# MatthewRalston/kmerdb

Hardware: AMD Instinct MI355X
Metric: k-mers counted/sec at k=12, synthetic 150 bp FASTQ (higher is better)
Workload: dtype u64

## Files before the change

### kmerdb_amd/csrc/kdb_engine.hip

```cpp
#include <hip/hip_runtime.h>

#include <cstdarg>
#include <cstddef>
#include <cstdio>
#include <cstdlib>
#include <algorithm>
#include <atomic>
#include <cstring>
#include <string>
#include <thread>
#include <vector>

#include "../../include/kdbhip.h"
#include "kdb_kernels.hip.h"
#include "kdb_hist.hip.h"
#include "kdb_scatter.hip.h"
#include "kdb_smallk.hip.h"
#include "kdb_probe.hip.h"
#include "kdb_hostparse.cpp.h"
#include "kdb_kdbwriter.cpp.h"

namespace {

thread_local std::string g_err;
// ... 180 lines not shown
        e->ev_pool.push_back(s.a);
        e->ev_pool.push_back(s.b);
    }
    e->spans.clear();
    return KDB_OK;
}

int ensure_staging(kdb_engine *e)
{
    if (e->staging_ready) return KDB_OK;
    for (int b = 0; b < NBUF; b++) {
        HIP_TRY(hipHostMalloc((void **)&e->h_bases[b], e->stage_bytes + 64, hipHostMallocDefault));
        HIP_TRY(hipHostMalloc((void **)&e->h_offs[b], (e->stage_reads + 1) * sizeof(uint64_t), hipHostMallocDefault));
        HIP_TRY(hipMalloc((void **)&e->d_bases[b], e->stage_bytes + 64));
        HIP_TRY(hipMalloc((void **)&e->d_offs[b], (e->stage_reads + 1) * sizeof(uint64_t)));
        HIP_TRY(hipEventCreateWithFlags(&e->ev_copied[b], hipEventDisableTiming));
        HIP_TRY(hipEventCreateWithFlags(&e->ev_done[b], hipEventDisableTiming));
    }
    e->staging_ready = true;
    const int64_t want = e->accum_bytes >= 0 ? e->accum_bytes : (e->k >= 13 ? (int64_t)1 << 30 : 0);
    if (want > 0) {
        e->acc_cap = (size_t)want < e->stage_bytes ? e->stage_bytes : (size_t)want;
        e->acc_reads_cap = e->acc_cap / 64 + e->stage_reads;
        for (int s = 0; s < 2; s++) {
            HIP_TRY(hipMalloc((void **)&e->d_acc_bases[s], e->acc_cap + 64));
            HIP_TRY(hipMalloc((void **)&e->d_acc_offs[s], (e->acc_reads_cap + 1) * sizeof(uint64_t)));
            HIP_TRY(hipEventCreateWithFlags(&e->ev_acc_done[s], hipEventDisableTiming));
        }
        HIP_TRY(hipEventCreateWithFlags(&e->ev_acc_copied, hipEventDisableTiming));
        e->acc_ready = true;
    }
    return KDB_OK;
}

int overlap_join(kdb_engine *e)
{
    if (e->ov.last < 0) return KDB_OK;
    HIP_TRY(hipStreamWaitEvent(e->s_compute, e->ov.hist_done[e->ov.last], 0));
    e->ov.last = -1;
    return KDB_OK;
}

int overlap_streams(kdb_engine *e)
{
    const bool want_hist = e->overlap != 0, want_mask = want_hist && e->overlap_hist_cus > 0;
    if (e->s_hist) { HIP_TRY(hipStreamSynchronize(e->s_hist)); HIP_TRY(hipStreamDestroy(e->s_hist)); e->s_hist = nullptr; }
    kdb::overlap_free(e->ov);
    if (e->compute_masked || want_mask) {
        HIP_TRY(hipStreamSynchronize(e->s_compute));
        HIP_TRY(hipStreamDestroy(e->s_compute));
        e->s_compute = nullptr;
        e->compute_masked = false;
    }
    if (!want_hist) {
        if (!e->s_compute) HIP_TRY(hipStreamCreateWithFlags(&e->s_compute, hipStreamNonBlocking));
        return KDB_OK;
    }
    if (!want_mask) {
        if (!e->s_compute) HIP_TRY(hipStreamCreateWithFlags(&e->s_compute, hipStreamNonBlocking));
        HIP_TRY(hipStreamCreateWithFlags(&e->s_hist, hipStreamNonBlocking));
        e->ov.grid = 0;
        return KDB_OK;
    }
    if (!getenv("KDB_ALLOW_CU_MASKS")) {
        e->overlap_hist_cus = 0;
        (void)overlap_streams(e);
        return fail(KDB_ERR_ARG, "overlap_hist_cus: CU-masked streams are a diagnostic (set KDB_ALLOW_CU_MASKS=1; see include/kdbhip.h)");
    }
    hipDeviceProp_t prop;
    HIP_TRY(hipGetDeviceProperties(&prop, e->device));
    const int ncu = prop.multiProcessorCount, H = e->overlap_hist_cus;
    if (H >= ncu || ncu > 1024) return fail(KDB_ERR_ARG, "overlap_hist_cus=%d of %d CUs", H, ncu);
    std::vector<uint32_t> mh((size_t)(ncu + 31) / 32, 0u), ms((size_t)(ncu + 31) / 32, 0u);
    int given = 0;
    for (int i = 0; i < ncu; i++) {
        bool hist;
        if (e->overlap_mask_mode == 1) hist = given < H && (int)(((long long)i * H) / ncu) != (int)(((long long)(i + 1) * H) / ncu);
        else if (e->overlap_mask_mode == 2) hist = given < H && (i % 32) < (H * 32 + ncu - 1) / ncu;
        else hist = i < H;
        if (hist) { mh[(size_t)i / 32] |= 1u << (i % 32); given++; } else ms[(size_t)i / 32] |= 1u << (i % 32);
    }
    HIP_TRY(hipExtStreamCreateWithCUMask(&e->s_compute, (uint32_t)ms.size(), ms.data()));
    e->compute_masked = true;
    HIP_TRY(hipExtStreamCreateWithCUMask(&e->s_hist, (uint32_t)mh.size(), mh.data()));
    e->ov.grid = 2u * (uint32_t)(ncu - given);
    return KDB_OK;
}

enum : int { BATCH_HOST_FED = 1, BATCH_CONST_INPUT = 2 };
int grow(void **p, size_t *cap, size_t need_bytes);
int launch_batch(kdb_engine *e, uint8_t *d_bases, size_t nbytes, const uint64_t *d_offs, size_t nreads, int first_is_continuation, int flags);

int flush_accumulated(kdb_engine *e)
{
    if (!e->acc_ready || e->acc_nr == 0) return KDB_OK;
    const int s = e->acc_slot;
    HIP_TRY(hipEventRecord(e->ev_acc_copied, e->s_copy));
    HIP_TRY(hipStreamWaitEvent(e->s_compute, e->ev_acc_copied, 0));
    int rc = launch_batch(e, e->d_acc_bases[s], e->acc_nb, e->d_acc_offs[s], e->acc_nr, 0, BATCH_HOST_FED);
    if (rc != KDB_OK) return rc;
    HIP_TRY(hipEventRecord(e->ev_acc_done[s], e->s_compute));
    e->acc_inflight[s] = true;
    e->acc_slot = s ^ 1;
    e->acc_nb = e->acc_nr = 0;
    return KDB_OK;
}

int launch_batch(kdb_engine *e, uint8_t *d_bases, size_t nbytes, const uint64_t *d_offs, size_t nreads, int first_is_continuation, int flags)
{
    if (nreads == 0) return KDB_OK;
    if (e->tableless) return fail(KDB_ERR_STATE, "this engine was created by kdb_create_ids: it has no count vector");
    const uint64_t ntiles = (nbytes + kdb::TILE_BYTES - 1) / kdb::TILE_BYTES;
    if (ntiles > 0x7FFFFFFFull) return fail(KDB_ERR_ARG, "batch too large: %zu bytes", nbytes);
    bool marked = false;
    auto mark = [&]() {
        ProfScope ps(e, KDB_KERNEL_MARK);
        const unsigned mg = (unsigned)std::min<uint64_t>((nreads + 255) / 256, 4096);
        if (flags & BATCH_CONST_INPUT)
            hipLaunchKernelGGL(kdb::require_uniform_kernel, dim3(1), dim3(1), 0, e->s_compute, e->d_ctr);
        else {
            hipLaunchKernelGGL(kdb::mark_reads_kernel, dim3(mg), dim3(256), 0, e->s_compute, d_bases, d_offs, (uint64_t)nreads,
                               first_is_continuation, e->d_ctr);
            marked = true;
        }
    };
    auto unmark = [&]() {
        if (!marked) return;
        ProfScope ps(e, KDB_KERNEL_MARK);
        const unsigned ug = (unsigned)std::min<uint64_t>((nreads + 255) / 256, 4096);
        hipLaunchKernelGGL(kdb::unmark_reads_kernel, dim3(ug), dim3(256), 0, e->s_compute, d_bases, d_offs, (uint64_t)nreads, first_is_continuation,
                           (const kdb::DevCounters *)e->d_ctr);
        marked = false;
    };
    bool no_first_rec = false;
    {
        const size_t need = ((nbytes >> kdb::FIRST_REC_SHIFT) + 2) * sizeof(uint32_t);
        if (e->first_rec_cap < need && e->d_first_rec) HIP_TRY(hipStreamSynchronize(e->s_compute));
        int grc = grow((void **)&e->d_first_rec, &e->first_rec_cap, need);
        if (grc == KDB_ERR_NOMEM) no_first_rec = true;
        else if (grc != KDB_OK) return grc;
    }
    {
        ProfScope ps(e, KDB_KERNEL_MARK);
        const dim3 grid((unsigned)((nreads + 255) / 256)), block(256);
        HIP_TRY(hipMemsetAsync(&e->d_ctr->neg_min_len, 0, kdb::PER_BATCH_WORDS * sizeof(unsigned long long), e->s_compute));
        const dim3 lgrid(grid.x < 1024u ? grid.x : 1024u);
        hipLaunchKernelGGL(kdb::lens_kernel, lgrid, block, 0, e->s_compute, d_offs, (uint64_t)nreads, (uint64_t)nbytes,
                           e->min_len > 0 ? e->min_len : e->k, first_is_continuation, e->d_ctr, e->d_first_rec);
    }
    if (nbytes == 0) return KDB_OK;
    if (nreads > 0xFFFFFFF0ull) return fail(KDB_ERR_ARG, "batch of %zu records: at most 2^32 - 16 per submit", nreads);
    e->bytes_in += nbytes;
    const kdb::RecStarts rs{d_offs, e->d_first_rec, (uint32_t)nreads, first_is_continuation ? 1u : 0u};
    int algo = (int)e->algo;
    if (algo == 0 || algo == 3) algo = 2;
    if (no_first_rec && algo == 2) { algo = 1; e->oom_fallbacks++; e->tp.table_is_zero = false; }
    const bool paged2 = algo == 2 && e->k > e->one_level_max_k;
    if (!paged2 || e->n_mode == KDB_N_EXPAND || !e->tp.defer) e->tp.table_is_zero = false;
    if (algo == 2) {
        EngineProf hook(e);
        const bool ex = e->n_mode == KDB_N_EXPAND;
        int rc;
        if (e->k <= kdb::SMALLK_LDS_MAX_K && !e->smallk_old)
            rc = kdb::smallk_lds_count(e->s_compute, d_bases, nbytes, rs, e->k, e->canonical, ex, e->sc.grid, e->d_table, e->d_ctr, hook);
        else if (e->k <= kdb::SMALLK_MAX) {
            mark();
            rc = kdb::smallk_count(e->s_compute, d_bases, nbytes, e->k, e->canonical, ex, e->d_table, e->d_ctr, hook);
            unmark();
        }
        else if (e->k <= e->one_level_max_k) {
            rc = 3;
            if (e->overlap && e->s_hist && !ex) {
                e->ov.sc[0].grid = e->sc.grid; e->ov.sc[0].lo_bits = e->sc.lo_bits; e->ov.sc[0].contig_pages = e->sc.contig_pages; e->ov.sc[0].wide_lines = e->sc.wide_lines;
                rc = kdb::scatter_count_overlapped(e->ov, e->s_compute, e->s_hist, d_bases, nbytes, rs, e->k, e->canonical, e->d_table, e->d_ctr, hook);
            }
            if (rc == 3) {
                { const int jrc = overlap_join(e); if (jrc != KDB_OK) return jrc; }
                rc = kdb::scatter_count(e->sc, e->s_compute, d_bases, nbytes, rs, e->k, e->canonical, ex, e->d_table, e->d_ctr, hook);
            }
        }
        else {
            const size_t lost = nreads * (size_t)(e->k - 1);
            rc = kdb::twolevel_paged_count(e->tp, e->s_compute, d_bases, nbytes, rs, nbytes > lost ? nbytes - lost : 0, e->k, e->canonical, ex, e->d_table, e->d_ctr, hook);
        }
        if (rc == 2) { e->oom_fallbacks++; algo = 1; e->tp.table_is_zero = false; }
        else if (rc != 0) return fail(KDB_ERR_HIP, "LDS-histogram path failed: %s", kdb::partition_error());
    }
    if (algo == 1) {
        { const int jrc = overlap_join(e); if (jrc != KDB_OK) return jrc; }
        mark();
        {
            ProfScope ps(e, KDB_KERNEL_COUNT);
            const bool ex = (e->n_mode == KDB_N_EXPAND);
            const dim3 grid((unsigned)ntiles), block(kdb::TPB);
#define KDB_LAUNCH_DIRECT(ID, EX)                                                                              \
    hipLaunchKernelGGL((kdb::count_direct_kernel<ID, EX>), grid, block, 0, e->s_compute, d_bases, (uint64_t)nbytes, \
                       e->k, e->canonical, e->d_table, e->d_ctr)
            if (e->k <= 16) { if (ex) KDB_LAUNCH_DIRECT(uint32_t, true); else KDB_LAUNCH_DIRECT(uint32_t, false); }
            else            { if (ex) KDB_LAUNCH_DIRECT(uint64_t, true); else KDB_LAUNCH_DIRECT(uint64_t, false); }
#undef KDB_LAUNCH_DIRECT
        }
        unmark();
    }
    if (e->n_mode == KDB_N_EXPAND && e->d_worklist) {
        ProfScope ps(e, KDB_KERNEL_COUNT);
        hipLaunchKernelGGL(kdb::expand_worklist_kernel, dim3(1024), dim3(256), 0, e->s_compute, e->d_table, e->d_ctr, e->k, e->canonical);
    }
    if (e->n_mode == KDB_N_DROP) {
        ProfScope ps(e, KDB_KERNEL_MARK);
        hipLaunchKernelGGL(kdb::resolve_suspects_kernel, dim3(4), dim3(256), 0, e->s_compute, (const uint8_t *)d_bases, (uint64_t)nbytes, d_offs, (uint64_t)nreads,
                           e->k, e->d_ctr);
    }
    HIP_TRY(hipGetLastError());
    return KDB_OK;
}

int flush_pending_paged(kdb_engine *e)
{
    if (e->tp.pending == 0) return KDB_OK;
    EngineProf hook(e);
    if (kdb::twolevel_paged_flush(e->tp, e->s_compute, e->d_table, e->d_ctr, hook)) return fail(KDB_ERR_HIP, "LDS-histogram path failed: %s", kdb::partition_error());
    return KDB_OK;
}

int check_errors(kdb_engine *e)
{
    kdb::DevCounters c;
    HIP_TRY(hipMemcpy(&c, e->d_ctr, sizeof c, hipMemcpyDeviceToHost));
    if (c.n_short)
        return fail(KDB_ERR_SHORT_READ, "%llu record(s) shorter than k=%d (reference: kmer.py:461-463 raises)",
                    c.n_short, e->k);
    if (c.bad_layout)
        return fail(KDB_ERR_ARG, "read_offsets must rise from 0 to nbytes (records tile the residue buffer exactly)");
    if (c.internal_err)
        return fail(KDB_ERR_STATE, "internal: a scatter kernel ran out of its page sequence (%llu times); counts are incomplete", c.internal_err);
    if (c.not_uniform)
        return fail(KDB_ERR_ARG, "kdb_submit_device_const needs records of one length (the buffer is never marked); use kdb_submit_device");
    if (c.n_bad)
        return fail(KDB_ERR_BAD_RESIDUE, "%llu residue(s) outside ACGTN%s (reference: kmer.py:309 / :170 raises)", c.n_bad,
                    e->n_mode == KDB_N_DROP ? " that no N in their window shields" : "");
    if (c.marks_seen != c.marks_set)
        return fail(KDB_ERR_BAD_RESIDUE, "the residue buffer holds %lld byte(s) with bit 7 set that are not record starts of their batch "
                                         "(not residues -- kmer.py:170 raises -- or marks left in a device buffer by a job that was aborted)",
                    (long long)(c.marks_seen - c.marks_set));
    return KDB_OK;
}

int grow(void **p, size_t *cap, size_t need_bytes)
{
    if (*cap >= need_bytes) return KDB_OK;
    if (*p) { (void)hipFree(*p); *p = nullptr; *cap = 0; }
    size_t want = need_bytes + need_bytes / 4 + 256;
    hipError_t err = hipMalloc(p, want);
    if (err != hipSuccess) { (void)hipGetLastError(); return fail(KDB_ERR_NOMEM, "hipMalloc(%zu) failed: %s", want, hipGetErrorString(err)); }
    *cap = want;
    return KDB_OK;
}

int shred_scratch(kdb_engine *e, size_t nbytes, size_t nreads)
{
    int rc;
    if ((rc = grow((void **)&e->sh_seq, &e->sh_seq_cap, nbytes + 64)) != KDB_OK) return rc;
    if ((rc = grow((void **)&e->sh_ids, &e->sh_ids_cap, nbytes * 8ull)) != KDB_OK) return rc;
    if (nreads && (rc = grow((void **)&e->sh_offs, &e->sh_offs_cap, (nreads + 1) * sizeof(uint64_t))) != KDB_OK) return rc;
    if (!e->sh_ctr) HIP_TRY(hipMalloc((void **)&e->sh_ctr, sizeof(kdb::DevCounters)));
    if (!e->sh_suspects) HIP_TRY(hipMalloc((void **)&e->sh_suspects, e->suspects_cap * sizeof(unsigned long long)));
    return KDB_OK;
}

int create_common(kdb_engine *e, kdb_engine **out)
{
    hipError_t err;
    if ((err = hipStreamCreateWithFlags(&e->s_compute, hipStreamNonBlocking)) != hipSuccess ||
        (err = hipStreamCreateWithFlags(&e->s_copy, hipStreamNonBlocking)) != hipSuccess ||
        (err = hipMalloc((void **)&e->d_ctr, sizeof(kdb::DevCounters))) != hipSuccess) {
        kdb_destroy(e);
        return fail(KDB_ERR_HIP, "engine setup failed: %s", hipGetErrorString(err));
    }
    int rc = kdb_reset(e);
    if (rc != KDB_OK) { kdb_destroy(e); return rc; }
    if (const char *opts = getenv("KDB_ENGINE_OPTS")) {
        std::string all(opts);
        for (size_t at = 0; at < all.size();) {
            size_t end = all.find(',', at);
            if (end == std::string::npos) end = all.size();
            const std::string kv = all.substr(at, end - at);
            at = end + 1;
            if (kv.empty()) continue;
            const size_t eq = kv.find('=');
            if (eq == std::string::npos) { kdb_destroy(e); return fail(KDB_ERR_ARG, "KDB_ENGINE_OPTS: '%s' is not name=value", kv.c_str()); }
            rc = kdb_set_option(e, kv.substr(0, eq).c_str(), (int64_t)strtoll(kv.c_str() + eq + 1, nullptr, 0));
            if (rc != KDB_OK) { kdb_destroy(e); return rc; }
        }
    }
    *out = e;
    return KDB_OK;
}

}

namespace {
struct ProbePattern { const char *name; void (*launch)(const uint8_t *, uint64_t, uint8_t *, uint64_t, uint32_t, uint32_t *, hipStream_t); uint32_t read_bytes, write_bytes; };
template <int RM, int WM, int NR, int NW>
void probe_launch(const uint8_t *src, uint64_t sb, uint8_t *dst, uint64_t db, uint32_t steps, uint32_t *sink, hipStream_t st)
{
    hipLaunchKernelGGL((kdbprobe::pattern<RM, WM, NR, NW>), dim3(512), dim3(512), 0, st, src, sb, dst, db, steps, sink);
}
using namespace kdbprobe;
#define KDB_PROBE(name, RM, WM, NR, NW) {name, probe_launch<RM, WM, NR, NW>, (uint32_t)(NR * (RM == R_PAGES15 ? 1536 : RM ? 1024 : 0)), (uint32_t)(NW * (WM ? 1024 : 0))}
const ProbePattern PROBES[] = {
    KDB_PROBE("stream_read", R_STREAM, W_NONE, 4, 0),
    KDB_PROBE("stream_write", R_NONE, W_STREAM, 0, 4),
    KDB_PROBE("pages_1k_read", R_PAGES, W_NONE, 4, 0),
    KDB_PROBE("lines_64_write", R_NONE, W_LINES_SC1, 0, 2),
    KDB_PROBE("pieces_128_write", R_NONE, W_CHUNK128_SC1, 0, 2),
    KDB_PROBE("scatter_64", R_STREAM, W_LINES_SC1, 1, 2),
    KDB_PROBE("scatter_128", R_STREAM, W_CHUNK128_SC1, 1, 2),
    KDB_PROBE("level1_64", R_STREAM, W_LINES_SC1, 1, 3),
    KDB_PROBE("level1_128", R_STREAM, W_CHUNK128_SC1, 1, 3),
    KDB_PROBE("level2_64", R_PAGES15, W_LINES_SC1, 2, 2),
    KDB_PROBE("level2_128", R_PAGES15, W_CHUNK128_SC1, 2, 2),
};
#undef KDB_PROBE
constexpr int N_PROBES = (int)(sizeof(PROBES) / sizeof(PROBES[0]));
}

extern "C" {

int kdb_abi_version(void) { return KDB_ABI_VERSION; }

const char *kdb_last_error(void) { return g_err.c_str(); }

int kdb_device_count(int *n_out)
{
    if (!n_out) return fail(KDB_ERR_ARG, "n_out is NULL");
    HIP_TRY(hipGetDeviceCount(n_out));
    return KDB_OK;
}

const char *kdb_prof_kernel_name(int kernel_id)
{
    if (kernel_id < 0 || kernel_id >= KDB_N_KERNELS) return "";
    return KERNEL_NAMES[kernel_id];
}

int kdb_create(int k, int canonicalize, int n_mode, int device_id, void *d_table, kdb_engine **out)
{
    if (!out) return fail(KDB_ERR_ARG, "out is NULL");
    *out = nullptr;
    if (k < 1 || k > 17) return fail(KDB_ERR_ARG, "k=%d outside 1..17 (4^k uint64 table must fit in HBM)", k);
    if (n_mode != KDB_N_DROP && n_mode != KDB_N_EXPAND) return fail(KDB_ERR_ARG, "n_mode=%d", n_mode);
    int ndev = 0;
    HIP_TRY(hipGetDeviceCount(&ndev));
    if (device_id < 0 || device_id >= ndev) return fail(KDB_ERR_ARG, "device_id=%d but %d device(s) visible", device_id, ndev);
    DeviceGuard g(device_id);
    kdb_engine *e = new kdb_engine();
    e->k = k; e->canonical = canonicalize ? 1 : 0; e->n_mode = n_mode; e->device = device_id;
    e->nbins = 1ull << (2 * k);
    if (d_table) {
        e->d_table = (unsigned long long *)d_table;
        e->owns_table = false;
    } else {
        size_t free_b = 0, total_b = 0;
        (void)hipMemGetInfo(&free_b, &total_b);
        const unsigned long long need = e->nbins * 8ull;
        if (free_b && need > free_b) {
            delete e;
            return fail(KDB_ERR_NOMEM, "4^%d uint64 table needs %llu bytes, device has %zu free", k, need, free_b);
        }
        hipError_t me = hipMalloc((void **)&e->d_table, need);
        if (me != hipSuccess) { delete e; return fail(KDB_ERR_NOMEM, "hipMalloc(%llu) failed: %s", need, hipGetErrorString(me)); }
        e->owns_table = true;
    }
    return create_common(e, out);
}

int kdb_create_ids(int k, int canonicalize, int device_id, kdb_engine **out)
{
    if (!out) return fail(KDB_ERR_ARG, "out is NULL");
    *out = nullptr;
    if (k < 1 || k > 17) return fail(KDB_ERR_ARG, "k=%d outside 1..17", k);
    int ndev = 0;
    HIP_TRY(hipGetDeviceCount(&ndev));
    if (device_id < 0 || device_id >= ndev) return fail(KDB_ERR_ARG, "device_id=%d but %d device(s) visible", device_id, ndev);
    DeviceGuard g(device_id);
    kdb_engine *e = new kdb_engine();
    e->k = k; e->canonical = canonicalize ? 1 : 0; e->n_mode = KDB_N_DROP; e->device = device_id;
    e->nbins = 0; e->tableless = true;
    return create_common(e, out);
}

int kdb_destroy(kdb_engine *e)
{
    if (!e) return KDB_OK;
    DeviceGuard g(e->device);
    if (e->s_compute) (void)hipStreamSynchronize(e->s_compute);
    if (e->s_copy) (void)hipStreamSynchronize(e->s_copy);
    if (e->s_hist) { (void)hipStreamSynchronize(e->s_hist); (void)hipStreamDestroy(e->s_hist); }
    kdb::overlap_free(e->ov);
    kdb::scatter_free(e->sc);
    kdb::twolevel_paged_free(e->tp);
    for (auto &s : e->spans) { (void)hipEventDestroy(s.a); (void)hipEventDestroy(s.b); }
    for (auto ev : e->ev_pool) (void)hipEventDestroy(ev);
    for (int b = 0; b < NBUF; b++) {
        if (e->h_bases[b]) (void)hipHostFree(e->h_bases[b]);
        if (e->h_offs[b]) (void)hipHostFree(e->h_offs[b]);
        if (e->d_bases[b]) (void)hipFree(e->d_bases[b]);
        if (e->d_offs[b]) (void)hipFree(e->d_offs[b]);
        if (e->ev_copied[b]) (void)hipEventDestroy(e->ev_copied[b]);
        if (e->ev_done[b]) (void)hipEventDestroy(e->ev_done[b]);
    }
    for (int s2 = 0; s2 < 2; s2++) {
        if (e->d_acc_bases[s2]) (void)hipFree(e->d_acc_bases[s2]);
        if (e->d_acc_offs[s2]) (void)hipFree(e->d_acc_offs[s2]);
        if (e->ev_acc_done[s2]) (void)hipEventDestroy(e->ev_acc_done[s2]);
    }
    if (e->ev_acc_copied) (void)hipEventDestroy(e->ev_acc_copied);
    for (int s2 = 0; s2 < 2; s2++) if (e->ev_pin[s2]) (void)hipEventDestroy(e->ev_pin[s2]);
    if (e->d_worklist) (void)hipFree(e->d_worklist);
    if (e->d_suspects) (void)hipFree(e->d_suspects);
    if (e->d_first_rec) (void)hipFree(e->d_first_rec);
    if (e->sh_suspects) (void)hipFree(e->sh_suspects);
    if (e->sh_seq) (void)hipFree(e->sh_seq);
    if (e->sh_offs) (void)hipFree(e->sh_offs);
    if (e->sh_ids) (void)hipFree(e->sh_ids);
    if (e->sh_ctr) (void)hipFree(e->sh_ctr);
    if (e->d_acc_table) (void)hipFree(e->d_acc_table);
    if (e->d_ctr) (void)hipFree(e->d_ctr);
    if (e->owns_table && e->d_table) (void)hipFree(e->d_table);
    if (e->s_compute) (void)hipStreamDestroy(e->s_compute);
    if (e->s_copy) (void)hipStreamDestroy(e->s_copy);
    delete e;
    return KDB_OK;
}

int kdb_reset(kdb_engine *e)
{
    if (!e) return fail(KDB_ERR_ARG, "engine is NULL");
    DeviceGuard g(e->device);
    e->acc_nb = e->acc_nr = 0;
    kdb::twolevel_paged_drop(e->tp);
    HIP_TRY(hipStreamSynchronize(e->s_copy));
    HIP_TRY(hipStreamSynchronize(e->s_compute));
    if (e->s_hist) { HIP_TRY(hipStreamSynchronize(e->s_hist)); e->ov.last = -1; }
    if (e->nbins) HIP_TRY(hipMemsetAsync(e->d_table, 0, e->nbins * 8ull, e->s_compute));
    if (e->d_acc_table) HIP_TRY(hipMemsetAsync(e->d_acc_table, 0, e->nbins * 8ull, e->s_compute));
    e->folded_files = e->folded_total = 0;
    e->tp.table_is_zero = e->owns_table && !e->table_escaped;
    HIP_TRY(hipMemsetAsync(e->d_ctr, 0, sizeof(kdb::DevCounters), e->s_compute));
    unsigned long long wl[2] = {0, 0}, sus[2] = {0, 0};
    if (e->n_mode == KDB_N_EXPAND) {
        if (!e->d_worklist) HIP_TRY(hipMalloc((void **)&e->d_worklist, e->worklist_cap * sizeof(unsigned long long)));
        wl[0] = (unsigned long long)(uintptr_t)e->d_worklist; wl[1] = (unsigned long long)e->worklist_cap;
        HIP_TRY(hipMemcpyAsync(&e->d_ctr->wl, wl, sizeof wl, hipMemcpyHostToDevice, e->s_compute));
    } else if (!e->tableless) {
        if (!e->d_suspects) HIP_TRY(hipMalloc((void **)&e->d_suspects, e->suspects_cap * sizeof(unsigned long long)));
        sus[0] = (unsigned long long)(uintptr_t)e->d_suspects; sus[1] = (unsigned long long)e->suspects_cap;
        HIP_TRY(hipMemcpyAsync(&e->d_ctr->sus, sus, sizeof sus, hipMemcpyHostToDevice, e->s_compute));
    }
    HIP_TRY(hipStreamSynchronize(e->s_compute));
    return KDB_OK;
}

int kdb_submit_device(kdb_engine *e, void *d_bases, size_t nbytes, const void *d_read_offsets, size_t nreads)
{
    if (!e) return fail(KDB_ERR_ARG, "engine is NULL");
    if (nreads && (!d_bases || !d_read_offsets)) return fail(KDB_ERR_ARG, "NULL device buffer");
    if (((uintptr_t)d_bases & 15u) != 0) return fail(KDB_ERR_ARG, "d_bases must be 16-byte aligned");
    DeviceGuard g(e->device);
    return launch_batch(e, (uint8_t *)d_bases, nbytes, (const uint64_t *)d_read_offsets, nreads, 0, 0);
}

int kdb_submit_device_const(kdb_engine *e, const void *d_bases, size_t nbytes, const void *d_read_offsets, size_t nreads)
{
    if (!e) return fail(KDB_ERR_ARG, "engine is NULL");
    if (nreads && (!d_bases || !d_read_offsets)) return fail(KDB_ERR_ARG, "NULL device buffer");
    if (((uintptr_t)d_bases & 15u) != 0) return fail(KDB_ERR_ARG, "d_bases must be 16-byte aligned");
    DeviceGuard g(e->device);
    return launch_batch(e, (uint8_t *)const_cast<void *>(d_bases), nbytes, (const uint64_t *)d_read_offsets, nreads, 0, BATCH_CONST_INPUT);
}

static int submit_impl(kdb_engine *e, const uint8_t *bases, size_t nbytes, const uint64_t *offs, size_t nreads, bool src_pinned, bool first_continues = false)
{
    if (!e) return fail(KDB_ERR_ARG, "engine is NULL");
    if (nreads == 0) return KDB_OK;
    if (!offs || (!bases && nbytes)) return fail(KDB_ERR_ARG, "NULL host buffer");
    if (offs[nreads] < offs[0] || offs[nreads] > nbytes) return fail(KDB_ERR_ARG, "read_offsets exceed nbytes");
    DeviceGuard g(e->device);
    int rc = ensure_staging(e);
    if (rc != KDB_OK) return rc;
    if (src_pinned) {
        const int pi = e->pin_idx;
        if (!e->ev_pin[pi]) HIP_TRY(hipEventCreateWithFlags(&e->ev_pin[pi], hipEventDisableTiming));
        if (e->pin_used[pi]) HIP_TRY(hipEventSynchronize(e->ev_pin[pi]));
    }
    const uint64_t cap = e->stage_bytes;
    const uint64_t overlap = (uint64_t)(e->k - 1);
    size_t r = 0;
    bool cont = first_continues;
    uint64_t carry = first_continues ? offs[0] : 0;
    while (r < nreads) {
        const int b = e->next_buf;
        if (e->inflight[b]) { HIP_TRY(hipEventSynchronize(e->busy[b])); e->inflight[b] = false; }
        uint8_t *hb = e->h_bases[b];
        uint64_t *ho = e->h_offs[b];
        const int first_is_cont = cont ? 1 : 0;
        const uint64_t start = cont ? carry : offs[r];
        const size_t rmax = (nreads - r < e->stage_reads) ? nreads : r + e->stage_reads;
        const uint64_t *ub = std::upper_bound(offs + r + 1, offs + rmax + 1, start + cap);
        size_t r1 = (size_t)(ub - offs) - 1;
        uint64_t nb;
        size_t nr;
        ho[0] = 0;
        if (r1 <= r) {
            nb = cap; nr = 1; ho[1] = cap;
            carry = start + cap - overlap; cont = true;
        } else {
            nb = offs[r1] - start; nr = r1 - r;
            uint64_t prev = start;
            for (size_t i = 1; i <= nr; i++) {
                const uint64_t o = offs[r + i];
                if (o < prev) return fail(KDB_ERR_ARG, "read_offsets not monotone at %zu", r + i);
                prev = o;
                ho[i] = o - start;
            }
            r = r1; cont = false;
        }
        const bool accumulate = e->acc_ready && !first_is_cont && !cont && nb <= e->acc_cap && nr <= e->acc_reads_cap;
        if (accumulate) {
            if (e->acc_nb + nb > e->acc_cap || e->acc_nr + nr > e->acc_reads_cap) { rc = flush_accumulated(e); if (rc != KDB_OK) return rc; }
            const int s = e->acc_slot;
            if (e->acc_inflight[s]) { HIP_TRY(hipEventSynchronize(e->ev_acc_done[s])); e->acc_inflight[s] = false; }
            for (size_t i = 0; i <= nr; i++) ho[i] += e->acc_nb;
            const uint8_t *src = src_pinned ? bases + start : hb;
            if (!src_pinned) parallel_copy(hb, bases + start, nb, e->copy_threads);
            HIP_TRY(hipMemcpyAsync(e->d_acc_bases[s] + e->acc_nb, src, nb, hipMemcpyHostToDevice, e->s_copy));
            HIP_TRY(hipMemcpyAsync(e->d_acc_offs[s] + e->acc_nr, ho, (nr + 1) * sizeof(uint64_t), hipMemcpyHostToDevice, e->s_copy));
            HIP_TRY(hipEventRecord(e->ev_copied[b], e->s_copy));
            e->busy[b] = e->ev_copied[b];
            e->acc_nb += nb; e->acc_nr += nr;
        } else {
            rc = flush_accumulated(e);
            if (rc != KDB_OK) return rc;
            if (src_pinned) {
                HIP_TRY(hipMemcpyAsync(e->d_bases[b], bases + start, nb, hipMemcpyHostToDevice, e->s_copy));
            } else {
                parallel_copy(hb, bases + start, nb, e->copy_threads);
                HIP_TRY(hipMemcpyAsync(e->d_bases[b], hb, nb, hipMemcpyHostToDevice, e->s_copy));
            }
            HIP_TRY(hipMemcpyAsync(e->d_offs[b], ho, (nr + 1) * sizeof(uint64_t), hipMemcpyHostToDevice, e->s_copy));
            HIP_TRY(hipEventRecord(e->ev_copied[b], e->s_copy));
            HIP_TRY(hipStreamWaitEvent(e->s_compute, e->ev_copied[b], 0));
            rc = launch_batch(e, e->d_bases[b], nb, e->d_offs[b], nr, first_is_cont, BATCH_HOST_FED);
            if (rc != KDB_OK) return rc;
            HIP_TRY(hipEventRecord(e->ev_done[b], e->s_compute));
            e->busy[b] = e->ev_done[b];
        }
        e->inflight[b] = true;
        e->next_buf = (b + 1) % NBUF;
    }
    if (src_pinned) {
        HIP_TRY(hipEventRecord(e->ev_pin[e->pin_idx], e->s_copy));
        e->pin_used[e->pin_idx] = true;
        e->pin_idx ^= 1;
    }
    return KDB_OK;
}

int kdb_submit(kdb_engine *e, const uint8_t *bases, size_t nbytes, const uint64_t *offs, size_t nreads)
{
    return submit_impl(e, bases, nbytes, offs, nreads, false);
}

int kdb_submit_pinned(kdb_engine *e, const uint8_t *bases, size_t nbytes, const uint64_t *offs, size_t nreads)
{
    return submit_impl(e, bases, nbytes, offs, nreads, true);
}

int kdb_submit_ex(kdb_engine *e, const uint8_t *bases, size_t nbytes, const uint64_t *offs, size_t nreads, int flags)
{
    if (flags & ~(KDB_SUBMIT_PINNED | KDB_SUBMIT_CONTINUES)) return fail(KDB_ERR_ARG, "kdb_submit_ex: unknown flags 0x%x", flags);
    return submit_impl(e, bases, nbytes, offs, nreads, (flags & KDB_SUBMIT_PINNED) != 0, (flags & KDB_SUBMIT_CONTINUES) != 0);
}

int kdb_host_alloc(void **out, size_t nbytes)
{
    if (!out) return fail(KDB_ERR_ARG, "out is NULL");
    *out = nullptr;
    hipError_t err = hipHostMalloc(out, nbytes ? nbytes : 1, hipHostMallocDefault);
    if (err != hipSuccess) return fail(KDB_ERR_NOMEM, "hipHostMalloc(%zu) failed: %s", nbytes, hipGetErrorString(err));
    return KDB_OK;
}

int kdb_host_free(void *p)
{
    if (p) HIP_TRY(hipHostFree(p));
    return KDB_OK;
}

int kdb_sync(kdb_engine *e)
{
    if (!e) return fail(KDB_ERR_ARG, "engine is NULL");
// ... 810 lines not shown
```

### kmerdb_amd/csrc/kdb_kernels.hip.h

```cpp
#pragma once
#include <hip/hip_runtime.h>
#include <stdint.h>

namespace kdb {

constexpr int TPB = 256;
constexpr int CHUNKS_PER_THREAD = 4;
constexpr int TILE_CHUNKS = TPB * CHUNKS_PER_THREAD;
constexpr int TILE_BYTES = TILE_CHUNKS * 16;

struct DevCounters {
    unsigned long long total_kmers;
    unsigned long long n_short;
    unsigned long long n_bad;
    unsigned long long unique;
    unsigned long long sum;
    unsigned long long bad_layout;
    unsigned long long not_uniform;
    unsigned long long internal_err;
    unsigned long long table_dirty;
    unsigned long long marks_set, marks_seen;
    unsigned long long pages_bases, lines_bases;
    unsigned long long pages_ids, lines_ids;
    unsigned long long table_bytes;
    unsigned long long neg_min_len;
    unsigned long long max_len;
    unsigned long long wl_count;
    unsigned long long sus_count;
    unsigned long long *wl;
    unsigned long long wl_cap;
    unsigned long long *sus;
    unsigned long long sus_cap;
    unsigned long long *hot_side;
};
constexpr int PER_BATCH_WORDS = 4;

__device__ __forceinline__ uint32_t batch_uniform_len(const DevCounters *c)
{
    const unsigned long long mx = c->max_len, mn = ~c->neg_min_len;
    return (mx == mn && mx != 0 && mx < (1ull << 30)) ? (uint32_t)mx : 0u;
}

constexpr int FIRST_REC_SHIFT = 12;

__global__ void __launch_bounds__(256)
lens_kernel(const uint64_t *__restrict__ offs, uint64_t nreads, uint64_t nbytes, int k, int first_is_continuation, DevCounters *ctr,
            uint32_t *__restrict__ first_rec )
{
    __shared__ unsigned long long s_len[4], s_neg[4], s_short[4], s_bad[4];
    unsigned long long len = 0, neg = 0, nshort = 0, nbadl = 0;
    const uint64_t stride = (uint64_t)gridDim.x * blockDim.x;
    for (uint64_t rb = (uint64_t)blockIdx.x * blockDim.x + threadIdx.x; rb < nreads; rb += 4 * stride) {
        uint64_t sv[4], ev[4];
#pragma unroll
        for (int u = 0; u < 4; u++) {
            const uint64_t r = rb + (uint64_t)u * stride;
            sv[u] = r < nreads ? offs[r] : 0ull;
            ev[u] = r < nreads ? offs[r + 1] : 0ull;
        }
#pragma unroll
        for (int u = 0; u < 4; u++) {
            const uint64_t r = rb + (uint64_t)u * stride, s = sv[u], e = ev[u];
            if (r >= nreads) break;
            unsigned long long l = e - s;
            neg = neg > ~l ? neg : ~l;
            if (!(r == 0 && first_is_continuation)) nshort += (l < (uint64_t)k) ? 1 : 0;
            nbadl += (r == 0 && s != 0) + (r == nreads - 1 && e != nbytes) + (e < s || e > nbytes);
            if (r == 0 && first_is_continuation) l = ~0ull;
            len = len > l ? len : l;
            if (first_rec && e > s) {
                const uint64_t e2 = e < nbytes ? e : nbytes;
                for (uint64_t b = (s + ((1ull << FIRST_REC_SHIFT) - 1ull)) >> FIRST_REC_SHIFT; (b << FIRST_REC_SHIFT) < e2; b++) first_rec[b] = (uint32_t)r;
            }
        }
    }
#pragma unroll
    for (int o = 32; o > 0; o >>= 1) {
        const unsigned long long l2 = __shfl_down(len, o, 64), n2 = __shfl_down(neg, o, 64);
        len = len > l2 ? len : l2;
        neg = neg > n2 ? neg : n2;
        nshort += __shfl_down(nshort, o, 64);
        nbadl += __shfl_down(nbadl, o, 64);
    }
    const int wave = threadIdx.x >> 6;
    if ((threadIdx.x & 63) == 0) { s_len[wave] = len; s_neg[wave] = neg; s_short[wave] = nshort; s_bad[wave] = nbadl; }
    __syncthreads();
    if (threadIdx.x == 0) {
        for (int w = 1; w < 4; w++) {
            len = len > s_len[w] ? len : s_len[w];
            neg = neg > s_neg[w] ? neg : s_neg[w];
            nshort += s_short[w];
            nbadl += s_bad[w];
        }
        if (len > __hip_atomic_load(&ctr->max_len, __ATOMIC_RELAXED, __HIP_MEMORY_SCOPE_AGENT))
            __hip_atomic_fetch_max(&ctr->max_len, len, __ATOMIC_RELAXED, __HIP_MEMORY_SCOPE_AGENT);
        if (neg > __hip_atomic_load(&ctr->neg_min_len, __ATOMIC_RELAXED, __HIP_MEMORY_SCOPE_AGENT))
            __hip_atomic_fetch_max(&ctr->neg_min_len, neg, __ATOMIC_RELAXED, __HIP_MEMORY_SCOPE_AGENT);
        if (nshort) __hip_atomic_fetch_add(&ctr->n_short, nshort, __ATOMIC_RELAXED, __HIP_MEMORY_SCOPE_AGENT);
        if (nbadl) __hip_atomic_fetch_add(&ctr->bad_layout, nbadl, __ATOMIC_RELAXED, __HIP_MEMORY_SCOPE_AGENT);
    }
}

__global__ void __launch_bounds__(256)
mark_reads_kernel(uint8_t *__restrict__ bases, const uint64_t *__restrict__ offs, uint64_t nreads,
                  int first_is_continuation, DevCounters *ctr)
{
    if (batch_uniform_len(ctr) || ctr->bad_layout) return;
    const uint64_t stride = (uint64_t)gridDim.x * blockDim.x;
    for (uint64_t r = (uint64_t)blockIdx.x * blockDim.x + threadIdx.x; r < nreads; r += stride) {
        const uint64_t s = offs[r], e = offs[r + 1];
        if (e > s && !(r == 0 && first_is_continuation)) {
            const uint8_t b = bases[s];
            if (b & 0x80u) atomicAdd(&ctr->n_bad, 1ull);
            bases[s] = b | 0x80u;
        }
    }
    if (blockIdx.x == 0 && threadIdx.x == 0) ctr->marks_set += nreads - (first_is_continuation ? 1ull : 0ull);
}

__global__ void __launch_bounds__(256)
unmark_reads_kernel(uint8_t *__restrict__ bases, const uint64_t *__restrict__ offs, uint64_t nreads,
                    int first_is_continuation, const DevCounters *ctr)
{
    if (batch_uniform_len(ctr) || ctr->bad_layout) return;
    const uint64_t stride = (uint64_t)gridDim.x * blockDim.x;
    for (uint64_t r = (uint64_t)blockIdx.x * blockDim.x + threadIdx.x; r < nreads; r += stride) {
        const uint64_t s = offs[r], e = offs[r + 1];
        if (e > s && !(r == 0 && first_is_continuation))
            bases[s] = bases[s] & 0x7Fu;
    }
}

__global__ void __launch_bounds__(256)
hibit_check_kernel(const uint8_t *__restrict__ bases, uint64_t nbytes, DevCounters *ctr)
{
    const uint4 *v4 = reinterpret_cast<const uint4 *>(bases);
    const uint64_t n16 = nbytes / 16, stride = (uint64_t)gridDim.x * blockDim.x;
    uint32_t nbad = 0;
    for (uint64_t i = (uint64_t)blockIdx.x * blockDim.x + threadIdx.x; i < n16; i += stride) {
        const uint4 x = v4[i];
        const uint32_t m = (x.x | x.y | x.z | x.w) & 0x80808080u;
        if (m) nbad += __builtin_popcount(x.x & 0x80808080u) + __builtin_popcount(x.y & 0x80808080u) +
                       __builtin_popcount(x.z & 0x80808080u) + __builtin_popcount(x.w & 0x80808080u);
    }
    if (blockIdx.x == 0 && threadIdx.x < (nbytes & 15u)) nbad += bases[n16 * 16 + threadIdx.x] >> 7;
    if (__ballot(nbad != 0) == 0) return;
    unsigned long long w = 0;
#pragma unroll
    for (int o = 32; o > 0; o >>= 1) nbad += (uint32_t)__shfl_xor((int)nbad, o, 64);
    w = nbad;
    if ((threadIdx.x & 63) == 0 && w) __hip_atomic_fetch_add(&ctr->n_bad, w, __ATOMIC_RELAXED, __HIP_MEMORY_SCOPE_AGENT);
}

__global__ void require_uniform_kernel(DevCounters *ctr)
{
    const unsigned long long mx = ctr->max_len, mn = ~ctr->neg_min_len;
    if (!(mx == mn && mx != 0 && mx < (1ull << 30))) ctr->not_uniform += 1;
}

__device__ __forceinline__ uint32_t uniform_starts(uint32_t x , uint32_t L)
{
    uint32_t d = x ? L - x : 0u, m = 0;
    if (L >= 16u) {
        d = d < 16u ? d : 16u;
        return (1u << d) & 0xFFFFu;
    }
    while (d < 16u) { m |= 1u << d; d += L; }
    return m;
}

struct Enc {
    uint32_t fwd;
    uint32_t rc;
    uint32_t inv;
    uint32_t st;
    uint32_t nn;
    uint32_t bad;
};

__device__ __forceinline__ uint32_t nonzero_bytes(uint32_t z )
{
    return (z + 0x7F7F7F7Fu) & 0x80808080u;
}

__device__ __forceinline__ uint32_t rev2(uint32_t x)
{
    uint32_t y = __builtin_bitreverse32(x);
    return ((y >> 1) & 0x55555555u) | ((y & 0x55555555u) << 1);
}

__device__ __forceinline__ bool is_iupac10(uint32_t c )
{
    return (c & 0xE0u) == 0x40u && ((0x02CC2914u >> (c & 31u)) & 1u) != 0u;
}

__device__ __forceinline__ bool residue_has_n_free_window(const uint8_t *__restrict__ bases, uint64_t s, uint64_t e, uint64_t p, int k)
{
    int run = 1;
#pragma unroll 1
    for (uint64_t q = p; q > s && run < k;) {
        q--;
        if ((bases[q] & 0x7Fu) == 0x4Eu) break;
        run++;
    }
#pragma unroll 1
    for (uint64_t q = p + 1; q < e && run < k; q++) {
        if ((bases[q] & 0x7Fu) == 0x4Eu) break;
        run++;
    }
    return run >= k;
}

__device__ __forceinline__ uint32_t defer_suspects16(uint32_t errs, uint64_t pos0, DevCounters *ctr)
{
#pragma unroll 1
    for (uint32_t m = errs; m; m &= m - 1u) {
        const unsigned long long slot = __hip_atomic_fetch_add(&ctr->sus_count, 1ull, __ATOMIC_RELAXED, __HIP_MEMORY_SCOPE_AGENT);
        if (slot < ctr->sus_cap) ctr->sus[slot] = pos0 + (uint64_t)__builtin_ctz(m);
    }
    return 0u;
}

__device__ __forceinline__ bool suspect_is_bad(const uint8_t *__restrict__ bases, uint64_t nbytes, const uint64_t *__restrict__ offs, uint64_t nreads, uint64_t p, int k)
{
    if (!is_iupac10(bases[p] & 0x7Fu)) return true;
    uint64_t s = 0, e = nbytes;
    if (offs) {
        uint64_t lo = 0, hi = nreads - 1;
        while (lo < hi) { const uint64_t mid = (lo + hi + 1) >> 1; if (offs[mid] <= p) lo = mid; else hi = mid - 1; }
        s = offs[lo]; e = offs[lo + 1] < nbytes ? offs[lo + 1] : nbytes;
    }
    return residue_has_n_free_window(bases, s, e, p, k);
}

__global__ void __launch_bounds__(256)
resolve_suspects_kernel(const uint8_t *__restrict__ bases, uint64_t nbytes, const uint64_t *__restrict__ offs , uint64_t nreads,
                        int k, DevCounters *ctr)
{
    const unsigned long long listed = ctr->sus_count;
    const unsigned long long tid = (unsigned long long)blockIdx.x * blockDim.x + threadIdx.x, nthreads = (unsigned long long)gridDim.x * blockDim.x;
    unsigned long long bad = 0;
    if (listed <= ctr->sus_cap) {
        for (unsigned long long i = tid; i < listed; i += nthreads)
            if (suspect_is_bad(bases, nbytes, offs, nreads, ctr->sus[i], k)) bad++;
    } else {
        const uint64_t nwhole = nbytes / 16;
        for (uint64_t g0 = tid * 4; g0 < nwhole; g0 += nthreads * 4) {
            uint4 v[4];
#pragma unroll
            for (int u = 0; u < 4; u++) v[u] = g0 + u < nwhole ? *reinterpret_cast<const uint4 *>(bases + (g0 + u) * 16ull) : make_uint4(0x41414141u, 0x41414141u, 0x41414141u, 0x41414141u);
#pragma unroll
            for (int u = 0; u < 4; u++) {
                const uint32_t w[4] = {v[u].x, v[u].y, v[u].z, v[u].w};
#pragma unroll
                for (int q = 0; q < 4; q++) {
                    const uint32_t x7 = w[q] & 0x7F7F7F7Fu;
                    const uint32_t t = ((x7 ^ (x7 >> 1)) >> 1) & 0x03030303u;
                    const uint32_t other = nonzero_bytes(x7 ^ __builtin_amdgcn_perm(0u, 0x54474341u , t)) & nonzero_bytes(x7 ^ 0x4E4E4E4Eu);
                    for (uint32_t m = other; m; m &= m - 1u)
                        if (suspect_is_bad(bases, nbytes, offs, nreads, (g0 + u) * 16ull + 4u * (uint32_t)q + ((uint32_t)__builtin_ctz(m) >> 3), k)) bad++;
                }
            }
        }
        if (tid == 0)
            for (uint64_t p = nwhole * 16; p < nbytes; p++) {
                const uint32_t c = bases[p] & 0x7Fu;
                if (c != 0x41u && c != 0x43u && c != 0x47u && c != 0x54u && c != 0x4Eu && suspect_is_bad(bases, nbytes, offs, nreads, p, k)) bad++;
            }
    }
    if (bad) __hip_atomic_fetch_add(&ctr->n_bad, bad, __ATOMIC_RELAXED, __HIP_MEMORY_SCOPE_AGENT);
}

__device__ __forceinline__ uint32_t gather16(uint32_t y0, uint32_t y1, uint32_t y2, uint32_t y3)
{
    uint32_t lo = __builtin_amdgcn_udot4(y1, 0x80402010u, __builtin_amdgcn_udot4(y0, 0x08040201u, 0u, false), false);
    uint32_t hi = __builtin_amdgcn_udot4(y3, 0x80402010u, __builtin_amdgcn_udot4(y2, 0x08040201u, 0u, false), false);
    return ((hi << 8) | lo) >> 7;
}

template <bool EXPAND, bool NEED_BAD, bool FULL>
__device__ __forceinline__ Enc encode16(const uint32_t w[4], int nvalid , bool uniform, uint32_t ustarts)
{
    uint32_t fwd = 0;
    uint32_t notacgt[4], notn[4], start[4];
#pragma unroll
    for (int q = 0; q < 4; q++) {
        const uint32_t x = w[q];
        const uint32_t x7 = x & 0x7F7F7F7Fu;
        const uint32_t t = ((x7 >> 1) ^ (x7 >> 2)) & 0x03030303u;
        fwd |= __builtin_amdgcn_udot4(t, 0x01041040u, 0u, false) << (24 - 8 * q);
        const uint32_t expect = __builtin_amdgcn_perm(0u, 0x54474341u , t);
        notacgt[q] = nonzero_bytes(x7 ^ expect);
        if (EXPAND || NEED_BAD) notn[q] = nonzero_bytes(x7 ^ 0x4E4E4E4Eu);
        start[q] = x & 0x80808080u;
    }
    const uint32_t exist = (FULL || nvalid >= 16) ? 0xFFFFu : ((1u << nvalid) - 1u);
    Enc e;
    e.fwd = fwd;
    e.rc = ~rev2(fwd);
    const uint32_t inv = gather16(notacgt[0], notacgt[1], notacgt[2], notacgt[3]);
    e.inv = FULL ? inv : ((inv | ~exist) & 0xFFFFu);
    e.st = uniform ? ustarts : gather16(start[0], start[1], start[2], start[3]);
    if (!FULL) e.st &= exist;
    e.bad = 0; e.nn = 0;
    if (EXPAND || NEED_BAD) {
        e.bad = gather16(notacgt[0] & notn[0], notacgt[1] & notn[1], notacgt[2] & notn[2], notacgt[3] & notn[3]) & exist;
        if (EXPAND) e.nn = inv & ~e.bad & exist;
        if (NEED_BAD && uniform && ((start[0] | start[1] | start[2] | start[3]) != 0u))
            e.bad |= gather16(start[0], start[1], start[2], start[3]) & exist;
    }
    return e;
}

__device__ __forceinline__ int load_chunk(const uint8_t *__restrict__ bases, uint64_t nbytes, uint64_t g, uint32_t w[4])
{
    uint64_t b0 = g * 16ull;
    if (b0 + 16ull <= nbytes) {
        const uint4 v = *reinterpret_cast<const uint4 *>(bases + b0);
        w[0] = v.x; w[1] = v.y; w[2] = v.z; w[3] = v.w;
        return 16;
    }
    w[0] = w[1] = w[2] = w[3] = 0;
    if (b0 >= nbytes) return 0;
    int n = (int)(nbytes - b0);
    for (int i = 0; i < n; i++) w[i >> 2] |= (uint32_t)bases[b0 + i] << (8 * (i & 3));
    return n;
}

template <bool EXPAND>
struct TileLds {
    uint32_t fwd[TILE_CHUNKS + 1];
    uint32_t rc[TILE_CHUNKS + 1];
    uint32_t msk[TILE_CHUNKS + 1];
    uint32_t nn[EXPAND ? TILE_CHUNKS + 1 : 1];
};

struct UniformStarts {
    uint32_t L, stepmod, jmod;
    __device__ __forceinline__ UniformStarts(uint32_t ulen, int threads)
        : L(ulen), stepmod(ulen ? (uint32_t)(threads * 16) % ulen : 0u), jmod(ulen ? (16u * threadIdx.x) % ulen : 0u) {}
};

template <bool EXPAND, bool NEED_BAD>
__device__ __forceinline__ uint32_t stage_chunk(TileLds<EXPAND> &L, const uint8_t *__restrict__ bases, uint64_t nbytes, uint64_t g, int c,
                                                bool uniform, uint32_t ustarts, DevCounters *ctr = nullptr)
{
    uint32_t w[4];
    Enc e;
    if ((g + 1) * 16ull <= nbytes) {
        const uint4 v = *reinterpret_cast<const uint4 *>(bases + g * 16ull);
        w[0] = v.x; w[1] = v.y; w[2] = v.z; w[3] = v.w;
        e = encode16<EXPAND, NEED_BAD, true>(w, 16, uniform, ustarts);
    } else {
        const int nv = load_chunk(bases, nbytes, g, w);
        e = encode16<EXPAND, NEED_BAD, false>(w, nv, uniform, ustarts);
    }
    L.fwd[c] = e.fwd; L.rc[c] = e.rc; L.msk[c] = e.inv | (e.st << 16);
    if (EXPAND) L.nn[c] = e.nn;
    if (NEED_BAD && !EXPAND && e.bad && ctr) {
        uint32_t hib = 0;
        if (uniform) hib = gather16(w[0] & 0x80808080u, w[1] & 0x80808080u, w[2] & 0x80808080u, w[3] & 0x80808080u);
        const uint32_t over = defer_suspects16(e.bad & ~hib, g * 16ull, ctr);
        return ((uint32_t)__builtin_popcount(e.bad & hib) + over) | (uniform ? 0u : (uint32_t)__builtin_popcount(e.st) << 16);
    }
    return NEED_BAD ? (uint32_t)__builtin_popcount(e.bad) | (uniform ? 0u : (uint32_t)__builtin_popcount(e.st) << 16) : 0u;
}

template <bool EXPAND, int THREADS = TPB, bool NEED_BAD = true>
__device__ __forceinline__ void stage_tile(TileLds<EXPAND> &L, const uint8_t *__restrict__ bases, uint64_t nbytes,
                                           uint64_t tile, uint32_t *bad_count, const UniformStarts &us, DevCounters *ctr = nullptr)
{
    const int j = threadIdx.x;
    uint32_t nbad = 0;
    uint32_t x = 0, tmod = 0;
    const bool uniform = us.L != 0;
    if (uniform) {
        tmod = (uint32_t)((tile * (uint64_t)TILE_BYTES) % us.L);
        x = tmod + us.jmod;
        if (x >= us.L) x -= us.L;
    }
#pragma unroll
    for (int q = 0; q < TILE_CHUNKS / THREADS; q++) {
        const int c = j + q * THREADS;
        nbad += stage_chunk<EXPAND, NEED_BAD>(L, bases, nbytes, tile * TILE_CHUNKS + (uint64_t)c, c, uniform,
                                              uniform ? uniform_starts(x, us.L) : 0u, ctr);
        if (uniform) { x += us.stepmod; if (x >= us.L) x -= us.L; }
    }
    if (j == 0) {
        uint32_t hx = 0;
        if (uniform) { hx = tmod + (uint32_t)TILE_BYTES % us.L; if (hx >= us.L) hx -= us.L; }
        (void)stage_chunk<EXPAND, false>(L, bases, nbytes, (tile + 1) * TILE_CHUNKS, TILE_CHUNKS, uniform,
                                         uniform ? uniform_starts(hx, us.L) : 0u);
    }
    *bad_count = nbad;
}

struct Hood {
    uint32_t f0, f1;
    uint32_t r0, r1;
    uint32_t V;
    uint32_t S;
    __device__ __forceinline__ uint64_t F() const { return ((uint64_t)f0 << 32) | f1; }
    __device__ __forceinline__ uint64_t R() const { return ((uint64_t)r1 << 32) | r0; }
};

template <bool EXPAND>
__device__ __forceinline__ Hood load_hood(const TileLds<EXPAND> &L, int c)
{
    Hood h;
    h.f0 = L.fwd[c]; h.f1 = L.fwd[c + 1]; h.r0 = L.rc[c]; h.r1 = L.rc[c + 1];
    const uint32_t m0 = L.msk[c], m1 = L.msk[c + 1];
    h.V = (m0 & 0xFFFFu) | (m1 << 16);
    h.S = (m0 >> 16) | (m1 & 0xFFFF0000u);
    return h;
}

__device__ __forceinline__ bool window_crosses(const Hood &h, int i, uint32_t k1mask) { return (((h.S >> 1) >> i) & k1mask) != 0; }

struct WinOr {
    uint32_t s0, s1, s2, s3, d, w;
    __device__ __forceinline__ explicit WinOr(int k)
    {
        w = (uint32_t)(k - 1);
        uint32_t m = 1;
// ... 412 lines not shown
```

### kmerdb_amd/csrc/kdb_scatter.hip.h

```cpp
#pragma once
#include <hip/hip_runtime.h>
#include <stdint.h>

#include "kdb_kernels.hip.h"
#include "kdb_hist.hip.h"

namespace kdb {

constexpr int SC_THREADS = 512;
constexpr int SC_TILE_CHUNKS = 512;
constexpr int SC_LINE_BYTES = 64;
constexpr int SC_PAGE_LINES = 16;
constexpr int SC_PAGE_BYTES = SC_LINE_BYTES * SC_PAGE_LINES;
constexpr int SC_TAG_SHIFT = 12;
constexpr uint32_t SC_NO_PAGE = 0xFFFFFFFFu;
constexpr int SC_GRID = 512;
constexpr int SC_HOT = 64;
constexpr int SC_LO_BITS_ONE_LEVEL = 9, SC_LO_BITS_TWO_LEVEL = 12;
constexpr int SC_LO_BITS_MAX = 15;


constexpr int SC_TILE_STRIDE = SC_TILE_CHUNKS - 1;
constexpr int SC_TILE_POS = SC_TILE_STRIDE * 16;
constexpr uint32_t SC_NPOS_MAX = 256;
// ... 81 lines not shown
        mark(p);
    }
}

template <bool EXPAND, bool NLIST = false , typename TILE>
__device__ __forceinline__ uint32_t sc_stage_chunk(TILE &L, const ScChunk &ch, int c, bool uniform, uint32_t ustarts, uint32_t gen, uint64_t pos0, DevCounters *ctr,
                                                   bool owner = true )
{
    const uint32_t w[4] = {ch.v.x, ch.v.y, ch.v.z, ch.v.w};
    uint32_t fwd = 0, back[4];
#pragma unroll
    for (int q = 0; q < 4; q++) {
        const uint32_t t = ((w[q] ^ (w[q] >> 1)) >> 1) & 0x03030303u;
        fwd |= __builtin_amdgcn_udot4(t, 0x01041040u, 0u, false) << (24 - 8 * q);
        back[q] = w[q] ^ __builtin_amdgcn_perm(0u, 0x54474341u , t);
    }
    if (uniform && ((back[0] | back[1] | back[2] | back[3]) | ch.nexist) == 0u) {
        L.fwd[c] = fwd; L.msk[c] = ustarts << 16;
        if (EXPAND) L.nn[c] = 0u;
        return 0u;
    }
    uint32_t notacgt[4];
#pragma unroll
    for (int q = 0; q < 4; q++) notacgt[q] = nonzero_bytes(back[q] & 0x7F7F7F7Fu);
    const uint32_t exist = 0xFFFFu & ~ch.nexist;
    const uint32_t inv = gather16(notacgt[0], notacgt[1], notacgt[2], notacgt[3]) | ch.nexist;
    uint32_t st = ustarts;
    uint32_t nbad = 0, nn = 0, nmark = 0, hi16 = 0;
    const uint32_t hib = (w[0] | w[1] | w[2] | w[3]) & 0x80808080u;
    if (!uniform) {
        st = gather16(w[0] & 0x80808080u, w[1] & 0x80808080u, w[2] & 0x80808080u, w[3] & 0x80808080u) & exist;
        nmark = (uint32_t)__builtin_popcount(st);
    } else if (hib) {
        hi16 = gather16(w[0] & 0x80808080u, w[1] & 0x80808080u, w[2] & 0x80808080u, w[3] & 0x80808080u) & exist;
        nbad = (uint32_t)__builtin_popcount(hi16);
    }
    if (inv & exist) {
        uint32_t b4[4];
#pragma unroll
        for (int q = 0; q < 4; q++) b4[q] = notacgt[q] & nonzero_bytes((w[q] & 0x7F7F7F7Fu) ^ 0x4E4E4E4Eu);
        const uint32_t bad = gather16(b4[0], b4[1], b4[2], b4[3]) & exist;
        nn = inv & ~bad & exist;
        uint32_t errs = bad & ~hi16;
        nbad += (!EXPAND && errs) ? (owner ? defer_suspects16(errs, pos0, ctr) : 0u) : (uint32_t)__builtin_popcount(errs);
    }
    L.fwd[c] = fwd; L.msk[c] = inv | ((st & exist) << 16);
    if (EXPAND) { L.nn[c] = nn; if (nn) L.has_n[0] = gen; }
    if (EXPAND && NLIST && nn) {
        uint32_t sl = atomicAdd(&L.ncnt, (uint32_t)__builtin_popcount(nn));
#pragma unroll 1
        for (uint32_t m = nn; m; m &= m - 1u) { if (sl < SC_NPOS_MAX) L.npos[sl] = (uint16_t)(16u * (uint32_t)c + (uint32_t)__builtin_ctz(m)); sl++; }
    }
    return nbad | (nmark << 16);
}

#ifdef KDB_SC_PROF
__device__ unsigned long long g_sc_prof[32];
__device__ int g_sc_ablate;
#define SC_ABLATE(bit) (g_sc_ablate & (bit))
#define SC_STAMP_INIT unsigned long long sc_last, sc_acc[8] = {0, 0, 0, 0, 0, 0, 0, 0}; asm volatile("s_memtime %0\n\ts_waitcnt lgkmcnt(0)" : "=s"(sc_last) :: "memory")
#define SC_STAMP(i) do { unsigned long long sc_t; asm volatile("s_memtime %0\n\ts_waitcnt lgkmcnt(0)" : "=s"(sc_t) :: "memory"); sc_acc[i] += sc_t - sc_last; sc_last = sc_t; } while (0)
#define SC_STAMP_FN [&](int sc_i) { SC_STAMP(sc_i); }
#define SC_STAMP_END_AT(o) do { if ((threadIdx.x & 63) == 0) for (int q = 0; q < 8; q++) atomicAdd(&g_sc_prof[(o) + q], sc_acc[q]); if (threadIdx.x == 0) atomicAdd(&g_sc_prof[(o) + 8], 1ull); } while (0)
#define SC_STAMP_END SC_STAMP_END_AT(0)
__device__ unsigned long long g_sc_wg[2][2][1024];
#define SC_WG_CLOCK(kern, what) do { if (threadIdx.x == 0 && blockIdx.x < 1024) g_sc_wg[kern][what][blockIdx.x] = wall_clock64(); } while (0)
#else
#define SC_WG_CLOCK(kern, what)
#define SC_ABLATE(bit) 0
#define SC_STAMP_INIT
#define SC_STAMP(i)
#define SC_STAMP_FN NoStamp()
#define SC_STAMP_END_AT(o)
#define SC_STAMP_END
#endif

struct u24 {};
struct u16w {};
template <typename ELEM> struct ElemFmt;
template <> struct ElemFmt<uint16_t> { using lo_t = uint16_t; static constexpr bool HI = false; static constexpr int LINE_ELEMS = 32, PAGE_BYTES = 1024, LINE_BYTES = 64, PAGE_LINES = 16; };
template <> struct ElemFmt<uint32_t> { using lo_t = uint32_t; static constexpr bool HI = false; static constexpr int LINE_ELEMS = 16, PAGE_BYTES = 1024, LINE_BYTES = 64, PAGE_LINES = 16; };
template <> struct ElemFmt<u24>      { using lo_t = uint16_t; static constexpr bool HI = true;  static constexpr int LINE_ELEMS = 32, PAGE_BYTES = 1536, LINE_BYTES = 64, PAGE_LINES = 16; };
template <> struct ElemFmt<u16w>     { using lo_t = uint16_t; static constexpr bool HI = false; static constexpr int LINE_ELEMS = 64, PAGE_BYTES = 1024, LINE_BYTES = 128, PAGE_LINES = 8; };
struct u24w {};
struct u32w {};
template <> struct ElemFmt<u24w>     { using lo_t = uint16_t; static constexpr bool HI = true;  static constexpr int LINE_ELEMS = 64, PAGE_BYTES = 1536, LINE_BYTES = 128, PAGE_LINES = 8; };
template <> struct ElemFmt<u32w>     { using lo_t = uint32_t; static constexpr bool HI = false; static constexpr int LINE_ELEMS = 32, PAGE_BYTES = 1024, LINE_BYTES = 128, PAGE_LINES = 8; };
constexpr int SC_HI_OFFSET = SC_PAGE_LINES * SC_LINE_BYTES;

template <typename ELEM, int RINGS, int C>
struct alignas(16) RingLds {
    using F = ElemFmt<ELEM>;
    using lo_t = typename F::lo_t;
    static_assert((C & (C - 1)) == 0 && C >= 2 * F::LINE_ELEMS, "ring = at least two lines, power of two");
    static constexpr uint32_t SZ = (uint32_t)sizeof(lo_t);
    static constexpr uint32_t INC = (1u << 16) | SZ;
    static constexpr uint32_t POS_MASK = (uint32_t)C * SZ - 1u;
    static constexpr uint32_t FULL_MASK = 0xFFFF0000u & ~((uint32_t)(C - 1) << 16);
    static constexpr uint32_t WRAP = F::HI ? 2u * (uint32_t)C : (uint32_t)C;
    uint32_t word[RINGS];
    lo_t ring[RINGS * C];
    uint8_t hi[F::HI ? RINGS * WRAP : 4];
    uint32_t pg_count;
    uint32_t retry[2];
    unsigned long long hot_tag[SC_HOT];
    uint32_t hot_cnt[SC_HOT];

    __device__ __forceinline__ void put(uint32_t woff , uint32_t got , uint32_t el)
    {
        const uint32_t off = (woff * (uint32_t)(C * sizeof(lo_t) / 4)) | (got & POS_MASK);
        *reinterpret_cast<lo_t *>(reinterpret_cast<char *>(ring) + off) = (lo_t)el;
        if (F::HI) *(reinterpret_cast<uint8_t *>(hi) + ((woff * (WRAP / 4u)) | ((got & (WRAP * SZ - 1u)) / SZ))) = (uint8_t)(el >> 16);
    }
    static __device__ __forceinline__ void decode(uint32_t wd, uint32_t *r, uint32_t *head)
    {
        const uint32_t fill = wd >> 16;
        *head = ((wd & 0xFFFFu) / SZ - fill) & (WRAP - 1u);
        *r = fill > (uint32_t)C ? (uint32_t)C : fill;
    }
    static __device__ __forceinline__ uint32_t encode(uint32_t head, uint32_t fill)
    {
        return (fill << 16) | (((head + fill) & (WRAP - 1u)) * SZ);
    }
    static __device__ __forceinline__ uint32_t line_elem(uint32_t b, uint32_t p)
    {
        const uint32_t lo = b * (uint32_t)C + (p & (uint32_t)(C - 1));
        return F::HI ? lo | ((b * WRAP + (p & (WRAP - 1u) & ~(2u * (uint32_t)F::LINE_ELEMS - 1u))) << 16) : lo;
    }
};

template <typename ELEM>
__device__ __forceinline__ uint8_t *page_line(uint8_t *pages, uint32_t line )
{
    using F = ElemFmt<ELEM>;
    if (F::PAGE_BYTES == F::PAGE_LINES * F::LINE_BYTES) return pages + (size_t)line * F::LINE_BYTES;
    return pages + (size_t)(line / F::PAGE_LINES) * F::PAGE_BYTES + (size_t)(line % F::PAGE_LINES) * F::LINE_BYTES;
}
template <typename ELEM>
__device__ __forceinline__ uint8_t *page_line_hi(uint8_t *pages, uint32_t line)
{
    using F = ElemFmt<ELEM>;
    return pages + (size_t)(line / F::PAGE_LINES) * F::PAGE_BYTES + SC_HI_OFFSET + (size_t)(line % F::PAGE_LINES) * (F::LINE_BYTES / 2);
}

struct ScOut {
    uint8_t *pages;
    uint32_t *tag;
    uint32_t wg_pages;
    const uint32_t *wg_range;
    uint32_t contig;
    uint32_t wg_base;
    uint32_t grid;
    uint32_t extra_elems;
};

__device__ __forceinline__ uint32_t sc_pin(uint32_t v) { asm volatile("" : "+s"(v)); return v; }

__device__ __forceinline__ ScOut sc_out_of_workgroup(ScOut o)
{
    if (o.wg_range) {
        o.wg_base = o.wg_range[blockIdx.x];
        o.wg_pages = o.wg_range[blockIdx.x + 1] - o.wg_base;
    } else {
        o.wg_base = o.contig ? blockIdx.x * o.wg_pages : blockIdx.x;
    }
    o.wg_base = sc_pin(o.wg_base); o.wg_pages = sc_pin(o.wg_pages); o.contig = sc_pin(o.contig);
    o.grid = sc_pin(gridDim.x);
    return o;
}

struct RingOwner {
    uint32_t pg = SC_NO_PAGE, ln = 0;
};

template <typename ELEM, int RINGS, int C>
__device__ __forceinline__ uint32_t ring_next_line(RingLds<ELEM, RINGS, C> &R, const ScOut &o, RingOwner &w, uint32_t bucket, DevCounters *ctr)
{
    constexpr uint32_t LINE_ELEMS = ElemFmt<ELEM>::LINE_ELEMS, PAGE_LINES = ElemFmt<ELEM>::PAGE_LINES;
    if (w.pg == SC_NO_PAGE || w.ln == PAGE_LINES) {
        const bool tag_when_taken = o.wg_range == nullptr;
        if (w.pg != SC_NO_PAGE && !tag_when_taken && !SC_ABLATE(4)) o.tag[w.pg] = (bucket << SC_TAG_SHIFT) | (PAGE_LINES * LINE_ELEMS);
        uint32_t p = atomicAdd(&R.pg_count, 1u);
        const uint32_t cap = o.wg_pages;
        if (p >= cap) {
            __hip_atomic_fetch_add(&ctr->internal_err, 1ull, __ATOMIC_RELAXED, __HIP_MEMORY_SCOPE_AGENT);
            p = cap - 1;
        }
        w.pg = (o.wg_range || o.contig) ? o.wg_base + p : p * o.grid + o.wg_base;
        w.ln = 0;
        if (tag_when_taken && !SC_ABLATE(4)) o.tag[w.pg] = (bucket << SC_TAG_SHIFT) | (PAGE_LINES * LINE_ELEMS);
    }
    return w.pg * PAGE_LINES + w.ln++;
}

__device__ __forceinline__ void store_line16(uint8_t *p, const uint4 &x)
{
#if defined(KDB_LINE_STORE_PLAIN)
    *reinterpret_cast<uint4 *>(p) = x;
#else
    typedef uint32_t u32x4 __attribute__((ext_vector_type(4)));
    const u32x4 v = {x.x, x.y, x.z, x.w};
#if defined(KDB_LINE_STORE_NT)
    asm volatile("global_store_dwordx4 %0, %1, off nt" : : "v"(p), "v"(v) : "memory");
#else
    asm volatile("global_store_dwordx4 %0, %1, off sc1" : : "v"(p), "v"(v) : "memory");
#endif
#endif
}

struct LineDesc { uint32_t elem, line; };

template <typename ELEM, int RINGS, int C, typename Stamp>
__device__ __forceinline__ void rings_flush_wave(RingLds<ELEM, RINGS, C> &R, const ScOut &o, RingOwner &w, uint32_t b, uint32_t bucket, DevCounters *ctr,
                                                 LineDesc *desc , Stamp stamp)
{
    using F = ElemFmt<ELEM>;
    using lo_t = typename F::lo_t;
    constexpr uint32_t LINE_ELEMS = F::LINE_ELEMS;
    const uint32_t lane = threadIdx.x & 63u;
    const uint32_t wd = b < (uint32_t)RINGS ? R.word[b] : 0u;
    uint32_t r, base;
    R.decode(wd, &r, &base);
    const uint32_t nfull = r / LINE_ELEMS;
#pragma unroll 1
    for (uint32_t l = 0; l < (uint32_t)C / LINE_ELEMS; l++) {
        const bool has = nfull > l;
        const uint64_t m = __ballot(has);
        if (!m) break;
        const uint32_t n = (uint32_t)__popcll(m);
        if (has) {
            LineDesc d;
            d.elem = R.line_elem(b, base + l * LINE_ELEMS);
            d.line = ring_next_line(R, o, w, bucket, ctr);
            desc[lane_rank_in(m)] = d;
        }
        __builtin_amdgcn_wave_barrier();
        stamp(6);
        const char *const rb = reinterpret_cast<const char *>(R.ring), *const hb = reinterpret_cast<const char *>(R.hi);
        constexpr uint32_t LPL = (uint32_t)F::LINE_BYTES / 16u, GROUP = 64u / LPL;
        const uint32_t q16 = (lane & (LPL - 1u)) * 16u;
        for (uint32_t g = 0; g < n; g += 2u * GROUP) {
            const uint32_t e0 = g + lane / LPL, e1 = e0 + GROUP;
            const LineDesc d0 = desc[e0 < n ? e0 : 0u], d1 = desc[e1 < n ? e1 : 0u];
            const uint32_t lo0 = F::HI ? d0.elem & 0xFFFFu : d0.elem, lo1 = F::HI ? d1.elem & 0xFFFFu : d1.elem;
            const uint4 x0 = *reinterpret_cast<const uint4 *>(rb + lo0 * (uint32_t)sizeof(lo_t) + q16);
            const uint4 x1 = *reinterpret_cast<const uint4 *>(rb + lo1 * (uint32_t)sizeof(lo_t) + q16);
            uint4 y0 = make_uint4(0, 0, 0, 0), y1 = y0;
            const bool pair0 = F::HI && (lo0 & LINE_ELEMS) != 0u, pair1 = F::HI && (lo1 & LINE_ELEMS) != 0u;
            if (F::HI) {
                y0 = *reinterpret_cast<const uint4 *>(hb + (d0.elem >> 16) + q16);
                y1 = *reinterpret_cast<const uint4 *>(hb + (d1.elem >> 16) + q16);
            }
            if (e0 < n) {
                if (!SC_ABLATE(1)) store_line16(page_line<ELEM>(o.pages, d0.line) + q16, x0);
                if (pair0 && !SC_ABLATE(2)) store_line16(page_line_hi<ELEM>(o.pages, d0.line - 1u) + q16, y0);
            }
            if (e1 < n) {
                if (!SC_ABLATE(1)) store_line16(page_line<ELEM>(o.pages, d1.line) + q16, x1);
                if (pair1 && !SC_ABLATE(2)) store_line16(page_line_hi<ELEM>(o.pages, d1.line - 1u) + q16, y1);
            }
        }
        __builtin_amdgcn_wave_barrier();
        stamp(7);
    }
    if (nfull) R.word[b] = R.encode(base + nfull * LINE_ELEMS, r - nfull * LINE_ELEMS);
}

template <typename ELEM, int RINGS, int C>
__device__ __forceinline__ void ring_copy_line(RingLds<ELEM, RINGS, C> &R, const ScOut &o, RingOwner &w, uint32_t elem, uint32_t bucket, DevCounters *ctr)
{
    using F = ElemFmt<ELEM>;
    const uint32_t line = ring_next_line(R, o, w, bucket, ctr);
    const uint4 *src = reinterpret_cast<const uint4 *>(&R.ring[F::HI ? elem & 0xFFFFu : elem]);
    uint4 *dst = reinterpret_cast<uint4 *>(page_line<ELEM>(o.pages, line));
    constexpr int Q = F::LINE_BYTES / 16;
    uint4 x[Q];
#pragma unroll
    for (int q = 0; q < Q; q++) x[q] = src[q];
#pragma unroll
    for (int q = 0; q < Q; q++) dst[q] = x[q];
    if (F::HI) {
        const uint4 *sh = reinterpret_cast<const uint4 *>(&R.hi[elem >> 16]);
        uint4 *dh = reinterpret_cast<uint4 *>(page_line_hi<ELEM>(o.pages, line & ~1u));
        uint4 y[Q];
#pragma unroll
        for (int q = 0; q < Q; q++) y[q] = sh[q];
#pragma unroll
        for (int q = 0; q < Q; q++) dh[q] = y[q];
    }
}

template <typename ELEM, int RINGS, int C>
__device__ __forceinline__ void ring_drain(RingLds<ELEM, RINGS, C> &R, const ScOut &o, RingOwner &w, uint32_t b, uint32_t bucket, DevCounters *ctr)
{
    constexpr uint32_t LINE_ELEMS = ElemFmt<ELEM>::LINE_ELEMS;
    uint32_t r, base;
    R.decode(R.word[b], &r, &base);
    const uint32_t nfull = r / LINE_ELEMS, rem = r - nfull * LINE_ELEMS;
    if (ElemFmt<ELEM>::HI && r == 0 && w.pg != SC_NO_PAGE && (w.ln & 1u)) {
        constexpr int Q = ElemFmt<ELEM>::LINE_BYTES / 16;
        const uint4 *sh = reinterpret_cast<const uint4 *>(&R.hi[R.line_elem(b, base - LINE_ELEMS) >> 16]);
        uint4 *dh = reinterpret_cast<uint4 *>(page_line_hi<ELEM>(o.pages, w.pg * (uint32_t)ElemFmt<ELEM>::PAGE_LINES + w.ln - 1u));
        uint4 y[Q];
#pragma unroll
        for (int q = 0; q < Q; q++) y[q] = sh[q];
#pragma unroll
        for (int q = 0; q < Q; q++) dh[q] = y[q];
    }
    for (uint32_t l = 0; l < nfull + (rem ? 1u : 0u); l++)
        ring_copy_line(R, o, w, R.line_elem(b, base + l * LINE_ELEMS), bucket, ctr);
    if (w.pg != SC_NO_PAGE) o.tag[w.pg] = (bucket << SC_TAG_SHIFT) | ((w.ln - (rem ? 1u : 0u)) * LINE_ELEMS + rem);
    R.word[b] = 0;
    w = RingOwner();
}

struct NoStamp { __device__ __forceinline__ void operator()(int) const {} };
struct NoHook { __device__ __forceinline__ void operator()() const {} };
template <bool V> struct BoolTag { static constexpr bool value = V; };
template <typename ELEM, int RINGS, int C, int NID, int ROUND, typename Make, typename Overlap, typename Stamp = NoStamp, typename Between = NoHook>
__device__ __forceinline__ void rings_place(RingLds<ELEM, RINGS, C> &R, const ScOut &out, RingOwner &own, uint32_t my_ring ,
                                            uint32_t my_bucket, DevCounters *ctr,
                                            LineDesc *desc, Make make, uint32_t pend, uint32_t &round,
                                            Overlap overlap, Stamp stamp = Stamp() , Between between = Between())
{
    static_assert(NID % ROUND == 0, "whole rounds");
    using RL = RingLds<ELEM, RINGS, C>;
    const int j = threadIdx.x;
    bool overlapped = false, hooked = false;
    uint32_t woff[NID], el[NID];
#pragma unroll
    for (int g = 0; g < NID; g += ROUND) {
        uint32_t retry_mask = (pend >> g) & ((1u << ROUND) - 1u);
        auto pass = [&](auto first_tag) -> bool {
            constexpr bool FIRST = decltype(first_tag)::value;
            auto requests = [&]() {
            uint32_t sh = retry_mask << (32 - ROUND);
            bool act[ROUND];
            uint32_t got[ROUND];
#pragma unroll
            for (int u = ROUND - 1; u >= 0; u--) {
                if (FIRST) make(g + u, woff[g + u], el[g + u]);
                uint32_t nsh;
                act[u] = __builtin_uadd_overflow(sh, sh, &nsh);
                sh = nsh;
                got[u] = 0u;
                if (act[u]) got[u] = atomicAdd(reinterpret_cast<uint32_t *>(reinterpret_cast<char *>(R.word) + woff[g + u]), RL::INC);
            }
            if (!overlapped) { overlapped = true; overlap(); }
            uint32_t ovf = 0;
#pragma unroll
            for (int u = 0; u < ROUND; u++) ovf |= got[u];
            if (FIRST && __ballot((ovf & RL::FULL_MASK) != 0) == 0) {
#pragma unroll
                for (int u = 0; u < ROUND; u++) {
                    if (act[u])
                        R.put(woff[g + u], got[u], el[g + u]);
                }
                retry_mask = 0;
            } else {
                uint32_t still = 0;
#pragma unroll
                for (int u = 0; u < ROUND; u++) {
                    if (act[u]) {
                        if ((got[u] & RL::FULL_MASK) == 0) R.put(woff[g + u], got[u], el[g + u]);
                        else still |= 1u << u;
                    }
                }
                retry_mask = still;
            }
            };
            requests();
            if (__ballot(retry_mask != 0) && (j & 63) == 0) R.retry[round & 1u] = 1u;
            stamp(1);
            __syncthreads();
            stamp(2);
            if (!hooked) { hooked = true; between(); }
            const uint32_t again = R.retry[round & 1u];
            if (j == 0) R.retry[(round + 1u) & 1u] = 0u;
            rings_flush_wave(R, out, own, my_ring, my_bucket, ctr, desc + (j & ~63), stamp);
            round++;
            stamp(3);
            __syncthreads();
            stamp(4);
            return again != 0u;
        };
        bool again = pass(BoolTag<true>());
        while (again) again = pass(BoolTag<false>());
    }
}

__device__ __forceinline__ void hot_add(unsigned long long *__restrict__ table, DevCounters *ctr, unsigned long long id, unsigned long long n)
{
    unsigned long long *side = ctr->hot_side;
    if (side) {
        const unsigned long long slot = __hip_atomic_fetch_add(&side[0], 1ull, __ATOMIC_RELAXED, __HIP_MEMORY_SCOPE_AGENT);
        if (slot < side[1]) { side[2 + 2 * slot] = id; side[3 + 2 * slot] = n; }
        else __hip_atomic_fetch_add(&ctr->internal_err, 1ull, __ATOMIC_RELAXED, __HIP_MEMORY_SCOPE_AGENT);
        return;
    }
    __hip_atomic_fetch_add(&table[id], n, __ATOMIC_RELAXED, __HIP_MEMORY_SCOPE_AGENT);
    ctr->table_dirty = 1;
}

__global__ void hot_side_kernel(DevCounters *ctr, unsigned long long *side, unsigned long long cap)
{
    if (side) { side[0] = 0ull; side[1] = cap; }
    ctr->hot_side = side;
}

__global__ void __launch_bounds__(256)
apply_hot_kernel(const unsigned long long *__restrict__ side, unsigned long long *__restrict__ table)
{
    const unsigned long long n = side[0] < side[1] ? side[0] : side[1];
    for (unsigned long long i = (unsigned long long)blockIdx.x * blockDim.x + threadIdx.x; i < n; i += (unsigned long long)gridDim.x * blockDim.x)
        __hip_atomic_fetch_add(&table[side[2 + 2 * i]], side[3 + 2 * i], __ATOMIC_RELAXED, __HIP_MEMORY_SCOPE_AGENT);
}

__device__ __forceinline__ uint32_t windows_nonly16(const Hood &h, uint32_t N32, uint32_t bad16, const WinOr &o)
{
    Hood a = h, b = h;
    a.V = h.V & ~N32; a.S = 0u;
    b.V = 0u;
    return bad16 & ~windows_bad16(a, o) & ~windows_bad16(b, o) & 0xFFFFu;
}

struct NWindow { uint64_t base; uint32_t sh0, sh1, nfill; };

__device__ __forceinline__ NWindow nwindow_decode(uint64_t F, int i, int k, uint64_t idmask, uint32_t nwin )
{
    NWindow w;
    const uint32_t m = (uint32_t)__builtin_popcount(nwin);
    const uint32_t j0 = (uint32_t)__builtin_ctz(nwin | 0x80000000u), rest = nwin & (nwin - 1u);
    const uint32_t j1 = rest ? (uint32_t)__builtin_ctz(rest) : j0;
    w.sh0 = 2u * ((uint32_t)k - 1u - j0); w.sh1 = 2u * ((uint32_t)k - 1u - j1);
    w.base = ((F >> (64 - 2 * k - 2 * i)) & idmask) & ~(3ull << w.sh0) & ~(3ull << w.sh1);
    w.nfill = m == 1u ? 4u : m == 2u ? 16u : 0u;
    return w;
}

template <bool CANON>
__device__ __forceinline__ uint64_t nwindow_fill(const NWindow &w, uint32_t f, int k, uint64_t idmask)
{
    uint64_t id = w.base | ((uint64_t)(f & 3u) << w.sh0) | ((uint64_t)(f >> 2) << w.sh1);
    if (CANON) {
        uint64_t y = __builtin_bitreverse64(id);
        y = ((y >> 1) & 0x5555555555555555ull) | ((y & 0x5555555555555555ull) << 1);
        const uint64_t r = (~y >> (64 - 2 * k)) & idmask;
        id = id < r ? id : r;
    }
    return id;
}

constexpr uint32_t NQ_ENTRIES = 128;
struct NQueue {
    uint32_t *q0, *q1;
    uint32_t n;
    __device__ __forceinline__ uint32_t &at(uint32_t e) { return (e < 64u ? q0 : q1)[e & 63u]; }
};

__device__ __forceinline__ uint32_t wave_incl_scan(uint32_t v);

__device__ __forceinline__ uint32_t wave_incl_scan(uint32_t v)
{
    v += (uint32_t)__builtin_amdgcn_update_dpp(0, (int)v, 0x111, 0xF, 0xF, false);
    v += (uint32_t)__builtin_amdgcn_update_dpp(0, (int)v, 0x112, 0xF, 0xF, false);
    v += (uint32_t)__builtin_amdgcn_update_dpp(0, (int)v, 0x114, 0xF, 0xF, false);
    v += (uint32_t)__builtin_amdgcn_update_dpp(0, (int)v, 0x118, 0xF, 0xF, false);
    v += (uint32_t)__builtin_amdgcn_update_dpp(0, (int)v, 0x142, 0xA, 0xF, false);
    v += (uint32_t)__builtin_amdgcn_update_dpp(0, (int)v, 0x143, 0xC, 0xF, false);
    return v;
}

template <typename ID, typename ELEM, int RINGS, int C, int ROUND, bool EXPAND, bool CANON, int K = 0, int THREADS = SC_THREADS, bool RAGGED = false>
__global__ void __launch_bounds__(THREADS, 4)
scatter_bases_kernel(const uint8_t *__restrict__ bases, uint64_t nbytes, uint32_t tile0, uint32_t ntiles, int k,
                     int ring_shift ,
                     int ring_bits , int sub_log2 ,
                     ScOut out_arg, unsigned long long *__restrict__ table, DevCounters *ctr, RecStarts rs)
{
    constexpr int NID = 16;
    if ((batch_uniform_len(ctr) == 0u) != RAGGED) return;
    if (RAGGED && ctr->bad_layout) return;
    constexpr int TILE_CHUNKS = THREADS, TILE_STRIDE = THREADS - 1, TILE_POS = TILE_STRIDE * 16;
    using Tile = ScTile<EXPAND, TILE_CHUNKS>;
    if (K == 17 && !ElemFmt<ELEM>::HI) { k = 17; ring_shift = SC_LO_BITS_TWO_LEVEL + 9; ring_bits = 9; sub_log2 = __builtin_ctz((unsigned)RINGS) - 9; }
    else
    if (K && !ElemFmt<ELEM>::HI) { k = K; ring_shift = SC_LO_BITS_ONE_LEVEL; ring_bits = 2 * K - (int)(8 * sizeof(typename ElemFmt<ELEM>::lo_t) - (K <= 12 ? 1 : 0)); sub_log2 = __builtin_ctz((unsigned)RINGS) - ring_bits; }
    if (K && ElemFmt<ELEM>::HI) { k = K; ring_shift = SC_LO_BITS_TWO_LEVEL + 9; ring_bits = 2 * K - 24; sub_log2 = __builtin_ctz((unsigned)RINGS) - ring_bits; }
    const ScOut out = sc_out_of_workgroup(out_arg);
    const uint32_t G = out.grid;
    ntiles = sc_pin(ntiles);
    __shared__ Tile T[2];
    static_assert(sizeof(Tile) >= THREADS * sizeof(LineDesc), "a dead tile image holds the waves' line lists");
    __shared__ RingLds<ELEM, RINGS, C> R;
    const int j = threadIdx.x;
    for (int b = j; b < RINGS; b += THREADS) R.word[b] = 0;
    if (j == 0) { R.pg_count = 0; R.retry[0] = 0; R.retry[1] = 0; T[0].has_n[0] = 0; T[1].has_n[0] = 0; T[0].ncnt = 0; T[1].ncnt = 0; }
    if (j < SC_HOT) { R.hot_tag[j] = 0ull; R.hot_cnt[j] = 0; }
    if (EXPAND) __syncthreads();
    RingOwner own;
    static_assert(THREADS % RINGS == 0, "whole threads per ring");
    constexpr int OWN_STEP = THREADS / RINGS;
    const uint32_t my_ring = (j % OWN_STEP) == 0 ? (uint32_t)(j / OWN_STEP) : (uint32_t)RINGS;
    const uint32_t my_bucket = my_ring >> sub_log2;
    const uint32_t sub4 = ((uint32_t)j & ((1u << sub_log2) - 1u)) * 4u;
    const int ring_word_sh = sub_log2 + 2;
    const int canonical = CANON ? 1 : 0;
    const IdParams<ID> idp(k, canonical);
    const WinOr winor(k);
    const uint64_t idmask = (1ull << (2 * k)) - 1ull;
    const uint32_t kmask = (1u << k) - 1u;
    const ID keep = (ID)(((ID)1 << ring_shift) - 1);
    const bool owner_of_windows = j < TILE_STRIDE;
    const uint32_t ulen = batch_uniform_len(ctr);
    uint32_t x = 0, xstep = 0;
    if (ulen) {
        x = (uint32_t)((((uint64_t)tile0 + blockIdx.x) * (uint64_t)TILE_POS + 16ull * j) % ulen);
        xstep = (uint32_t)(((uint64_t)G * TILE_POS) % ulen);
    }
    unsigned long long extra = 0;
    uint32_t stat_tot = 0;
    uint32_t round = 0;
    int buf = sc_pin(0);
    SC_STAMP_INIT;
    SC_WG_CLOCK(0, 0);

    const uint32_t my_byte = 16u * (uint32_t)j;
    auto fetch_tile = [&](uint64_t tile_no) -> ScChunk {
        const uint64_t first = tile_no * (uint64_t)(TILE_STRIDE * 16);
        if (first + (uint64_t)(TILE_CHUNKS * 16) <= nbytes) {
            ScChunk c;
            c.v = load_once16(bases + first + my_byte);
            c.nexist = 0u;
            return c;
        }
        return sc_fetch(bases, nbytes, tile_no * TILE_STRIDE + (uint64_t)j);
    };
    ScChunk mine;
    mine.v = make_uint4(0, 0, 0, 0); mine.nexist = 0xFFFFu;
    if (blockIdx.x < ntiles) {
        mine = fetch_tile((uint64_t)tile0 + blockIdx.x);
        const uint32_t nb_ = sc_stage_chunk<EXPAND, true>(T[0], mine, j, true, ulen ? uniform_starts(x, ulen) : 0u, blockIdx.x + 1u,
                                                          (((uint64_t)tile0 + blockIdx.x) * TILE_STRIDE + (uint64_t)j) * 16ull, ctr, owner_of_windows);
        if (owner_of_windows) stat_tot += nb_;
        if (ulen) { x += xstep; if (x >= ulen) x -= ulen; }
        if (blockIdx.x + G < ntiles) mine = fetch_tile((uint64_t)tile0 + blockIdx.x + G);
    }
    __syncthreads();
    constexpr bool ragged = RAGGED;
    auto first_rec_of = [&](uint64_t tile_no) -> uint32_t {
        uint32_t idx = (uint32_t)((tile_no * (uint64_t)TILE_POS) >> FIRST_REC_SHIFT);
        asm volatile("" : "+v"(idx));
        return rs.first_rec[idx];
    };
    uint32_t first_next = 0;
    StartProbe probe, probe2;
    probe.r = 0; probe.off = ~0ull; probe.beyond = ~0ull;
    probe2 = probe;
    if (ragged && blockIdx.x < ntiles) {
        const uint64_t P0 = ((uint64_t)tile0 + blockIdx.x) * (uint64_t)TILE_POS;
        starts_apply<THREADS>(T[0], rs, P0, starts_fetch<THREADS>(rs, rs.first_rec[P0 >> FIRST_REC_SHIFT], j));
        if (blockIdx.x + G < ntiles) probe2 = starts_fetch<THREADS>(rs, rs.first_rec[(((uint64_t)tile0 + blockIdx.x + G) * (uint64_t)TILE_POS) >> FIRST_REC_SHIFT], j);
        if (blockIdx.x + 2 * G < ntiles) first_next = first_rec_of((uint64_t)tile0 + blockIdx.x + 2ull * G);
        __syncthreads();
    }

    auto ring_and_element = [&](ID id, uint32_t &woff_u, uint32_t &el_u) {
        const uint32_t ring = sizeof(ID) > 4 ? (uint32_t)((uint64_t)id >> ring_shift) & ((1u << ring_bits) - 1u)
                                             : __builtin_amdgcn_ubfe((uint32_t)id, (uint32_t)ring_shift, (uint32_t)ring_bits);
        woff_u = (ring << ring_word_sh) | sub4;
        el_u = bfi((uint32_t)keep, (uint32_t)id, (uint32_t)(id >> ring_bits));
    };

    for (uint32_t t = blockIdx.x; t < ntiles; t += G) {
        const uint64_t tile = (uint64_t)tile0 + t;
        const Hood h = sc_load_hood<CANON>(T[buf], j < TILE_STRIDE ? j : 0);
        const uint32_t bad16 = owner_of_windows ? windows_bad16(h, winor) : 0xFFFFu;
        uint32_t N32 = 0;
        if (EXPAND && owner_of_windows) N32 = (T[buf].nn[j] & 0xFFFFu) | (T[buf].nn[j + 1] << 16);
        const uint32_t ncnt = EXPAND ? T[buf].ncnt : 0u;
        const uint32_t kinv = (1u << 20) / (uint32_t)k + 1u;
        uint32_t np_first = 0;
        if (EXPAND) np_first = T[buf].npos[(((uint32_t)j * kinv) >> 20) & (SC_NPOS_MAX - 1u)];
        if (EXPAND && ncnt != 0u) {
            SC_STAMP(0);
            constexpr uint32_t PAGE_ELEMS = (uint32_t)ElemFmt<ELEM>::LINE_ELEMS * (uint32_t)ElemFmt<ELEM>::PAGE_LINES;
            using RL = RingLds<ELEM, RINGS, C>;
            const uint32_t tiles_left = (ntiles - t + G - 1u) / G;
            const uint32_t fills_max = ncnt <= SC_NPOS_MAX ? 8u * ncnt * (uint32_t)k : (uint32_t)THREADS * 8u;
            const uint32_t need = (uint32_t)(((uint64_t)tiles_left * TILE_POS + (uint64_t)fills_max + (uint64_t)RINGS * C + PAGE_ELEMS - 1u) / PAGE_ELEMS) + (uint32_t)RINGS + 2u;
            const bool room = R.pg_count + need <= out.wg_pages;
            auto place4 = [&](const ID (&fid)[4], uint32_t live) {
                uint32_t fw[4], fe[4], fg[4];
#pragma unroll
                for (int u = 0; u < 4; u++) {
                    ring_and_element(fid[u], fw[u], fe[u]);
                    fg[u] = RL::FULL_MASK;
                    if (room && ((live >> u) & 1u)) fg[u] = atomicAdd(reinterpret_cast<uint32_t *>(reinterpret_cast<char *>(R.word) + fw[u]), RL::INC);
                }
#pragma unroll
                for (int u = 0; u < 4; u++) {
                    if (!((live >> u) & 1u)) continue;
                    if ((fg[u] & RL::FULL_MASK) == 0u) { R.put(fw[u], fg[u], fe[u]); continue; }
                    __hip_atomic_fetch_add(&table[(uint64_t)fid[u]], 1ull, __ATOMIC_RELAXED, __HIP_MEMORY_SCOPE_AGENT);
                    extra += 1ull; ctr->table_dirty = 1;
                }
            };
            if (ncnt <= SC_NPOS_MAX) {
                const uint32_t npairs = ncnt * (uint32_t)k;
#pragma unroll 1
                for (uint32_t pr = (uint32_t)j; pr < npairs; pr += (uint32_t)THREADS) {
                    const uint32_t n = (pr * kinv) >> 20, w = pr - n * (uint32_t)k;
                    const int W = (int)(pr == (uint32_t)j ? np_first : (uint32_t)T[buf].npos[n]) - (int)w;
                    if (W < 0 || W >= TILE_POS) continue;
                    const int wc = W >> 4;
                    const uint32_t wi = (uint32_t)W & 15u;
                    const uint32_t m0 = T[buf].msk[wc], m1 = T[buf].msk[wc + 1];
                    const uint32_t f0w = T[buf].fwd[wc], f1w = T[buf].fwd[wc + 1];
                    const uint32_t Vw = (m0 & 0xFFFFu) | (m1 << 16), Sw = (m0 >> 16) | (m1 & 0xFFFF0000u);
                    const uint32_t Nw = (T[buf].nn[wc] & 0xFFFFu) | (T[buf].nn[wc + 1] << 16);
                    const uint32_t nwin = (Nw >> wi) & kmask;
                    const bool ok = ((Vw >> wi) & kmask) == nwin && (((Sw >> 1) >> wi) & (kmask >> 1)) == 0u && (nwin & ((1u << w) - 1u)) == 0u;
                    if (!ok) continue;
                    const uint64_t F = ((uint64_t)f0w << 32) | f1w;
                    if (__builtin_popcount(nwin) > 2) { expand_n_window(table, F, (int)wi, k, canonical, idmask, nwin, &extra, ctr); continue; }
                    if (sizeof(ID) == 4) {
                        const uint32_t km2 = 2u * (uint32_t)(k - 1), rest = nwin & (nwin - 1u);
                        const uint32_t s0 = km2 - 2u * (uint32_t)__builtin_ctz(nwin), s1 = rest ? km2 - 2u * (uint32_t)__builtin_ctz(rest) : s0;
                        const uint32_t top = wi ? __builtin_amdgcn_alignbit(f0w, f1w, 32u - 2u * wi) : f0w;
                        const uint32_t bf = (top >> (32 - 2 * k)) & ~(3u << s0) & ~(3u << s1);
                        const uint32_t br = CANON ? (rc_word(bf) >> (32 - 2 * k)) & ~(3u << (km2 - s0)) & ~(3u << (km2 - s1)) : 0u;
#pragma unroll 1
                        for (uint32_t g = 0; g < (rest ? 4u : 1u); g++) {
                            const uint32_t bfg = rest ? bf | (g << s1) : bf, brg = rest ? br | ((3u - g) << (km2 - s1)) : br;
                            ID fid[4];
#pragma unroll
                            for (uint32_t u = 0; u < 4u; u++) {
                                const uint32_t a = bfg | (u << s0), r = brg | ((3u - u) << (km2 - s0));
                                fid[u] = (ID)(CANON ? (a < r ? a : r) : a);
                            }
                            place4(fid, 0xFu);
                        }
                        continue;
                    }
                    const NWindow nw = nwindow_decode(F, (int)wi, k, idmask, nwin);
#pragma unroll 1
                    for (uint32_t f0 = 0; f0 < nw.nfill; f0 += 4u) {
                        ID fid[4];
// ... 15 lines not shown
            const uint32_t nonly = (N32 && bad16) ? windows_nonly16(h, N32, bad16, winor) : 0u;
            const uint32_t km2 = 2u * (uint32_t)(k - 1);
            ID nbf[2] = {0, 0}, nbr[2] = {0, 0};
            uint32_t nsh[2] = {0, 0}, pend2 = 0;
            if (__ballot(nonly != 0u)) {
                uint32_t one_n = 0, two_n = 0;
#pragma unroll 1
                for (uint32_t m = nonly; m; m &= m - 1u) {
                    const int i = __builtin_ctz(m);
                    const uint32_t nwin = (N32 >> i) & kmask, cnt = (uint32_t)__builtin_popcount(nwin);
                    if (cnt == 1u) one_n |= 1u << i;
                    else if (cnt == 2u) two_n |= 1u << i;
                    else expand_n_window(table, h.F(), i, k, canonical, idmask, nwin, &extra, ctr);
                }
                const uint32_t mine_n = (uint32_t)__builtin_popcount(one_n) + 4u * (uint32_t)__builtin_popcount(two_n);
                const uint32_t incl = wave_incl_scan(mine_n), tot = (uint32_t)__builtin_amdgcn_readlane((int)incl, 63);
                uint32_t sl = incl - mine_n;
                Q.n = tot < NQ_ENTRIES ? tot : NQ_ENTRIES;
#pragma unroll 1
                for (uint32_t m = one_n | two_n; m; m &= m - 1u) {
                    const uint32_t i = (uint32_t)__builtin_ctz(m), nwin = (N32 >> i) & kmask;
                    const uint32_t j0 = (uint32_t)__builtin_ctz(nwin), rest = nwin & (nwin - 1u);
                    const uint32_t e0 = lane | (i << 6) | (j0 << 10);
                    if (!rest) {
                        if (sl < NQ_ENTRIES) Q.at(sl) = e0; else to_vector(nwindow_decode(h.F(), (int)i, k, idmask, nwin));
                        sl++;
                    } else if (sl + 4u <= NQ_ENTRIES) {
                        const uint32_t e1 = e0 | ((uint32_t)__builtin_ctz(rest) << 15) | (1u << 22);
                        Q.at(sl) = e1; Q.at(sl + 1u) = e1 | (1u << 20); Q.at(sl + 2u) = e1 | (2u << 20); Q.at(sl + 3u) = e1 | (3u << 20);
                        sl += 4u;
                    } else {
                        to_vector(nwindow_decode(h.F(), (int)i, k, idmask, nwin));
                        for (uint32_t q = 0; q < 4u; q++) if (sl + q < NQ_ENTRIES) Q.at(sl + q) = 0xFFFFFFFFu;
                        sl += 4u;
                    }
                }
                __builtin_amdgcn_wave_barrier();
            }
            if (Q.n) {
#pragma unroll
                for (uint32_t q = 0; q < 2u; q++) {
                    const uint32_t ei = lane * 2u + q;
                    const uint32_t e = ei < Q.n ? Q.at(ei) : 0xFFFFFFFFu;
                    if (e != 0xFFFFFFFFu) {
                        const int c = wbase + (int)(e & 63u);
                        const uint32_t i = (e >> 6) & 15u, s0 = km2 - 2u * ((e >> 10) & 31u);
                        const uint64_t F = ((uint64_t)T[buf].fwd[c] << 32) | T[buf].fwd[c + 1];
                        ID bf = (ID)((F >> (64 - 2 * k - 2 * (int)i)) & idmask) & ~((ID)3 << s0);
                        if ((e >> 22) & 1u) { const uint32_t s1 = km2 - 2u * ((e >> 15) & 31u); bf = (bf & ~((ID)3 << s1)) | ((ID)((e >> 20) & 3u) << s1); }
                        nbf[q] = bf; nsh[q] = s0; pend2 |= 0xFu << (4u * q);
                        if (CANON) {
                            uint64_t y = __builtin_bitreverse64((uint64_t)bf);
                            y = ((y >> 1) & 0x5555555555555555ull) | ((y & 0x5555555555555555ull) << 1);
                            nbr[q] = (ID)((~y >> (64 - 2 * k)) & idmask) & ~((ID)3 << (km2 - s0));
                        }
                    }
                }
            }
            auto fill_id = [&](int u) -> ID {
                const ID f0 = (ID)(u & 3);
                ID id = nbf[u >> 2] | (f0 << nsh[u >> 2]);
                if (CANON) {
                    const ID r = nbr[u >> 2] | (((ID)3 - f0) << (km2 - nsh[u >> 2]));
                    id = id < r ? id : r;
                }
                return id;
            };
            if (pend2 & 0xFu) { const ID fid[4] = {fill_id(0), fill_id(1), fill_id(2), fill_id(3)}; place4(fid, pend2 & 0xFu); }
            if (pend2 >> 4)   { const ID fid[4] = {fill_id(4), fill_id(5), fill_id(6), fill_id(7)}; place4(fid, pend2 >> 4); }
            }
            SC_STAMP(5);
        }
        uint64_t same; uint32_t id0;
        const bool degenerate = wave_dominant(k < 16 ? h.f0 >> (32 - 2 * k) : h.f0, &same, &id0);
        uint32_t pend = ~bad16 & 0xFFFFu;
        if (degenerate) {
#pragma unroll 1
            for (int u = 0; u < NID; u++) {
                const ID idu = idp.id_any(h, u);
                const bool live = (pend >> u) & 1u;
                const uint64_t act = __ballot(live);
                if (!act) continue;
                const int first = __ffsll((unsigned long long)act) - 1;
                const uint32_t lo0 = (uint32_t)__builtin_amdgcn_readlane((int)(uint32_t)idu, first);
                const uint32_t hi0 = sizeof(ID) > 4 ? (uint32_t)__builtin_amdgcn_readlane((int)(uint32_t)((uint64_t)idu >> 32), first) : 0u;
                const bool same_id = live && (uint32_t)idu == lo0 && (sizeof(ID) > 4 ? (uint32_t)((uint64_t)idu >> 32) == hi0 : true);
                const uint64_t grp = __ballot(same_id);
                if (__popcll(grp) >= 16 && same_id) {
                    pend &= ~(1u << u);
                    if (lane_rank_in(grp) == 0) {
                        const uint32_t n = (uint32_t)__popcll(grp);
                        const unsigned long long want = (1ull << 40) | (unsigned long long)idu;
                        const uint32_t hs = ((uint32_t)idu * 2654435761u) >> (32 - 6);
                        const unsigned long long old = atomicCAS(&R.hot_tag[hs], 0ull, want);
                        if (old == 0ull || old == want) atomicAdd(&R.hot_cnt[hs], n);
                        else hot_add(table, ctr, (unsigned long long)idu, (unsigned long long)n);
                        extra += (unsigned long long)n;
                    }
                }
            }
        }
        uint32_t r2lo = 0, r2hi = 0;
        if (CANON && sizeof(ID) == 4) {
            const uint64_t r2 = h.R() << (2 * (16 - k));
            r2lo = (uint32_t)r2; r2hi = (uint32_t)(r2 >> 32);
        }
        auto make = [&](int u, uint32_t &woff_u, uint32_t &el_u) {
            ID id;
            if (CANON && sizeof(ID) == 4) {
                const uint32_t wf = u == 0 ? h.f0 : __builtin_amdgcn_alignbit(h.f0, h.f1, 32 - 2 * u);
                const uint32_t wr = u == 0 ? r2lo : __builtin_amdgcn_alignbit(r2hi, r2lo, 2 * u);
                id = (ID)((wf < wr ? wf : wr) >> (32 - 2 * k));
            } else {
                id = idp.id(h, u);
            }
            ring_and_element(id, woff_u, el_u);
        };
        SC_STAMP(0);
        rings_place<ELEM, RINGS, C, NID, ROUND>(R, out, own, my_ring, my_bucket, ctr, reinterpret_cast<LineDesc *>(&T[buf]), make, pend, round, [&]() {
            if (t + G < ntiles) {
                const uint32_t nb_ = sc_stage_chunk<EXPAND, true>(T[buf ^ 1], mine, j, true, ulen ? uniform_starts(x, ulen) : 0u, t + G + 1u,
                                                                  ((tile + G) * TILE_STRIDE + (uint64_t)j) * 16ull, ctr, owner_of_windows);
                if (owner_of_windows) stat_tot += nb_;
                if (ulen) { x += xstep; if (x >= ulen) x -= ulen; }
                if (ragged) {
                    probe = probe2;
                    if (t + 2 * G < ntiles) {
                        probe2 = starts_fetch<THREADS>(rs, first_next, j);
                        if (t + 3 * G < ntiles) first_next = first_rec_of(tile + 3ull * G);
                    }
                }
                if (t + 2 * G < ntiles) mine = fetch_tile(tile + 2ull * G);
            }
        }, SC_STAMP_FN, [&]() {
            if (ragged && t + G < ntiles) starts_apply<THREADS>(T[buf ^ 1], rs, (tile + G) * (uint64_t)TILE_POS, probe);
            if (EXPAND && j == 0) T[buf].ncnt = 0u;
        });
        SC_STAMP(1);
        buf = sc_pin(buf ^ 1);
    }

    if (my_ring < (uint32_t)RINGS && !SC_ABLATE(8)) ring_drain(R, out, own, my_ring, my_bucket, ctr);
    if (j < SC_HOT && R.hot_tag[j])
        hot_add(table, ctr, R.hot_tag[j] & ((1ull << 40) - 1ull), (unsigned long long)R.hot_cnt[j]);
    SC_STAMP(5);
    SC_STAMP_END;
    SC_WG_CLOCK(0, 1);
    const unsigned long long we = wave_sum(extra), wb = wave_sum((unsigned long long)(stat_tot & 0xFFFFu)), wm = wave_sum((unsigned long long)(stat_tot >> 16));
    if ((j & 63) == 0) {
        if (we) __hip_atomic_fetch_add(&ctr->total_kmers, we, __ATOMIC_RELAXED, __HIP_MEMORY_SCOPE_AGENT);
        if (wb) __hip_atomic_fetch_add(&ctr->n_bad, wb, __ATOMIC_RELAXED, __HIP_MEMORY_SCOPE_AGENT);
        if (wm) __hip_atomic_fetch_add(&ctr->marks_seen, wm, __ATOMIC_RELAXED, __HIP_MEMORY_SCOPE_AGENT);
    }
}

struct PageEntry { uint32_t page, nelems; };

__device__ __forceinline__ uint32_t l2_digit_of(const uint32_t *__restrict__ page_base, uint32_t nb1, uint32_t p)
{
    uint32_t lo = 0, hi = nb1 - 1;
    while (lo < hi) { const uint32_t mid = (lo + hi + 1) >> 1; if (page_base[mid] <= p) lo = mid; else hi = mid - 1; }
    return lo;
}

__global__ void __launch_bounds__(1024)
l2_plan_kernel(const uint32_t *__restrict__ page_base1 , uint32_t nb1, uint32_t G, uint32_t rings, uint32_t in_page_elems,
               uint32_t *__restrict__ wg_range , uint32_t *__restrict__ cursor ,
               uint32_t cap , DevCounters *ctr)
{
    __shared__ uint32_t wsum[1024 / 64];
    const uint32_t w = threadIdx.x, P = page_base1[nb1];
    uint32_t need = 0;
    if (w < G) {
        const uint32_t s0 = (uint32_t)((uint64_t)P * w / G), s1 = (uint32_t)((uint64_t)P * (w + 1) / G);
        if (s1 > s0) {
            const uint32_t d0 = l2_digit_of(page_base1, nb1, s0), d1 = l2_digit_of(page_base1, nb1, s1 - 1);
            need = ((s1 - s0) * in_page_elems + 511u) / 512u + rings * (d1 - d0 + 1u) + 1u;
        }
    }
    uint32_t tot;
    const uint32_t excl = block_excl_scan<1024>(need, wsum, &tot);
    const uint32_t range0 = *cursor;
    const bool fits = tot <= cap - (range0 < cap ? range0 : cap);
    __syncthreads();
    if (w < G) wg_range[w] = range0 + (fits ? excl : 0u);
    if (w == 0) { wg_range[G] = range0 + (fits ? tot : 0u); *cursor = range0 + (fits ? tot : 0u); if (!fits) atomicAdd(&ctr->internal_err, 1ull); }
}

template <typename IN , typename ELEM , int RINGS, int C, bool FIXED = false ,
          int THREADS = SC_THREADS>
__global__ void __launch_bounds__(THREADS, 4)
scatter_ids_kernel(const uint8_t *__restrict__ pages1, const PageEntry *__restrict__ list1, const uint32_t *__restrict__ page_base1, uint32_t nb1,
                   int ring_shift, int ring_bits, ScOut out_arg, DevCounters *ctr)
{
    if (FIXED) { ring_shift = SC_LO_BITS_TWO_LEVEL; ring_bits = 9; }
    const ScOut out = sc_out_of_workgroup(out_arg);
    constexpr int NID = 16;
    constexpr int EP = ElemFmt<IN>::LINE_ELEMS * SC_PAGE_LINES / 64;
    constexpr int PPT = NID / EP;
    constexpr uint32_t NWAVES = THREADS / 64;
    constexpr uint32_t L2_TILE_PAGES = NWAVES * PPT;
    constexpr size_t IN_PAGE_BYTES = ElemFmt<IN>::PAGE_BYTES;
    static_assert(THREADS % RINGS == 0, "whole threads per ring");
    constexpr int OWN_STEP = THREADS / RINGS;
    __shared__ RingLds<ELEM, RINGS, C> R;
    __shared__ LineDesc desc[THREADS];
    const int j = threadIdx.x, wave = j >> 6, lane = j & 63;
    for (int b = j; b < RINGS; b += THREADS) R.word[b] = 0;
    if (j == 0) { R.pg_count = 0; R.retry[0] = 0; R.retry[1] = 0; }
    RingOwner own;
    const uint32_t my_ring = (j % OWN_STEP) == 0 ? (uint32_t)(j / OWN_STEP) : (uint32_t)RINGS;
    const uint32_t keep = (1u << ring_shift) - 1u;
    const uint32_t P = page_base1[nb1];
    const uint32_t s0 = (uint32_t)((uint64_t)P * blockIdx.x / out.grid), s1 = (uint32_t)((uint64_t)P * (blockIdx.x + 1) / out.grid);
    uint32_t round = 0;
    __syncthreads();
    if (s1 == s0) return;

    struct TileIt { uint32_t pos, npg, b1, end_b1; bool valid; };
    auto tile_after = [&](const TileIt &t) {
        TileIt n = t;
        n.pos = t.pos + t.npg;
        n.valid = t.valid && n.pos < s1;
        if (n.valid && n.pos == t.end_b1) {
            n.b1 = l2_digit_of(page_base1, nb1, n.pos);
            n.end_b1 = page_base1[n.b1 + 1] < s1 ? page_base1[n.b1 + 1] : s1;
        }
        n.npg = n.valid ? (n.end_b1 - n.pos < L2_TILE_PAGES ? n.end_b1 - n.pos : L2_TILE_PAGES) : 0u;
        return n;
    };
    uint4 nx[PPT];
    uint2 nh[ElemFmt<IN>::HI ? PPT : 1];
    uint32_t nxvalid[PPT];
    PageEntry ent[PPT];
    auto load_entries = [&](const TileIt &t) {
#pragma unroll
        for (int q = 0; q < PPT; q++) {
            const uint32_t pi = (uint32_t)q * NWAVES + (uint32_t)wave;
            ent[q].page = 0; ent[q].nelems = 0;
            if (pi < t.npg) ent[q] = list1[t.pos + pi];
        }
    };
    auto load_pages = [&]() {
#pragma unroll
        for (int q = 0; q < PPT; q++) {
            const uint32_t first = (uint32_t)lane * (uint32_t)EP, ne = ent[q].nelems;
            nxvalid[q] = ne > first ? (ne - first < (uint32_t)EP ? ne - first : (uint32_t)EP) : 0u;
            nx[q] = make_uint4(0, 0, 0, 0);
            if (ElemFmt<IN>::HI) nh[q] = make_uint2(0, 0);
            if (ne) {
                const uint8_t *pg = pages1 + (size_t)ent[q].page * IN_PAGE_BYTES;
                nx[q] = reinterpret_cast<const uint4 *>(pg)[lane];
                if (ElemFmt<IN>::HI) nh[q] = reinterpret_cast<const uint2 *>(pg + SC_HI_OFFSET)[lane];
            }
        }
    };
    constexpr bool ENTRIES_AHEAD = ElemFmt<IN>::HI;
    TileIt A;
    A.pos = s0; A.b1 = l2_digit_of(page_base1, nb1, s0); A.valid = true;
    A.end_b1 = page_base1[A.b1 + 1] < s1 ? page_base1[A.b1 + 1] : s1;
    A.npg = A.end_b1 - A.pos < L2_TILE_PAGES ? A.end_b1 - A.pos : L2_TILE_PAGES;
    uint32_t cur_b1 = A.b1;
    load_entries(A);
    load_pages();
    TileIt B = tile_after(A);
    if (ENTRIES_AHEAD) load_entries(B);
    TileIt Cn = tile_after(B);
    SC_STAMP_INIT;
    SC_WG_CLOCK(1, 0);
    while (true) {
        uint32_t pend = 0;
#pragma unroll
        for (int q = 0; q < PPT; q++) pend |= ((1u << nxvalid[q]) - 1u) << (q * EP);
        auto make = [&](int idx, uint32_t &woff_u, uint32_t &el_u) {
            const int q = idx / EP, i = idx % EP;
            const uint32_t lo[4] = {nx[q].x, nx[q].y, nx[q].z, nx[q].w};
            uint32_t e;
            if (ElemFmt<IN>::HI) {
                const uint32_t hb[2] = {nh[q].x, nh[q].y};
                e = ((lo[i >> 1] >> (16 * (i & 1))) & 0xFFFFu) | (((hb[i >> 2] >> (8 * (i & 3))) & 0xFFu) << 16);
            } else {
                e = lo[i & 3];
            }
            woff_u = __builtin_amdgcn_ubfe(e, (uint32_t)ring_shift, (uint32_t)ring_bits) << 2;
            el_u = bfi(keep, e, e >> ring_bits);
        };
        SC_STAMP(0);
        if (A.b1 != cur_b1) {
            if (my_ring < (uint32_t)RINGS) ring_drain(R, out, own, my_ring, (cur_b1 << ring_bits) | my_ring, ctr);
            cur_b1 = A.b1;
            __syncthreads();
        }
        const TileIt Dn = tile_after(Cn);
        rings_place<ELEM, RINGS, C, NID, NID>(R, out, own, my_ring, (cur_b1 << ring_bits) | my_ring, ctr, desc, make, pend, round, [&]() {
            if (!B.valid) return;
            if (ENTRIES_AHEAD) {
                load_pages();
#pragma unroll
                for (int q = 0; q < PPT; q++) asm volatile("" : "+v"(nxvalid[q]));
                asm volatile("" ::: "memory");
                load_entries(Cn);
            }
            else { load_entries(B); load_pages(); }
        }, SC_STAMP_FN);
        if (!B.valid) break;
        A = B;
        B = Cn;
        Cn = Dn;
    }
    if (my_ring < (uint32_t)RINGS) ring_drain(R, out, own, my_ring, (cur_b1 << ring_bits) | my_ring, ctr);
    SC_STAMP(5);
    SC_STAMP_END_AT(16);
    SC_WG_CLOCK(1, 1);
}

constexpr int PAGES_LDS_NB = 4096;
constexpr int PAGES_THREADS = 1024;

__device__ __forceinline__ uint32_t pages_window_start(const uint32_t *__restrict__ tag, uint32_t p0, uint32_t p1, uint32_t *s_min)
{
    if (threadIdx.x == 0) *s_min = 0xFFFFFFFFu;
    __syncthreads();
    uint32_t m = 0xFFFFFFFFu;
    for (uint32_t p = p0 + threadIdx.x; p < p1; p += PAGES_THREADS) {
        const uint32_t t = tag[p];
        if (t != SC_NO_PAGE && (t & ((1u << SC_TAG_SHIFT) - 1u))) { const uint32_t b = t >> SC_TAG_SHIFT; m = b < m ? b : m; }
    }
#pragma unroll
    for (int o = 32; o > 0; o >>= 1) { const uint32_t x = (uint32_t)__shfl_xor((int)m, o, 64); m = x < m ? x : m; }
    if ((threadIdx.x & 63) == 0 && m != 0xFFFFFFFFu) atomicMin(s_min, m);
    __syncthreads();
    return *s_min;
}

__global__ void __launch_bounds__(PAGES_THREADS)
pages_count_kernel(const uint32_t *__restrict__ tag, uint32_t npages, uint32_t nb, uint32_t *__restrict__ bkt_pages, uint32_t *__restrict__ bkt_elems,
                   unsigned long long *__restrict__ stat , uint32_t line_elems)
{
    __shared__ uint32_t cp[PAGES_LDS_NB], ce[PAGES_LDS_NB];
    __shared__ uint32_t s_min, s_pages, s_lines;
    const uint32_t chunk = (npages + gridDim.x - 1) / gridDim.x, p0 = blockIdx.x * chunk, p1 = p0 + chunk < npages ? p0 + chunk : npages;
    const uint32_t w0 = pages_window_start(tag, p0, p1, &s_min);
    if (w0 == 0xFFFFFFFFu) return;
    for (uint32_t b = threadIdx.x; b < (uint32_t)PAGES_LDS_NB; b += PAGES_THREADS) { cp[b] = 0; ce[b] = 0; }
    if (threadIdx.x == 0) { s_pages = 0; s_lines = 0; }
    __syncthreads();
    uint32_t my_pages = 0, my_lines = 0;
    for (uint32_t p = p0 + threadIdx.x; p < p1; p += PAGES_THREADS) {
        const uint32_t t = tag[p];
        if (t == SC_NO_PAGE) continue;
        const uint32_t b = t >> SC_TAG_SHIFT, n = t & ((1u << SC_TAG_SHIFT) - 1u);
        if (n == 0) continue;
        my_pages++; my_lines += (n + line_elems - 1u) / line_elems;
        if (b - w0 < (uint32_t)PAGES_LDS_NB) { atomicAdd(&cp[b - w0], 1u); atomicAdd(&ce[b - w0], n); }
        else { atomicAdd(&bkt_pages[b], 1u); atomicAdd(&bkt_elems[b], n); }
    }
    if (stat) {
#pragma unroll
        for (int o = 32; o > 0; o >>= 1) { my_pages += (uint32_t)__shfl_xor((int)my_pages, o, 64); my_lines += (uint32_t)__shfl_xor((int)my_lines, o, 64); }
        if ((threadIdx.x & 63) == 0 && my_pages) { atomicAdd(&s_pages, my_pages); atomicAdd(&s_lines, my_lines); }
    }
    __syncthreads();
    for (uint32_t b = threadIdx.x; b < (uint32_t)PAGES_LDS_NB && w0 + b < nb; b += PAGES_THREADS)
        if (cp[b]) { atomicAdd(&bkt_pages[w0 + b], cp[b]); atomicAdd(&bkt_elems[w0 + b], ce[b]); }
    if (stat && threadIdx.x == 0 && s_pages) {
        __hip_atomic_fetch_add(&stat[0], (unsigned long long)s_pages, __ATOMIC_RELAXED, __HIP_MEMORY_SCOPE_AGENT);
        __hip_atomic_fetch_add(&stat[1], (unsigned long long)s_lines, __ATOMIC_RELAXED, __HIP_MEMORY_SCOPE_AGENT);
    }
}

__global__ void __launch_bounds__(1024)
pages_scan_kernel(const uint32_t *__restrict__ bkt_pages, const uint32_t *__restrict__ bkt_elems, uint32_t nb,
                  uint32_t *__restrict__ page_base, uint32_t *__restrict__ slice_base, uint32_t slice_pages, DevCounters *ctr)
{
    __shared__ uint32_t wsum[1024 / 64];
    __shared__ unsigned long long s_tot;
    const uint32_t j = threadIdx.x;
    if (j == 0) s_tot = 0;
    const uint32_t per = (nb + 1023u) / 1024u;
    const uint32_t lo = j * per < nb ? j * per : nb, hi = lo + per < nb ? lo + per : nb;
    uint32_t sum = 0, ssum = 0;
    unsigned long long el = 0;
    for (uint32_t i = lo; i < hi; i++) { const uint32_t v = bkt_pages[i]; sum += v; ssum += (v + slice_pages - 1) / slice_pages; el += bkt_elems[i]; }
    uint32_t tot, stot;
    uint32_t run = block_excl_scan<1024>(sum, wsum, &tot);
    uint32_t srun = block_excl_scan<1024>(ssum, wsum, &stot);
    for (uint32_t i = lo; i < hi; i++) {
        const uint32_t v = bkt_pages[i];
        page_base[i] = run; slice_base[i] = srun;
        run += v; srun += (v + slice_pages - 1) / slice_pages;
    }
    el = wave_sum(el);
    if ((j & 63) == 0 && el) atomicAdd(&s_tot, el);
    __syncthreads();
    if (j == 0) {
        page_base[nb] = tot; slice_base[nb] = stot;
        if (ctr && s_tot) __hip_atomic_fetch_add(&ctr->total_kmers, s_tot, __ATOMIC_RELAXED, __HIP_MEMORY_SCOPE_AGENT);
    }
}

__global__ void __launch_bounds__(PAGES_THREADS)
pages_place_kernel(const uint32_t *__restrict__ tag, uint32_t npages, uint32_t nb, uint32_t *__restrict__ bkt_pages, const uint32_t *__restrict__ page_base,
                   PageEntry *__restrict__ list)
{
    __shared__ uint32_t cur[PAGES_LDS_NB];
    __shared__ uint32_t s_min;
    const uint32_t chunk = (npages + gridDim.x - 1) / gridDim.x, p0 = blockIdx.x * chunk, p1 = p0 + chunk < npages ? p0 + chunk : npages;
    const uint32_t w0 = pages_window_start(tag, p0, p1, &s_min);
    if (w0 == 0xFFFFFFFFu) return;
    for (uint32_t b = threadIdx.x; b < (uint32_t)PAGES_LDS_NB; b += PAGES_THREADS) cur[b] = 0;
    __syncthreads();
    for (uint32_t p = p0 + threadIdx.x; p < p1; p += PAGES_THREADS) {
        const uint32_t t = tag[p];
        if (t != SC_NO_PAGE && (t & ((1u << SC_TAG_SHIFT) - 1u)) && (t >> SC_TAG_SHIFT) - w0 < (uint32_t)PAGES_LDS_NB) atomicAdd(&cur[(t >> SC_TAG_SHIFT) - w0], 1u);
    }
    __syncthreads();
    for (uint32_t b = threadIdx.x; b < (uint32_t)PAGES_LDS_NB && w0 + b < nb; b += PAGES_THREADS) {
        const uint32_t c = cur[b];
        if (c) cur[b] = page_base[w0 + b] + atomicSub(&bkt_pages[w0 + b], c) - c;
    }
    __syncthreads();
    for (uint32_t p = p0 + threadIdx.x; p < p1; p += PAGES_THREADS) {
        const uint32_t t = tag[p];
        if (t == SC_NO_PAGE) continue;
        const uint32_t b = t >> SC_TAG_SHIFT, n = t & ((1u << SC_TAG_SHIFT) - 1u);
        if (n == 0) continue;
        const uint32_t pos = b - w0 < (uint32_t)PAGES_LDS_NB ? atomicAdd(&cur[b - w0], 1u) : page_base[b] + atomicSub(&bkt_pages[b], 1u) - 1u;
        list[pos].page = p;
        list[pos].nelems = n;
    }
}

constexpr uint32_t WRAP_MAX = 4096;
template <uint32_t CAP> struct WrapListT { uint32_t n; uint32_t e[CAP]; };
using WrapList = WrapListT<WRAP_MAX>;

__device__ __forceinline__ void wrap_note(WrapList &wl, uint32_t bin, uint32_t negative)
{
    const uint32_t s = atomicAdd(&wl.n, 1u);
    if (s < WRAP_MAX) wl.e[s] = bin | (negative << 16);
}

__device__ __noinline__ void hist_wrapped16(uint32_t *hist, uint32_t v, uint32_t old, WrapList &wl)
{
    if (v >> 15) {
        if ((old >> 16) == 0xFFFFu) wrap_note(wl, v, 0u);
    } else if ((old & 0xFFFFu) == 0xFFFFu) {
        wrap_note(wl, v, 0u);
        if ((old >> 16) == 0xFFFFu) wrap_note(wl, v | 0x8000u, 0u);
        const uint32_t old2 = atomicSub(&hist[v & 0x7FFFu], 0x10000u);
        if ((old2 >> 16) == 0u) wrap_note(wl, v | 0x8000u, 1u);
    }
}

__device__ __forceinline__ void hist_add_page_chunk16(uint32_t *hist, const uint4 &x, uint32_t nvalid, WrapList &wl)
{
    if (nvalid >= 8u) {
        const uint32_t w[4] = {x.x, x.y, x.z, x.w};
        uint32_t sh[8], old[8];
#pragma unroll
        for (uint32_t e = 0; e < 8; e++) {
            const uint32_t byte = (e & 1u) ? (w[e >> 1] >> 14) & 0x1FFFCu : (w[e >> 1] << 2) & 0x1FFFCu;
            sh[e] = (e & 1u) ? (w[e >> 1] >> 27) & 16u : (w[e >> 1] >> 11) & 16u;
            old[e] = atomicAdd(reinterpret_cast<uint32_t *>(reinterpret_cast<uint8_t *>(hist) + byte), 1u << sh[e]);
        }
        uint32_t m = 0u;
#pragma unroll
        for (uint32_t e = 0; e < 8; e++) {
            const uint32_t fld = __builtin_amdgcn_ubfe(old[e], sh[e], 16u);
            m = fld > m ? fld : m;
        }
        if (m == 0xFFFFu) {
#pragma unroll
            for (uint32_t e = 0; e < 8; e++) hist_wrapped16(hist, (e & 1u) ? w[e >> 1] >> 16 : w[e >> 1] & 0xFFFFu, old[e], wl);
        }
        return;
    }
    unsigned long long lo = ((unsigned long long)x.y << 32) | x.x, hi = ((unsigned long long)x.w << 32) | x.z;
#pragma unroll 1
    for (uint32_t e = 0; e < nvalid; e++) {
        const uint32_t v = (uint32_t)((e < 4u ? lo : hi) >> (16u * (e & 3u))) & 0xFFFFu;
        const uint32_t old = atomicAdd(&hist[v & 0x7FFFu], 1u << ((v >> 11) & 16u));
        hist_wrapped16(hist, v, old, wl);
    }
}

__device__ __forceinline__ void hist_add_page_chunk(uint32_t *hist, const uint4 &x, uint32_t nvalid)
{
    if (nvalid >= 8) { hist_add8(hist, x); return; }
    unsigned long long lo = ((unsigned long long)x.y << 32) | x.x, hi = ((unsigned long long)x.w << 32) | x.z;
    for (uint32_t e = 0; e < nvalid; e++) {
        const unsigned long long w = e < 4 ? lo : hi;
        atomicAdd(&hist[(uint32_t)(w >> (16 * (e & 3))) & 0xFFFFu], 1u);
    }
}

template <bool HALF = false>
__device__ __forceinline__ uint32_t hist_flush_runs(const uint32_t *hist_words, unsigned long long *__restrict__ dst, int lo_bits, int hi_shift, bool only_writer,
                                                int tid, bool dst_is_zero, uint64_t half_stride = 0 )
{
    const uint32_t lom = (1u << lo_bits) - 1u;
    constexpr int PAIRS = BUCKET_BINS / 2, NH = HALF ? 2 : 1, FLIGHT = HALF ? 8 : 4, U = FLIGHT / NH;
    auto pair = [&](int p, int h) -> uint2 {
        uint2 w = reinterpret_cast<const uint2 *>(hist_words)[p];
        if (HALF) { w.x = (w.x >> (16 * h)) & 0xFFFFu; w.y = (w.y >> (16 * h)) & 0xFFFFu; }
        return w;
    };
    auto at = [&](int p, int h) -> ulonglong2 * {
        const uint32_t i = 2u * (uint32_t)p;
        return reinterpret_cast<ulonglong2 *>(dst + (HALF && h ? half_stride : 0ull) + (((uint64_t)(i >> lo_bits)) << hi_shift) + (i & lom));
    };
    uint32_t moved = 0;
    if (only_writer && dst_is_zero) {
        for (int base = 0; base < PAIRS; base += U * P2_THREADS) {
#pragma unroll
            for (int u = 0; u < U; u++) {
#pragma unroll
                for (int h = 0; h < NH; h++) {
                    const uint2 c = pair(base + u * P2_THREADS + tid, h);
                    *at(base + u * P2_THREADS + tid, h) = make_ulonglong2((unsigned long long)c.x, (unsigned long long)c.y);
                }
            }
        }
        moved = 16u * (uint32_t)(NH * PAIRS / P2_THREADS);
    } else if (only_writer) {
        for (int base = 0; base < PAIRS; base += U * P2_THREADS) {
            uint2 c[U][NH];
            ulonglong2 v[U][NH];
#pragma unroll
            for (int u = 0; u < U; u++)
#pragma unroll
                for (int h = 0; h < NH; h++) c[u][h] = pair(base + u * P2_THREADS + tid, h);
#pragma unroll
            for (int u = 0; u < U; u++)
#pragma unroll
                for (int h = 0; h < NH; h++) v[u][h] = (c[u][h].x | c[u][h].y) ? *at(base + u * P2_THREADS + tid, h) : make_ulonglong2(0ull, 0ull);
#pragma unroll
            for (int u = 0; u < U; u++)
#pragma unroll
                for (int h = 0; h < NH; h++)
                    if (c[u][h].x | c[u][h].y) {
                        v[u][h].x += c[u][h].x; v[u][h].y += c[u][h].y;
                        *at(base + u * P2_THREADS + tid, h) = v[u][h];
                        moved += 32u;
                    }
        }
    } else {
        for (int p = tid; p < PAIRS; p += P2_THREADS) {
#pragma unroll
            for (int h = 0; h < NH; h++) {
                const uint2 c = pair(p, h);
                unsigned long long *const a = reinterpret_cast<unsigned long long *>(at(p, h));
                if (c.x) { __hip_atomic_fetch_add(a, (unsigned long long)c.x, __ATOMIC_RELAXED, __HIP_MEMORY_SCOPE_AGENT); moved += 16u; }
                if (c.y) { __hip_atomic_fetch_add(a + 1, (unsigned long long)c.y, __ATOMIC_RELAXED, __HIP_MEMORY_SCOPE_AGENT); moved += 16u; }
            }
        }
    }
    return moved;
}

template <bool BINS16>
__global__ void __launch_bounds__(P2_THREADS)
page_hist_kernel(const uint8_t *__restrict__ pages, const PageEntry *__restrict__ list, const uint32_t *__restrict__ page_base,
                 const uint32_t *__restrict__ slice_base, uint32_t nbuckets, unsigned long long *__restrict__ table,
                 int lo_bits ,
                 int hi_shift ,
                 int table_is_zero , DevCounters *ctr)
{
    constexpr int CH = SC_PAGE_BYTES / 16;
    constexpr int PPS = P2_THREADS / CH;
    __shared__ uint32_t hist[BUCKET_BINS];
    __shared__ WrapListT<BINS16 ? WRAP_MAX : 1u> wl;
    __shared__ unsigned long long s_moved;
    const int tid = threadIdx.x;
    uint32_t b, s, nslices;
    if (!p2_locate(slice_base, nbuckets, blockIdx.x, &b, &s, &nslices)) return;
    const uint32_t P0 = page_base[b], n = page_base[b + 1] - P0;
    const uint32_t g0 = P0 + (uint32_t)((uint64_t)n * s / nslices), g1 = P0 + (uint32_t)((uint64_t)n * (s + 1) / nslices);
    if (g1 == g0) return;
    const uint32_t ch = (uint32_t)tid & (CH - 1), first = ch * 8u;
    for (int i = tid; i < BUCKET_BINS; i += P2_THREADS) hist[i] = 0;
    if (tid == 0) s_moved = 0;
    if (BINS16 && tid == 0) wl.n = 0;
    __syncthreads();
    uint32_t i = g0 + (uint32_t)tid / CH;
    for (; i + 3u * PPS < g1; i += 4u * PPS) {
        PageEntry e[4];
        uint4 x[4];
#pragma unroll
        for (int u = 0; u < 4; u++) e[u] = list[i + u * PPS];
#pragma unroll
        for (int u = 0; u < 4; u++) x[u] = load_once16(reinterpret_cast<const uint4 *>(pages + (size_t)e[u].page * SC_PAGE_BYTES) + ch);
#pragma unroll
        for (int u = 0; u < 4; u++) {
            const uint32_t nv = e[u].nelems > first ? e[u].nelems - first : 0u;
            if constexpr (BINS16) hist_add_page_chunk16(hist, x[u], nv, wl); else hist_add_page_chunk(hist, x[u], nv);
        }
    }
    for (; i < g1; i += PPS) {
        const PageEntry e = list[i];
        const uint4 x = load_once16(reinterpret_cast<const uint4 *>(pages + (size_t)e.page * SC_PAGE_BYTES) + ch);
        const uint32_t nv = e.nelems > first ? e.nelems - first : 0u;
        if constexpr (BINS16) hist_add_page_chunk16(hist, x, nv, wl); else hist_add_page_chunk(hist, x, nv);
    }
    __syncthreads();
    unsigned long long *const dst = table + ((uint64_t)b << lo_bits);
    const bool zero = table_is_zero != 0 && ctr->table_dirty == 0;
    auto account = [&](uint32_t moved) {
        unsigned long long m = wave_sum((unsigned long long)moved);
        if ((tid & 63) == 0 && m) atomicAdd(&s_moved, m);
        __syncthreads();
        if (tid == 0 && s_moved) __hip_atomic_fetch_add(&ctr->table_bytes, s_moved, __ATOMIC_RELAXED, __HIP_MEMORY_SCOPE_AGENT);
    };
    if constexpr (!BINS16) { account(hist_flush_runs(hist, dst, lo_bits, hi_shift, nslices == 1, tid, zero)); return; }
    account(hist_flush_runs<true>(hist, dst, lo_bits, hi_shift, nslices == 1, tid, zero, (uint64_t)(1u << (BIN_BITS - lo_bits)) << hi_shift));
    if (wl.n == 0) return;
    __threadfence();
    __syncthreads();
    const uint32_t nw = wl.n < WRAP_MAX ? wl.n : WRAP_MAX;
    if (tid == 0 && wl.n > WRAP_MAX) __hip_atomic_fetch_add(&ctr->internal_err, 1ull, __ATOMIC_RELAXED, __HIP_MEMORY_SCOPE_AGENT);
    const uint32_t lom = (1u << lo_bits) - 1u;
    for (uint32_t q = (uint32_t)tid; q < nw; q += P2_THREADS) {
        const uint32_t v = wl.e[q] & 0xFFFFu;
        const unsigned long long d = (wl.e[q] >> 16) ? 0ull - 65536ull : 65536ull;
        __hip_atomic_fetch_add(dst + ((uint64_t)(v >> lo_bits) << hi_shift) + (v & lom), d, __ATOMIC_RELAXED, __HIP_MEMORY_SCOPE_AGENT);
    }
}

struct ScatterState {
    uint8_t *d_pages = nullptr; size_t pages_cap = 0, page_bytes = 0;
    uint32_t *d_tag = nullptr;
    PageEntry *d_list = nullptr;
    uint32_t *d_bkt = nullptr;
    size_t bkt_cap = 0;
    int grid = 0;
    int lo_bits = 0;
    int contig_pages = 1;
    int wide_lines = 1;
};

inline void scatter_free(ScatterState &st)
{
    if (st.d_pages) (void)hipFree(st.d_pages);
    if (st.d_tag) (void)hipFree(st.d_tag);
    if (st.d_list) (void)hipFree(st.d_list);
    if (st.d_bkt) (void)hipFree(st.d_bkt);
    st = ScatterState();
}

inline uint64_t scatter_max_tiles(uint32_t Gmax, uint32_t tile_pos = SC_TILE_POS)
{
    const uint64_t a = (1ull << 31) / tile_pos, b = 4095ull * Gmax;
    return a < b ? a : b;
}

inline uint32_t scatter_wg_pages(uint32_t tiles_per_wg, int rings, uint32_t page_elems, uint32_t tile_pos = SC_TILE_POS, uint32_t extra_elems = 0)
{
    return (uint32_t)(((uint64_t)tiles_per_wg * tile_pos + extra_elems + page_elems - 1) / page_elems) + (uint32_t)rings + 1u;
}

inline uint32_t scatter_extra_elems(uint32_t tiles_per_wg, uint32_t tile_pos, int n_expand)
{
    if (!n_expand) return 0u;
    const uint64_t half = (uint64_t)tiles_per_wg * tile_pos / 2, floor_ = 16u * 1024u + 1024u * 64u + 2048u;
    const uint64_t v = half > floor_ ? half : floor_;
    return (uint32_t)(v < 0x7FFFFFFFull ? v : 0x7FFFFFFFull);
}

inline int scatter_reserve(ScatterState &st, hipStream_t stream, size_t npages, size_t nb, size_t page_bytes = SC_PAGE_BYTES)
{
    if (st.pages_cap < npages || st.page_bytes != page_bytes) {
        if (st.d_pages) { if (hipStreamSynchronize(stream) != hipSuccess) return 1; (void)hipFree(st.d_pages); (void)hipFree(st.d_tag); (void)hipFree(st.d_list); st.d_pages = nullptr; st.d_tag = nullptr; st.d_list = nullptr; st.pages_cap = 0; }
        if (hipMalloc((void **)&st.d_pages, npages * page_bytes) != hipSuccess ||
            hipMalloc((void **)&st.d_tag, npages * sizeof(uint32_t)) != hipSuccess ||
            hipMalloc((void **)&st.d_list, npages * sizeof(PageEntry)) != hipSuccess) {
            (void)hipGetLastError();
            if (st.d_pages) (void)hipFree(st.d_pages);
            if (st.d_tag) (void)hipFree(st.d_tag);
            if (st.d_list) (void)hipFree(st.d_list);
            st.d_pages = nullptr; st.d_tag = nullptr; st.d_list = nullptr;
            return 2;
        }
        st.pages_cap = npages;
        st.page_bytes = page_bytes;
    }
    if (st.bkt_cap < nb) {
        if (st.d_bkt) { if (hipStreamSynchronize(stream) != hipSuccess) return 1; (void)hipFree(st.d_bkt); st.d_bkt = nullptr; st.bkt_cap = 0; }
        if (hipMalloc((void **)&st.d_bkt, (4 * nb + 2) * sizeof(uint32_t)) != hipSuccess) { (void)hipGetLastError(); return 2; }
        st.bkt_cap = nb;
    }
    return 0;
}

constexpr int SC1_THREADS = 1024, SC1_RINGS = 1024, SC1_GRID = 256, SC1_K = 13;
constexpr int SC1_TILE_POS = (SC1_THREADS - 1) * 16;

struct ScGeom {
    bool big; bool wide ;
    int binb, nb, rings, sub_log2, nb_bits, lo_bits, hi_shift;
    uint32_t tile_stride, tile_pos, Gmax;
    uint64_t ntiles_all, max_tiles;
};
struct ScLaunch { uint32_t nt, G, npages; };

inline ScGeom scatter_geometry(const ScatterState &st, size_t nbytes, int k, uint32_t grid_default = 0)
{
    ScGeom g;
    g.big = k == SC1_K;
    g.binb = g.big ? 16 : BIN_BITS;
    g.nb = 1 << (2 * k - g.binb);
    g.rings = g.big ? SC1_RINGS : 512;
    g.lo_bits = st.lo_bits ? st.lo_bits : SC_LO_BITS_ONE_LEVEL;
    g.wide = !g.big && st.wide_lines != 0;
    g.tile_stride = (g.big || g.wide) ? (uint32_t)SC1_THREADS - 1u : (uint32_t)SC_TILE_STRIDE;
    g.tile_pos = g.tile_stride * 16u;
    g.sub_log2 = 0; g.nb_bits = 2 * k - g.binb;
    while ((g.nb << g.sub_log2) < g.rings) g.sub_log2++;
    g.hi_shift = g.lo_bits + g.nb_bits;
    g.ntiles_all = ((nbytes + 15) / 16 + g.tile_stride - 1) / g.tile_stride;
    g.Gmax = st.grid > 0 ? (uint32_t)st.grid : (grid_default ? grid_default : (uint32_t)((g.big || g.wide) ? SC1_GRID : SC_GRID));
    g.max_tiles = scatter_max_tiles(g.Gmax, g.tile_pos);
    return g;
}

inline int scatter_reserve_for(ScatterState &st, hipStream_t stream, const ScGeom &g, int n_expand)
{
    const uint64_t nt = g.ntiles_all < g.max_tiles ? g.ntiles_all : g.max_tiles;
    const uint32_t G = (uint32_t)(nt < g.Gmax ? nt : g.Gmax);
    const uint32_t tpw = (uint32_t)((nt + G - 1) / G);
    const uint32_t wg_pages = scatter_wg_pages(tpw, g.rings, 512, g.tile_pos, scatter_extra_elems(tpw, g.tile_pos, n_expand));
    const int rc = scatter_reserve(st, stream, (size_t)G * wg_pages, (size_t)g.nb);
    if (rc == 2) { partition_error_ref() = "scratch allocation failed"; return 2; }
    if (rc) { partition_error_ref() = "stream error"; return 1; }
    return 0;
}

inline int scatter_stage1(ScatterState &st, hipStream_t stream, const ScGeom &g, uint64_t t0, const uint8_t *d_bases, size_t nbytes, const RecStarts &rs, int k,
                          int canonical, int n_expand, unsigned long long *d_table, DevCounters *d_ctr, ProfHook &prof, ScLaunch *L)
{
    constexpr int C = 64;
    const int nb = g.nb, lo_bits = g.lo_bits, nb_bits = g.nb_bits, sub_log2 = g.sub_log2;
    const uint32_t nt = (uint32_t)((g.ntiles_all - t0) < g.max_tiles ? (g.ntiles_all - t0) : g.max_tiles);
    const uint32_t G = nt < g.Gmax ? nt : g.Gmax;
    ScOut out;
    out.pages = st.d_pages; out.tag = st.d_tag;
    out.extra_elems = scatter_extra_elems((nt + G - 1) / G, g.tile_pos, n_expand);
    out.wg_pages = scatter_wg_pages((nt + G - 1) / G, g.rings, 512, g.tile_pos, out.extra_elems);
    out.wg_range = nullptr; out.contig = (uint32_t)st.contig_pages; out.wg_base = 0; out.grid = 0;
    const uint32_t npages = G * out.wg_pages;
    L->nt = nt; L->G = G; L->npages = npages;
    if (hipMemsetAsync(st.d_tag, 0xFF, (size_t)npages * sizeof(uint32_t), stream) != hipSuccess ||
        hipMemsetAsync(st.d_bkt, 0, 2 * (size_t)nb * sizeof(uint32_t), stream) != hipSuccess) { partition_error_ref() = "memset failed"; return 1; }
    prof.begin_on(KDB_KERNEL_SCATTER, stream);
#define KDB_LAUNCH_SC1(EL, CC, E, CN, KK, RG, TH, RAG)                                                                                     \
    hipLaunchKernelGGL((scatter_bases_kernel<uint32_t, EL, RG, CC, 16, E, CN, KK, TH, RAG>), dim3(G), dim3(TH), 0, stream, d_bases,       \
                       (uint64_t)nbytes, (uint32_t)t0, nt, k, lo_bits, nb_bits, sub_log2, out, d_table, d_ctr, rs)
#define KDB_LAUNCH_SC(EL, CC, E, CN, KK, RG, TH) do { KDB_LAUNCH_SC1(EL, CC, E, CN, KK, RG, TH, false); KDB_LAUNCH_SC1(EL, CC, E, CN, KK, RG, TH, true); } while (0)
#define KDB_LAUNCH_SC_MODES(EL, CC, KK, RG, TH)                                                                                            \
    do {                                                                                                                                   \
        if (n_expand) { if (canonical) KDB_LAUNCH_SC(EL, CC, true, true, KK, RG, TH); else KDB_LAUNCH_SC(EL, CC, true, false, KK, RG, TH); }   \
        else          { if (canonical) KDB_LAUNCH_SC(EL, CC, false, true, KK, RG, TH); else KDB_LAUNCH_SC(EL, CC, false, false, KK, RG, TH); } \
    } while (0)
    if (g.big) {
        if (lo_bits == SC_LO_BITS_ONE_LEVEL) KDB_LAUNCH_SC_MODES(uint16_t, C, SC1_K, SC1_RINGS, SC1_THREADS);
        else                                 KDB_LAUNCH_SC_MODES(uint16_t, C, 0, SC1_RINGS, SC1_THREADS);
    } else if (g.wide) {
        const bool compiled = lo_bits == SC_LO_BITS_ONE_LEVEL && (nb << sub_log2) == 512;
        if (compiled && k == 12)      KDB_LAUNCH_SC_MODES(u16w, 128, 12, 512, SC1_THREADS);
        else if (compiled && k == 11) KDB_LAUNCH_SC_MODES(u16w, 128, 11, 512, SC1_THREADS);
        else if (compiled && k == 10) KDB_LAUNCH_SC_MODES(u16w, 128, 10, 512, SC1_THREADS);
        else if (compiled && k == 9)  KDB_LAUNCH_SC_MODES(u16w, 128, 9, 512, SC1_THREADS);
        else                          KDB_LAUNCH_SC_MODES(u16w, 128, 0, 512, SC1_THREADS);
    } else if (k == 12 && lo_bits == SC_LO_BITS_ONE_LEVEL && sub_log2 == 0) {
        KDB_LAUNCH_SC_MODES(uint16_t, C, 12, 512, SC_THREADS);
    } else {
        KDB_LAUNCH_SC_MODES(uint16_t, C, 0, 512, SC_THREADS);
    }
#undef KDB_LAUNCH_SC_MODES
#undef KDB_LAUNCH_SC
#undef KDB_LAUNCH_SC1
    prof.end();
    if (hipGetLastError() != hipSuccess) { partition_error_ref() = "paged scatter failed to launch"; return 1; }
    return 0;
}

inline int scatter_stage2(ScatterState &st, hipStream_t stream, const ScGeom &g, const ScLaunch &L, unsigned long long *d_table, DevCounters *d_ctr, ProfHook &prof)
{
    const int nb = g.nb;
    const uint32_t npages = L.npages;
    uint32_t *const bkt_pages = st.d_bkt, *const bkt_elems = st.d_bkt + nb, *const page_base = st.d_bkt + 2 * nb, *const slice_base = st.d_bkt + 3 * nb + 1;
    prof.begin_on(KDB_KERNEL_PAGE_SORT, stream);
    const uint32_t pgrid = (npages + 4095u) / 4096u < 256u ? (npages + 4095u) / 4096u : 256u;
    const uint32_t target = 512u;
    const uint32_t est_pages = (uint32_t)(((uint64_t)L.nt * g.tile_pos * 2) / SC_PAGE_BYTES) + 1u;
    uint32_t slice_pages = (est_pages + target - 1) / target;
    if (slice_pages < 128u) slice_pages = 128u;
    hipLaunchKernelGGL(pages_count_kernel, dim3(pgrid), dim3(PAGES_THREADS), 0, stream, (const uint32_t *)st.d_tag, npages, (uint32_t)nb, bkt_pages, bkt_elems,
                       &d_ctr->pages_bases, 32u);
    hipLaunchKernelGGL(pages_scan_kernel, dim3(1), dim3(1024), 0, stream, (const uint32_t *)bkt_pages, (const uint32_t *)bkt_elems, (uint32_t)nb,
                       page_base, slice_base, slice_pages, d_ctr);
    hipLaunchKernelGGL(pages_place_kernel, dim3(pgrid), dim3(PAGES_THREADS), 0, stream, (const uint32_t *)st.d_tag, npages, (uint32_t)nb, bkt_pages,
                       (const uint32_t *)page_base, st.d_list);
    prof.end();
    prof.begin_on(KDB_KERNEL_PAGE_HIST, stream);
    const uint32_t p2_grid = npages / slice_pages + (uint32_t)nb + 1u;
    if (g.big)
        hipLaunchKernelGGL(page_hist_kernel<true>, dim3(p2_grid), dim3(P2_THREADS), 0, stream, (const uint8_t *)st.d_pages, (const PageEntry *)st.d_list,
                           (const uint32_t *)page_base, (const uint32_t *)slice_base, (uint32_t)nb, d_table, g.lo_bits, g.hi_shift, 0, d_ctr);
    else
        hipLaunchKernelGGL(page_hist_kernel<false>, dim3(p2_grid), dim3(P2_THREADS), 0, stream, (const uint8_t *)st.d_pages, (const PageEntry *)st.d_list,
                           (const uint32_t *)page_base, (const uint32_t *)slice_base, (uint32_t)nb, d_table, g.lo_bits, g.hi_shift, 0, d_ctr);
    prof.end();
    if (hipGetLastError() != hipSuccess) { partition_error_ref() = "paged scatter failed to launch"; return 1; }
    return 0;
}

inline int scatter_count(ScatterState &st, hipStream_t stream, const uint8_t *d_bases, size_t nbytes, const RecStarts &rs, int k, int canonical, int n_expand,
                         unsigned long long *d_table, DevCounters *d_ctr, ProfHook &prof)
{
    const ScGeom g = scatter_geometry(st, nbytes, k);
    { const int rc = scatter_reserve_for(st, stream, g, n_expand); if (rc) return rc; }
    for (uint64_t t0 = 0; t0 < g.ntiles_all; t0 += g.max_tiles) {
        ScLaunch L;
        if (scatter_stage1(st, stream, g, t0, d_bases, nbytes, rs, k, canonical, n_expand, d_table, d_ctr, prof, &L)) return 1;
        if (scatter_stage2(st, stream, g, L, d_table, d_ctr, prof)) return 1;
    }
    return 0;
}

struct OverlapState {
    ScatterState sc[2];
    unsigned long long *side[2] = {nullptr, nullptr};
    size_t side_cap = 0;
    hipEvent_t scattered[2] = {nullptr, nullptr}, hist_done[2] = {nullptr, nullptr};
    bool used[2] = {false, false};
    int next = 0, last = -1;
    uint32_t grid = 0;
};

inline void overlap_free(OverlapState &ov)
{
    for (int j = 0; j < 2; j++) {
        scatter_free(ov.sc[j]);
        if (ov.side[j]) (void)hipFree(ov.side[j]);
        if (ov.scattered[j]) (void)hipEventDestroy(ov.scattered[j]);
        if (ov.hist_done[j]) (void)hipEventDestroy(ov.hist_done[j]);
    }
    ov = OverlapState();
}

inline int scatter_count_overlapped(OverlapState &ov, hipStream_t s_scatter, hipStream_t s_hist, const uint8_t *d_bases, size_t nbytes, const RecStarts &rs, int k,
                                    int canonical, unsigned long long *d_table, DevCounters *d_ctr, ProfHook &prof)
{
    const int j = ov.next;
    ScatterState &st = ov.sc[j];
    st.grid = ov.sc[0].grid; st.lo_bits = ov.sc[0].lo_bits; st.contig_pages = ov.sc[0].contig_pages; st.wide_lines = ov.sc[0].wide_lines;
    const ScGeom g = scatter_geometry(st, nbytes, k, ov.grid);
    if (g.ntiles_all > g.max_tiles) return 3;
    for (int q = 0; q < 2; q++) {
        if (!ov.scattered[q] && hipEventCreateWithFlags(&ov.scattered[q], hipEventDisableTiming) != hipSuccess) { partition_error_ref() = "event creation failed"; return 1; }
        if (!ov.hist_done[q] && hipEventCreateWithFlags(&ov.hist_done[q], hipEventDisableTiming) != hipSuccess) { partition_error_ref() = "event creation failed"; return 1; }
    }
    if (ov.used[j] && hipStreamWaitEvent(s_scatter, ov.hist_done[j], 0) != hipSuccess) { partition_error_ref() = "stream wait failed"; return 1; }
    {
        const uint64_t nt = g.ntiles_all;
        const uint32_t G = (uint32_t)(nt < g.Gmax ? nt : g.Gmax);
        const uint32_t tpw = (uint32_t)((nt + G - 1) / G);
        const size_t need = (size_t)G * scatter_wg_pages(tpw, g.rings, 512, g.tile_pos, 0);
        if ((st.pages_cap < need || st.bkt_cap < (size_t)g.nb) && ov.used[j] && hipEventSynchronize(ov.hist_done[j]) != hipSuccess) { partition_error_ref() = "stream error"; return 1; }
        const int rc = scatter_reserve_for(st, s_scatter, g, 0);
        if (rc) return rc;
        const size_t side_need = (size_t)g.Gmax * SC_HOT + 65536;
        if (ov.side_cap < side_need) {
            for (int q = 0; q < 2; q++) {
                if (ov.side[q]) { if (ov.used[q] && hipEventSynchronize(ov.hist_done[q]) != hipSuccess) { partition_error_ref() = "stream error"; return 1; } (void)hipFree(ov.side[q]); ov.side[q] = nullptr; }
                if (hipMalloc((void **)&ov.side[q], (2 + 2 * side_need) * sizeof(unsigned long long)) != hipSuccess) { (void)hipGetLastError(); ov.side_cap = 0; partition_error_ref() = "scratch allocation failed"; return 2; }
            }
            ov.side_cap = side_need;
        }
    }
    hipLaunchKernelGGL(hot_side_kernel, dim3(1), dim3(1), 0, s_scatter, d_ctr, ov.side[j], (unsigned long long)ov.side_cap);
    ScLaunch L;
    if (scatter_stage1(st, s_scatter, g, 0, d_bases, nbytes, rs, k, canonical, 0, d_table, d_ctr, prof, &L)) return 1;
    hipLaunchKernelGGL(hot_side_kernel, dim3(1), dim3(1), 0, s_scatter, d_ctr, (unsigned long long *)nullptr, 0ull);
    if (hipEventRecord(ov.scattered[j], s_scatter) != hipSuccess || hipStreamWaitEvent(s_hist, ov.scattered[j], 0) != hipSuccess) { partition_error_ref() = "stream error"; return 1; }
    if (scatter_stage2(st, s_hist, g, L, d_table, d_ctr, prof)) return 1;
    hipLaunchKernelGGL(apply_hot_kernel, dim3(8), dim3(256), 0, s_hist, (const unsigned long long *)ov.side[j], d_table);
    if (hipGetLastError() != hipSuccess || hipEventRecord(ov.hist_done[j], s_hist) != hipSuccess) { partition_error_ref() = "paged scatter failed to launch"; return 1; }
    ov.used[j] = true;
    ov.last = j;
    ov.next = j ^ 1;
    return 0;
}

constexpr int PAGED_PENDING_MAX = 64;
constexpr int L1_RINGS = 256, L1_C = 64, L1_ROUND = 8;
constexpr int L1W_RINGS = 512, L1W_C = 32, L1W_ROUND = 8;

struct TwoLevelPaged {
    ScatterState l1;
    uint8_t *d_pages2 = nullptr; size_t cap2 = 0;
    uint32_t *d_tag2 = nullptr;
    PageEntry *d_list2 = nullptr;
    uint32_t *d_bkt2 = nullptr; size_t nb2_cap = 0;
    uint32_t *d_wg_range = nullptr;
    size_t used2 = 0;
    static constexpr int PROBES = 8;
    uint32_t *d_cursor = nullptr;
    uint32_t *h_probe = nullptr;
    hipEvent_t ev_probe[PROBES] = {nullptr, nullptr, nullptr, nullptr, nullptr, nullptr, nullptr, nullptr};
    size_t probe_bound[PROBES] = {0};
    bool probe_live[PROBES] = {false};
    int probe_next = 0;
    size_t slack = 0;
    size_t tags_dirty = 0;
    int pending = 0;
    int k_pending = 0;
    int defer = 1;
    size_t budget_bytes = 0;
    int l1_one_round = 1;
    int l1_wide = 1;
    int l2_wide = 1;
    int l1k = 1;
    size_t reserve_bytes = 0;
    size_t free_at_sizing = 0;
    bool table_is_zero = false;
    bool filled_up = false;
    bool grow_failed = false;
    uint64_t reallocs = 0;
    int grow = 1;
    uint64_t full_flushes = 0;
    int first_batches = 8;
    uint64_t flushes = 0, flushed_batches = 0;
};

inline void twolevel_paged_free(TwoLevelPaged &tp)
{
    scatter_free(tp.l1);
    if (tp.d_pages2) (void)hipFree(tp.d_pages2);
    if (tp.d_tag2) (void)hipFree(tp.d_tag2);
    if (tp.d_list2) (void)hipFree(tp.d_list2);
    if (tp.d_bkt2) (void)hipFree(tp.d_bkt2);
    if (tp.d_wg_range) (void)hipFree(tp.d_wg_range);
    if (tp.d_cursor) (void)hipFree(tp.d_cursor);
    if (tp.h_probe) (void)hipHostFree(tp.h_probe);
    for (int i = 0; i < TwoLevelPaged::PROBES; i++) if (tp.ev_probe[i]) (void)hipEventDestroy(tp.ev_probe[i]);
    const int defer = tp.defer, grow = tp.grow, first_batches = tp.first_batches, l1k = tp.l1k, l2_wide = tp.l2_wide, l1_wide = tp.l1_wide, l1_one_round = tp.l1_one_round;
    const size_t budget = tp.budget_bytes, reserve = tp.reserve_bytes;
    const ScatterState keep = tp.l1;
    tp = TwoLevelPaged();
    tp.defer = defer; tp.budget_bytes = budget; tp.reserve_bytes = reserve; tp.grow = grow; tp.first_batches = first_batches; tp.l1k = l1k; tp.l2_wide = l2_wide; tp.l1_wide = l1_wide; tp.l1_one_round = l1_one_round;
    tp.l1.grid = keep.grid; tp.l1.lo_bits = keep.lo_bits; tp.l1.contig_pages = keep.contig_pages;
}

inline void twolevel_paged_drop(TwoLevelPaged &tp)
{
    if (tp.used2 - tp.slack > tp.tags_dirty) tp.tags_dirty = tp.used2 - tp.slack;
    tp.used2 = 0; tp.slack = 0; tp.pending = 0;
    for (int i = 0; i < TwoLevelPaged::PROBES; i++) tp.probe_live[i] = false;
}

inline void twolevel_paged_poll(TwoLevelPaged &tp)
{
    for (int i = 0; i < TwoLevelPaged::PROBES; i++) {
        if (!tp.probe_live[i] || hipEventQuery(tp.ev_probe[i]) != hipSuccess) continue;
        tp.probe_live[i] = false;
        const size_t actual = tp.h_probe[i], bound = tp.probe_bound[i];
        if (bound >= actual && bound - actual > tp.slack) tp.slack = bound - actual;
    }
    (void)hipGetLastError();
}

inline void paged_bits(int k, int *d1_bits, int *bin_bits)
{
    *bin_bits = k == 17 ? 16 : 15;
    *d1_bits = 2 * k - *bin_bits - 9;
}

inline int twolevel_paged_flush(TwoLevelPaged &tp, hipStream_t stream, unsigned long long *d_table, DevCounters *d_ctr, ProfHook &prof)
{
    if (tp.pending == 0) return 0;
    const int k = tp.k_pending;
    int d1, binb;
    paged_bits(k, &d1, &binb);
    const uint32_t nb2 = 1u << (d1 + 9);
    const int table_is_zero = tp.table_is_zero ? 1 : 0;
    tp.table_is_zero = false;
    uint32_t *const bkt_pages = tp.d_bkt2, *const bkt_elems = tp.d_bkt2 + nb2, *const page_base = tp.d_bkt2 + 2 * (size_t)nb2,
             *const slice_base = tp.d_bkt2 + 3 * (size_t)nb2 + 1;
    twolevel_paged_poll(tp);
    const uint32_t npages = (uint32_t)(tp.used2 - tp.slack);
    if (npages == 0) {
        tp.flushes++; tp.flushed_batches += (uint64_t)tp.pending;
        twolevel_paged_drop(tp);
        return 0;
    }
    if (hipMemsetAsync(tp.d_bkt2, 0, 2 * (size_t)nb2 * sizeof(uint32_t), stream) != hipSuccess) { partition_error_ref() = "memset failed"; return 1; }
    prof.begin(KDB_KERNEL_PAGE_SORT);
    const uint32_t pgrid = (npages + 4095u) / 4096u < 2048u ? (npages + 4095u) / 4096u : 2048u;
    uint32_t slice_pages = (npages + 2047u) / 2048u;
    if (slice_pages < 128u) slice_pages = 128u;
    hipLaunchKernelGGL(pages_count_kernel, dim3(pgrid), dim3(PAGES_THREADS), 0, stream, (const uint32_t *)tp.d_tag2, npages, nb2, bkt_pages, bkt_elems,
                       &d_ctr->pages_ids, 32u);
    hipLaunchKernelGGL(pages_scan_kernel, dim3(1), dim3(1024), 0, stream, (const uint32_t *)bkt_pages, (const uint32_t *)bkt_elems, nb2, page_base, slice_base,
                       slice_pages, (DevCounters *)nullptr);
    hipLaunchKernelGGL(pages_place_kernel, dim3(pgrid), dim3(PAGES_THREADS), 0, stream, (const uint32_t *)tp.d_tag2, npages, nb2, bkt_pages,
                       (const uint32_t *)page_base, tp.d_list2);
    prof.end();
    prof.begin(KDB_KERNEL_PAGE_HIST);
    const uint32_t p2_grid = npages / slice_pages + nb2 + 1u;
    const int lo_bits = tp.l1.lo_bits ? tp.l1.lo_bits : SC_LO_BITS_TWO_LEVEL, hi_shift = lo_bits + d1 + 9;
    if (binb == 16)
        hipLaunchKernelGGL(page_hist_kernel<true>, dim3(p2_grid), dim3(P2_THREADS), 0, stream, (const uint8_t *)tp.d_pages2, (const PageEntry *)tp.d_list2,
                           (const uint32_t *)page_base, (const uint32_t *)slice_base, nb2, d_table, lo_bits, hi_shift, table_is_zero, d_ctr);
    else
        hipLaunchKernelGGL(page_hist_kernel<false>, dim3(p2_grid), dim3(P2_THREADS), 0, stream, (const uint8_t *)tp.d_pages2, (const PageEntry *)tp.d_list2,
                           (const uint32_t *)page_base, (const uint32_t *)slice_base, nb2, d_table, lo_bits, hi_shift, table_is_zero, d_ctr);
    prof.end();
    tp.flushes++; tp.flushed_batches += (uint64_t)tp.pending;
    twolevel_paged_drop(tp);
    if (hipGetLastError() != hipSuccess) { partition_error_ref() = "histogram pass over the page arena failed to launch"; return 1; }
    return 0;
}

inline int twolevel_paged_count(TwoLevelPaged &tp, hipStream_t stream, const uint8_t *d_bases, size_t nbytes, const RecStarts &rs,
                                size_t max_windows ,
                                int k, int canonical, int n_expand, unsigned long long *d_table, DevCounters *d_ctr, ProfHook &prof)
{
    int d1, binb;
    paged_bits(k, &d1, &binb);
    const int nb1 = 1 << d1;
    const uint32_t nb2 = 1u << (d1 + 9);
    const bool wide = k == 17;
    const int lo_bits = tp.l1.lo_bits ? tp.l1.lo_bits : SC_LO_BITS_TWO_LEVEL;
    const bool one_round1 = tp.l1_one_round != 0 && tp.l1_wide != 0 && !wide && (1 << d1) <= 128;
    const int rings1 = wide ? L1W_RINGS : (one_round1 ? 128 : L1_RINGS);
    const uint32_t l1_page_elems = wide ? 256u : 512u;
    const size_t l1_page_bytes = wide ? (size_t)ElemFmt<uint32_t>::PAGE_BYTES : (size_t)ElemFmt<u24>::PAGE_BYTES;
    int sub_log2 = 0;
    while ((nb1 << sub_log2) < rings1) sub_log2++;
    const bool wide1 = tp.l1_wide != 0;
    const uint32_t tile_stride1 = wide1 ? (uint32_t)SC1_THREADS - 1u : (uint32_t)SC_TILE_STRIDE, tile_pos1 = tile_stride1 * 16u;
    const uint64_t ntiles_all = ((nbytes + 15) / 16 + tile_stride1 - 1) / tile_stride1;
    const uint32_t Gmax = tp.l1.grid > 0 ? (uint32_t)tp.l1.grid : (uint32_t)(wide1 ? SC1_GRID : SC_GRID);
    const uint64_t max_tiles = scatter_max_tiles(Gmax, tile_pos1);
    if (tp.pending && tp.k_pending != k) { if (twolevel_paged_flush(tp, stream, d_table, d_ctr, prof)) return 1; }
    {
        const uint64_t nt = ntiles_all < max_tiles ? ntiles_all : max_tiles;
        const uint32_t G = (uint32_t)(nt < Gmax ? nt : Gmax);
        const uint32_t tpw = (uint32_t)((nt + G - 1) / G);
        const int rc = scatter_reserve(tp.l1, stream, (size_t)G * scatter_wg_pages(tpw, rings1, l1_page_elems, tile_pos1, scatter_extra_elems(tpw, tile_pos1, n_expand)),
                                       (size_t)nb1, l1_page_bytes);
        if (rc == 2) { partition_error_ref() = "scratch allocation failed"; return 2; }
        if (rc) { partition_error_ref() = "stream error"; return 1; }
    }
    if (!tp.d_wg_range && hipMalloc((void **)&tp.d_wg_range, (SC_GRID + 1) * sizeof(uint32_t)) != hipSuccess) { (void)hipGetLastError(); partition_error_ref() = "scratch allocation failed"; return 2; }
    if (!tp.d_cursor) {
        if (hipMalloc((void **)&tp.d_cursor, sizeof(uint32_t)) != hipSuccess ||
            hipHostMalloc((void **)&tp.h_probe, TwoLevelPaged::PROBES * sizeof(uint32_t), hipHostMallocDefault) != hipSuccess) { (void)hipGetLastError(); partition_error_ref() = "scratch allocation failed"; return 2; }
        for (int i = 0; i < TwoLevelPaged::PROBES; i++)
            if (hipEventCreateWithFlags(&tp.ev_probe[i], hipEventDisableTiming) != hipSuccess) { partition_error_ref() = "event creation failed"; return 1; }
    }
    if (tp.nb2_cap < nb2) {
        if (tp.d_bkt2) { if (hipStreamSynchronize(stream) != hipSuccess) return 1; (void)hipFree(tp.d_bkt2); tp.d_bkt2 = nullptr; tp.nb2_cap = 0; }
        if (hipMalloc((void **)&tp.d_bkt2, (4 * (size_t)nb2 + 2) * sizeof(uint32_t)) != hipSuccess) { (void)hipGetLastError(); partition_error_ref() = "scratch allocation failed"; return 2; }
        tp.nb2_cap = nb2;
    }
    uint32_t *const bkt_pages1 = tp.l1.d_bkt, *const bkt_elems1 = tp.l1.d_bkt + nb1, *const page_base1 = tp.l1.d_bkt + 2 * nb1, *const slice_base1 = tp.l1.d_bkt + 3 * nb1 + 1;
    for (uint64_t t0 = 0; t0 < ntiles_all; t0 += max_tiles) {
        const uint32_t nt = (uint32_t)((ntiles_all - t0) < max_tiles ? (ntiles_all - t0) : max_tiles);
        const uint32_t G = nt < Gmax ? nt : Gmax;
        ScOut out1;
        out1.pages = tp.l1.d_pages; out1.tag = tp.l1.d_tag; out1.wg_range = nullptr; out1.contig = (uint32_t)tp.l1.contig_pages; out1.wg_base = 0; out1.grid = 0;
        out1.extra_elems = scatter_extra_elems((nt + G - 1) / G, tile_pos1, n_expand);
        out1.wg_pages = scatter_wg_pages((nt + G - 1) / G, rings1, l1_page_elems, tile_pos1, out1.extra_elems);
        const uint32_t npages1 = G * out1.wg_pages;
        const bool wide2 = tp.l2_wide != 0;
        const uint32_t G2 = wide2 ? (uint32_t)SC1_GRID : (uint32_t)SC_GRID;
        const size_t pos = (size_t)nt * tile_pos1, elems = (pos < max_windows ? pos : max_windows) + (size_t)G * out1.extra_elems;
        const size_t need2 = (elems + 511) / 512 + (size_t)G * (size_t)rings1 + 2 * (size_t)G2 + 512 * ((size_t)nb1 + G2) + 16;
        if (tp.budget_bytes == 0) {
            size_t free_b = 0, total_b = 0;
            (void)hipMemGetInfo(&free_b, &total_b);
            tp.free_at_sizing = free_b;
            tp.budget_bytes = free_b / 100 * 85;
            if (tp.reserve_bytes && tp.budget_bytes + tp.reserve_bytes > free_b) tp.budget_bytes = free_b > tp.reserve_bytes ? free_b - tp.reserve_bytes : 0;
            if (tp.budget_bytes > (192ull << 30)) tp.budget_bytes = 192ull << 30;
            if (tp.budget_bytes < (1ull << 30)) tp.budget_bytes = 1ull << 30;
        }
        size_t budget_pages = tp.defer ? tp.budget_bytes / SC_PAGE_BYTES : 0;
        if (tp.grow_failed && budget_pages > tp.cap2) budget_pages = tp.cap2;
        if (budget_pages < need2) budget_pages = need2;
        bool may_grow = tp.filled_up && tp.cap2 + tp.cap2 / 4 <= budget_pages && tp.grow != 0;
        if (may_grow && tp.grow == 1) {
            const size_t next_cap = 2 * tp.cap2 < budget_pages ? 2 * tp.cap2 : budget_pages;
            const double alloc_ms = (double)next_cap * (double)SC_PAGE_BYTES / (double)(1ull << 30) * 46.0;
            const double sweep_ms = (double)(1ull << (2 * k)) * 16.0 / 5.5e9;
            may_grow = (double)tp.full_flushes * sweep_ms * 0.5 >= alloc_ms;
        }
        twolevel_paged_poll(tp);
        if (tp.used2 - tp.slack + need2 > tp.cap2 || tp.cap2 == 0 || may_grow) {
            if (tp.pending) { if (twolevel_paged_flush(tp, stream, d_table, d_ctr, prof)) return 1; }
            tp.filled_up = false;
            size_t want_cap = tp.cap2 == 0 ? (size_t)tp.first_batches * need2 : 2 * tp.cap2;
            if (want_cap > budget_pages) want_cap = budget_pages;
            if (want_cap < need2) want_cap = need2;
            if (tp.cap2 < need2 || (may_grow && tp.cap2 < want_cap) || tp.cap2 == 0) {
                if (hipStreamSynchronize(stream) != hipSuccess) return 1;
                const size_t old_cap = tp.cap2;
                if (tp.d_pages2) { (void)hipFree(tp.d_pages2); (void)hipFree(tp.d_tag2); (void)hipFree(tp.d_list2); tp.d_pages2 = nullptr; tp.d_tag2 = nullptr; tp.d_list2 = nullptr; tp.cap2 = 0; }
                const size_t tries[3] = {want_cap, old_cap >= need2 ? old_cap : need2, need2};
                for (int attempt = 0; attempt < 3 && !tp.d_pages2; attempt++) {
                    const size_t cap = tries[attempt];
                    if (attempt && cap == tries[attempt - 1]) continue;
                    if (hipMalloc((void **)&tp.d_pages2, cap * (size_t)SC_PAGE_BYTES) == hipSuccess &&
                        hipMalloc((void **)&tp.d_tag2, cap * sizeof(uint32_t)) == hipSuccess &&
                        hipMalloc((void **)&tp.d_list2, cap * sizeof(PageEntry)) == hipSuccess) { tp.cap2 = cap; tp.tags_dirty = cap; if (attempt) tp.grow_failed = true; break; }
                    (void)hipGetLastError();
                    if (tp.d_pages2) (void)hipFree(tp.d_pages2);
                    if (tp.d_tag2) (void)hipFree(tp.d_tag2);
                    if (tp.d_list2) (void)hipFree(tp.d_list2);
                    tp.d_pages2 = nullptr; tp.d_tag2 = nullptr; tp.d_list2 = nullptr;
                }
                tp.reallocs++;
                tp.full_flushes = 0;
                if (!tp.d_pages2) { partition_error_ref() = "scratch allocation failed"; return t0 == 0 ? 2 : 1; }
            }
        }
        if (tp.pending == 0) {
            if (tp.tags_dirty > tp.cap2) tp.tags_dirty = tp.cap2;
            if (hipMemsetAsync(tp.d_cursor, 0, sizeof(uint32_t), stream) != hipSuccess ||
                (tp.tags_dirty && hipMemsetAsync(tp.d_tag2, 0xFF, tp.tags_dirty * sizeof(uint32_t), stream) != hipSuccess)) { partition_error_ref() = "memset failed"; return 1; }
            tp.tags_dirty = 0;
        }
        if (hipMemsetAsync(tp.l1.d_tag, 0xFF, (size_t)npages1 * sizeof(uint32_t), stream) != hipSuccess ||
            hipMemsetAsync(tp.l1.d_bkt, 0, 2 * (size_t)nb1 * sizeof(uint32_t), stream) != hipSuccess) { partition_error_ref() = "memset failed"; return 1; }
        prof.begin(KDB_KERNEL_SCATTER);
#define KDB_LAUNCH_L1K(ID, EL, RG, CC, RD, TH, E, CN, RAG, KK)                                                                                 \
    hipLaunchKernelGGL((scatter_bases_kernel<ID, EL, RG, CC, RD, E, CN, KK, TH, RAG>), dim3(G), dim3(TH), 0, stream, d_bases,                 \
                       (uint64_t)nbytes, (uint32_t)t0, nt, k, lo_bits + 9, d1, sub_log2, out1, d_table, d_ctr, rs)
#define KDB_LAUNCH_L1R(ID, EL, RG, CC, RD, TH, E, CN, RAG) KDB_LAUNCH_L1K(ID, EL, RG, CC, RD, TH, E, CN, RAG, 0)
#define KDB_LAUNCH_L1(ID, EL, RG, CC, RD, TH, E, CN) do { KDB_LAUNCH_L1R(ID, EL, RG, CC, RD, TH, E, CN, false); KDB_LAUNCH_L1R(ID, EL, RG, CC, RD, TH, E, CN, true); } while (0)
#define KDB_LAUNCH_L1_MODES(ID, EL, RG, CC, RD, TH)                                                                                            \
    do {                                                                                                                                       \
        if (n_expand) { if (canonical) KDB_LAUNCH_L1(ID, EL, RG, CC, RD, TH, true, true); else KDB_LAUNCH_L1(ID, EL, RG, CC, RD, TH, true, false); }     \
        else          { if (canonical) KDB_LAUNCH_L1(ID, EL, RG, CC, RD, TH, false, true); else KDB_LAUNCH_L1(ID, EL, RG, CC, RD, TH, false, false); }   \
    } while (0)
        const bool compiled15 = !wide && k == 15 && !n_expand && canonical && lo_bits == SC_LO_BITS_TWO_LEVEL && tp.l1k;
        const bool compiled17 = wide && wide1 && !n_expand && canonical && lo_bits == SC_LO_BITS_TWO_LEVEL && tp.l1k;
        const bool compiled14 = !wide && k == 14 && !n_expand && canonical && lo_bits == SC_LO_BITS_TWO_LEVEL && tp.l1k;
        const bool compiled16 = !wide && k == 16 && !n_expand && canonical && lo_bits == SC_LO_BITS_TWO_LEVEL && tp.l1k;
        if (one_round1) {
            if (compiled15) {
                KDB_LAUNCH_L1K(uint32_t, u24w, 128, 256, 16, SC1_THREADS, false, true, false, 15);
                KDB_LAUNCH_L1K(uint32_t, u24w, 128, 256, 16, SC1_THREADS, false, true, true, 15);
            } else if (compiled14) {
                KDB_LAUNCH_L1K(uint32_t, u24w, 128, 256, 16, SC1_THREADS, false, true, false, 14);
                KDB_LAUNCH_L1K(uint32_t, u24w, 128, 256, 16, SC1_THREADS, false, true, true, 14);
            } else KDB_LAUNCH_L1_MODES(uint32_t, u24w, 128, 256, 16, SC1_THREADS);
        } else if (wide1 && compiled16) {
            KDB_LAUNCH_L1K(uint32_t, u24w, L1_RINGS, 2 * L1_C, L1_ROUND, SC1_THREADS, false, true, false, 16);
            KDB_LAUNCH_L1K(uint32_t, u24w, L1_RINGS, 2 * L1_C, L1_ROUND, SC1_THREADS, false, true, true, 16);
        } else if (wide1) {
            if (compiled15) {
                KDB_LAUNCH_L1K(uint32_t, u24w, L1_RINGS, 2 * L1_C, L1_ROUND, SC1_THREADS, false, true, false, 15);
                KDB_LAUNCH_L1K(uint32_t, u24w, L1_RINGS, 2 * L1_C, L1_ROUND, SC1_THREADS, false, true, true, 15);
            } else if (!wide) KDB_LAUNCH_L1_MODES(uint32_t, u24w, L1_RINGS, 2 * L1_C, L1_ROUND, SC1_THREADS);
            else if (compiled17) {
                KDB_LAUNCH_L1K(uint64_t, u32w, L1W_RINGS, 2 * L1W_C, L1W_ROUND, SC1_THREADS, false, true, false, 17);
                KDB_LAUNCH_L1K(uint64_t, u32w, L1W_RINGS, 2 * L1W_C, L1W_ROUND, SC1_THREADS, false, true, true, 17);
            }
            else KDB_LAUNCH_L1_MODES(uint64_t, u32w, L1W_RINGS, 2 * L1W_C, L1W_ROUND, SC1_THREADS);
        } else if (compiled15) {
            KDB_LAUNCH_L1K(uint32_t, u24, L1_RINGS, L1_C, L1_ROUND, SC_THREADS, false, true, false, 15);
            KDB_LAUNCH_L1K(uint32_t, u24, L1_RINGS, L1_C, L1_ROUND, SC_THREADS, false, true, true, 15);
        } else if (!wide) KDB_LAUNCH_L1_MODES(uint32_t, u24, L1_RINGS, L1_C, L1_ROUND, SC_THREADS);
        else KDB_LAUNCH_L1_MODES(uint64_t, uint32_t, L1W_RINGS, L1W_C, L1W_ROUND, SC_THREADS);
#undef KDB_LAUNCH_L1_MODES
#undef KDB_LAUNCH_L1
#undef KDB_LAUNCH_L1R
#undef KDB_LAUNCH_L1K
        prof.end();
        prof.begin(KDB_KERNEL_PAGE_SORT);
        const uint32_t pgrid = (npages1 + 4095u) / 4096u < 256u ? (npages1 + 4095u) / 4096u : 256u;
        hipLaunchKernelGGL(pages_count_kernel, dim3(pgrid), dim3(PAGES_THREADS), 0, stream, (const uint32_t *)tp.l1.d_tag, npages1, (uint32_t)nb1, bkt_pages1, bkt_elems1,
                           &d_ctr->pages_bases, wide ? 16u : 32u);
        hipLaunchKernelGGL(pages_scan_kernel, dim3(1), dim3(1024), 0, stream, (const uint32_t *)bkt_pages1, (const uint32_t *)bkt_elems1, (uint32_t)nb1, page_base1,
                           slice_base1, 1u << 20, d_ctr);
        hipLaunchKernelGGL(pages_place_kernel, dim3(pgrid), dim3(PAGES_THREADS), 0, stream, (const uint32_t *)tp.l1.d_tag, npages1, (uint32_t)nb1, bkt_pages1,
                           (const uint32_t *)page_base1, tp.l1.d_list);
        hipLaunchKernelGGL(l2_plan_kernel, dim3(1), dim3(1024), 0, stream, (const uint32_t *)page_base1, (uint32_t)nb1, G2, 512u, l1_page_elems, tp.d_wg_range, tp.d_cursor,
                           (uint32_t)tp.cap2, d_ctr);
        prof.end();
        tp.used2 += need2;
        {
            const int pi = tp.probe_next;
            if (!tp.probe_live[pi] && hipMemcpyAsync(&tp.h_probe[pi], tp.d_cursor, sizeof(uint32_t), hipMemcpyDeviceToHost, stream) == hipSuccess &&
                hipEventRecord(tp.ev_probe[pi], stream) == hipSuccess) {
                tp.probe_live[pi] = true; tp.probe_bound[pi] = tp.used2;
                tp.probe_next = (pi + 1) % TwoLevelPaged::PROBES;
            }
        }
        ScOut out2;
        out2.pages = tp.d_pages2; out2.tag = tp.d_tag2; out2.wg_pages = 0; out2.wg_range = tp.d_wg_range; out2.contig = 0; out2.wg_base = 0; out2.grid = 0; out2.extra_elems = 0;
        prof.begin(KDB_KERNEL_SCATTER_L2);
#define KDB_LAUNCH_L2(IN, EL, CC, FX, TH)                                                                                                       \
    hipLaunchKernelGGL((scatter_ids_kernel<IN, EL, 512, CC, FX, TH>), dim3(G2), dim3(TH), 0, stream, (const uint8_t *)tp.l1.d_pages,            \
                       (const PageEntry *)tp.l1.d_list, (const uint32_t *)page_base1, (uint32_t)nb1, lo_bits, 9, out2, d_ctr)
        const bool fixed2 = lo_bits == SC_LO_BITS_TWO_LEVEL && tp.l1k;
        if (wide2) {
            if (wide && fixed2) KDB_LAUNCH_L2(uint32_t, u16w, 128, true, SC1_THREADS);
            else if (wide) KDB_LAUNCH_L2(uint32_t, u16w, 128, false, SC1_THREADS);
            else if (fixed2) KDB_LAUNCH_L2(u24, u16w, 128, true, SC1_THREADS);
            else KDB_LAUNCH_L2(u24, u16w, 128, false, SC1_THREADS);
        } else {
            if (wide) KDB_LAUNCH_L2(uint32_t, uint16_t, 64, false, SC_THREADS);
            else if (fixed2) KDB_LAUNCH_L2(u24, uint16_t, 64, true, SC_THREADS);
            else KDB_LAUNCH_L2(u24, uint16_t, 64, false, SC_THREADS);
        }
#undef KDB_LAUNCH_L2
        prof.end();
        tp.pending++;
        tp.k_pending = k;
        if (hipGetLastError() != hipSuccess) { partition_error_ref() = "two-level paged scatter failed to launch"; return 1; }
        if (tp.defer && tp.used2 - tp.slack + need2 > tp.cap2) { tp.filled_up = true; tp.full_flushes++; }
        if (!tp.defer || tp.pending >= PAGED_PENDING_MAX || tp.used2 - tp.slack + need2 > tp.cap2) { if (twolevel_paged_flush(tp, stream, d_table, d_ctr, prof)) return 1; }
    }
    return 0;
}

}
```

Measured before the change: 717.2 billion.

## Fold page counting and scan into scatter kernel, fuse suspect resolution into placement

The one-level scatter kernel now counts each workgroup's pages per bucket itself. The last block to finish, found through an atomic ticket, computes the page and slice prefix bases. This removes the separate pages_count and pages_scan launches and the per-batch memsets of the tag and bucket arrays. Placement now scans only the pages each workgroup used. An extra block in that placement launch runs the suspect-resolution work, which drops one more launch in N-drop mode. The lens kernel reads offsets in aligned 16-byte pairs with a shuffle. In exchange the code depends on cross-block fences, counters that must be cleared on reset, and a grid limit.

Measured after the change: 727.9 billion (median of 6 runs). About the same (+1.5%).

```diff
diff --git a/kmerdb_amd/csrc/kdb_engine.hip b/kmerdb_amd/csrc/kdb_engine.hip
--- a/kmerdb_amd/csrc/kdb_engine.hip
+++ b/kmerdb_amd/csrc/kdb_engine.hip
@@ -356,6 +356,7 @@
     if (nreads > 0xFFFFFFF0ull) return fail(KDB_ERR_ARG, "batch of %zu records: at most 2^32 - 16 per submit", nreads);
     e->bytes_in += nbytes;
     const kdb::RecStarts rs{d_offs, e->d_first_rec, (uint32_t)nreads, first_is_continuation ? 1u : 0u};
+    bool suspects_judged = false;
     int algo = (int)e->algo;
     if (algo == 0 || algo == 3) algo = 2;
     if (no_first_rec && algo == 2) { algo = 1; e->oom_fallbacks++; e->tp.table_is_zero = false; }
@@ -380,7 +381,9 @@
             }
             if (rc == 3) {
                 { const int jrc = overlap_join(e); if (jrc != KDB_OK) return jrc; }
-                rc = kdb::scatter_count(e->sc, e->s_compute, d_bases, nbytes, rs, e->k, e->canonical, ex, e->d_table, e->d_ctr, hook);
+                const kdb::SuspectsJob sj{(const uint8_t *)d_bases, (uint64_t)nbytes, d_offs, (uint64_t)nreads, e->k};
+                rc = kdb::scatter_count(e->sc, e->s_compute, d_bases, nbytes, rs, e->k, e->canonical, ex, e->d_table, e->d_ctr, hook, ex ? nullptr : &sj);
+                suspects_judged = rc == 0 && !ex;
             }
         }
         else {
@@ -410,7 +413,7 @@
         ProfScope ps(e, KDB_KERNEL_COUNT);
         hipLaunchKernelGGL(kdb::expand_worklist_kernel, dim3(1024), dim3(256), 0, e->s_compute, e->d_table, e->d_ctr, e->k, e->canonical);
     }
-    if (e->n_mode == KDB_N_DROP) {
+    if (e->n_mode == KDB_N_DROP && !suspects_judged) {
         ProfScope ps(e, KDB_KERNEL_MARK);
         hipLaunchKernelGGL(kdb::resolve_suspects_kernel, dim3(4), dim3(256), 0, e->s_compute, (const uint8_t *)d_bases, (uint64_t)nbytes, d_offs, (uint64_t)nreads,
                            e->k, e->d_ctr);
@@ -652,6 +655,8 @@
     e->folded_files = e->folded_total = 0;
     e->tp.table_is_zero = e->owns_table && !e->table_escaped;
     HIP_TRY(hipMemsetAsync(e->d_ctr, 0, sizeof(kdb::DevCounters), e->s_compute));
+    if (kdb::scatter_clear(e->sc, e->s_compute) || kdb::scatter_clear(e->ov.sc[0], e->s_compute) || kdb::scatter_clear(e->ov.sc[1], e->s_compute))
+        return fail(KDB_ERR_HIP, "clearing the page sort's counters failed");
     unsigned long long wl[2] = {0, 0}, sus[2] = {0, 0};
     if (e->n_mode == KDB_N_EXPAND) {
         if (!e->d_worklist) HIP_TRY(hipMalloc((void **)&e->d_worklist, e->worklist_cap * sizeof(unsigned long long)));
diff --git a/kmerdb_amd/csrc/kdb_kernels.hip.h b/kmerdb_amd/csrc/kdb_kernels.hip.h
--- a/kmerdb_amd/csrc/kdb_kernels.hip.h
+++ b/kmerdb_amd/csrc/kdb_kernels.hip.h
@@ -50,27 +50,55 @@
     __shared__ unsigned long long s_len[4], s_neg[4], s_short[4], s_bad[4];
     unsigned long long len = 0, neg = 0, nshort = 0, nbadl = 0;
     const uint64_t stride = (uint64_t)gridDim.x * blockDim.x;
-    for (uint64_t rb = (uint64_t)blockIdx.x * blockDim.x + threadIdx.x; rb < nreads; rb += 4 * stride) {
-        uint64_t sv[4], ev[4];
-#pragma unroll
-        for (int u = 0; u < 4; u++) {
-            const uint64_t r = rb + (uint64_t)u * stride;
-            sv[u] = r < nreads ? offs[r] : 0ull;
-            ev[u] = r < nreads ? offs[r + 1] : 0ull;
-        }
-#pragma unroll
-        for (int u = 0; u < 4; u++) {
-            const uint64_t r = rb + (uint64_t)u * stride, s = sv[u], e = ev[u];
-            if (r >= nreads) break;
-            unsigned long long l = e - s;
-            neg = neg > ~l ? neg : ~l;
-            if (!(r == 0 && first_is_continuation)) nshort += (l < (uint64_t)k) ? 1 : 0;
-            nbadl += (r == 0 && s != 0) + (r == nreads - 1 && e != nbytes) + (e < s || e > nbytes);
-            if (r == 0 && first_is_continuation) l = ~0ull;
-            len = len > l ? len : l;
-            if (first_rec && e > s) {
-                const uint64_t e2 = e < nbytes ? e : nbytes;
-                for (uint64_t b = (s + ((1ull << FIRST_REC_SHIFT) - 1ull)) >> FIRST_REC_SHIFT; (b << FIRST_REC_SHIFT) < e2; b++) first_rec[b] = (uint32_t)r;
+    auto record = [&](uint64_t r, uint64_t s, uint64_t e) {
+        unsigned long long l = e - s;
+        neg = neg > ~l ? neg : ~l;
+        if (!(r == 0 && first_is_continuation)) nshort += (l < (uint64_t)k) ? 1 : 0;
+        nbadl += (r == 0 && s != 0) + (r == nreads - 1 && e != nbytes) + (e < s || e > nbytes);
+        if (r == 0 && first_is_continuation) l = ~0ull;
+        len = len > l ? len : l;
+        if (first_rec && e > s) {
+            const uint64_t e2 = e < nbytes ? e : nbytes;
+            for (uint64_t b = (s + ((1ull << FIRST_REC_SHIFT) - 1ull)) >> FIRST_REC_SHIFT; (b << FIRST_REC_SHIFT) < e2; b++) first_rec[b] = (uint32_t)r;
+        }
+    };
+    if ((reinterpret_cast<uintptr_t>(offs) & 15u) == 0) {
+        const uint64_t npairs = (nreads + 1) / 2;
+        const uint32_t lane = threadIdx.x & 63u;
+        for (uint64_t qw = (uint64_t)blockIdx.x * blockDim.x + (threadIdx.x & ~63u); qw < npairs; qw += 4 * stride) {
+            ulonglong2 pv[4];
+            uint64_t xv[4];
+#pragma unroll
+            for (int u = 0; u < 4; u++) {
+                const uint64_t q = qw + lane + (uint64_t)u * stride;
+                const bool act = q < npairs;
+                pv[u] = act ? *reinterpret_cast<const ulonglong2 *>(offs + 2 * q) : make_ulonglong2(0ull, 0ull);
+                xv[u] = (act && 2 * q + 1 < nreads && (lane == 63u || q + 1 >= npairs)) ? offs[2 * q + 2] : 0ull;
+            }
+#pragma unroll
+            for (int u = 0; u < 4; u++) {
+                const uint64_t q = qw + lane + (uint64_t)u * stride;
+                uint64_t nx = __shfl_down((unsigned long long)pv[u].x, 1, 64);
+                if (lane == 63u || q + 1 >= npairs) nx = xv[u];
+                if (q >= npairs) continue;
+                record(2 * q, pv[u].x, pv[u].y);
+                if (2 * q + 1 < nreads) record(2 * q + 1, pv[u].y, nx);
+            }
+        }
+    } else {
+        for (uint64_t rb = (uint64_t)blockIdx.x * blockDim.x + threadIdx.x; rb < nreads; rb += 4 * stride) {
+            uint64_t sv[4], ev[4];
+#pragma unroll
+            for (int u = 0; u < 4; u++) {
+                const uint64_t r = rb + (uint64_t)u * stride;
+                sv[u] = r < nreads ? offs[r] : 0ull;
+                ev[u] = r < nreads ? offs[r + 1] : 0ull;
+            }
+#pragma unroll
+            for (int u = 0; u < 4; u++) {
+                const uint64_t r = rb + (uint64_t)u * stride;
+                if (r >= nreads) break;
+                record(r, sv[u], ev[u]);
             }
         }
     }
@@ -233,12 +261,10 @@
     return residue_has_n_free_window(bases, s, e, p, k);
 }
 
-__global__ void __launch_bounds__(256)
-resolve_suspects_kernel(const uint8_t *__restrict__ bases, uint64_t nbytes, const uint64_t *__restrict__ offs , uint64_t nreads,
-                        int k, DevCounters *ctr)
+__device__ __forceinline__ void resolve_suspects(const uint8_t *__restrict__ bases, uint64_t nbytes, const uint64_t *__restrict__ offs ,
+                                                 uint64_t nreads, int k, DevCounters *ctr, unsigned long long tid, unsigned long long nthreads)
 {
     const unsigned long long listed = ctr->sus_count;
-    const unsigned long long tid = (unsigned long long)blockIdx.x * blockDim.x + threadIdx.x, nthreads = (unsigned long long)gridDim.x * blockDim.x;
     unsigned long long bad = 0;
     if (listed <= ctr->sus_cap) {
         for (unsigned long long i = tid; i < listed; i += nthreads)
@@ -270,6 +296,15 @@
     }
     if (bad) __hip_atomic_fetch_add(&ctr->n_bad, bad, __ATOMIC_RELAXED, __HIP_MEMORY_SCOPE_AGENT);
 }
+
+__global__ void __launch_bounds__(256)
+resolve_suspects_kernel(const uint8_t *__restrict__ bases, uint64_t nbytes, const uint64_t *__restrict__ offs , uint64_t nreads,
+                        int k, DevCounters *ctr)
+{
+    resolve_suspects(bases, nbytes, offs, nreads, k, ctr, (unsigned long long)blockIdx.x * blockDim.x + threadIdx.x, (unsigned long long)gridDim.x * blockDim.x);
+}
+
+struct SuspectsJob { const uint8_t *bases; uint64_t nbytes; const uint64_t *offs; uint64_t nreads; int k; };
 
 __device__ __forceinline__ uint32_t gather16(uint32_t y0, uint32_t y1, uint32_t y2, uint32_t y3)
 {
diff --git a/kmerdb_amd/csrc/kdb_scatter.hip.h b/kmerdb_amd/csrc/kdb_scatter.hip.h
--- a/kmerdb_amd/csrc/kdb_scatter.hip.h
+++ b/kmerdb_amd/csrc/kdb_scatter.hip.h
@@ -257,7 +257,17 @@
     uint32_t wg_base;
     uint32_t grid;
     uint32_t extra_elems;
+    uint32_t *fin;
 };
+
+constexpr uint32_t SC_FIN_MAX_GRID = 4096;
+inline size_t sc_fin_words(size_t nb) { return 4 * nb + 3 + SC_FIN_MAX_GRID; }
+__host__ __device__ __forceinline__ uint32_t sc_slice_pages(uint32_t ntiles, uint32_t tile_pos)
+{
+    const uint32_t est_pages = (uint32_t)(((uint64_t)ntiles * tile_pos * 2) / SC_PAGE_BYTES) + 1u;
+    const uint32_t sp = (est_pages + 511u) / 512u;
+    return sp < 128u ? 128u : sp;
+}
 
 __device__ __forceinline__ uint32_t sc_pin(uint32_t v) { asm volatile("" : "+s"(v)); return v; }
 
@@ -507,6 +517,95 @@
     ctr->table_dirty = 1;
 }
 
+template <int THREADS>
+__device__ __forceinline__ void sc_finish_counts(const ScOut &out, uint32_t *lds, const uint32_t *taken , uint32_t nb,
+                                                 uint32_t slice_pages, DevCounters *ctr)
+{
+    constexpr uint32_t MISC = 2048;
+    uint32_t *const cp = lds, *const ce = lds + nb;
+    uint32_t *const s_pages = lds + MISC, *const s_lines = lds + MISC + 1, *const s_last = lds + MISC + 2, *const wsum = lds + MISC + 8;
+    unsigned long long *const s_tot = reinterpret_cast<unsigned long long *>(lds + MISC + 4);
+    uint32_t *const bkt_pages = out.fin, *const bkt_elems = out.fin + nb, *const page_base = out.fin + 2 * nb, *const slice_base = out.fin + 3 * nb + 1;
+    uint32_t *const ticket = out.fin + 4 * nb + 2, *const used = ticket + 1;
+    const uint32_t j = threadIdx.x;
+    if (nb > 1024u) {
+        if (j == 0) __hip_atomic_fetch_add(&ctr->internal_err, 1ull, __ATOMIC_RELAXED, __HIP_MEMORY_SCOPE_AGENT);
+        return;
+    }
+    __syncthreads();
+    uint32_t npg = taken ? *taken : 0u;
+    if (npg > out.wg_pages) npg = out.wg_pages;
+    for (uint32_t b = j; b < 2u * nb; b += THREADS) lds[b] = 0;
+    if (j == 0) { *s_pages = 0; *s_lines = 0; *s_last = 0; *s_tot = 0ull; }
+    __syncthreads();
+    uint32_t my_pages = 0, my_lines = 0;
+    for (uint32_t p = j; p < npg; p += THREADS) {
+        const uint32_t pg = out.contig ? out.wg_base + p : p * out.grid + out.wg_base;
+        const uint32_t t = __hip_atomic_load(&out.tag[pg], __ATOMIC_RELAXED, __HIP_MEMORY_SCOPE_AGENT);
+        const uint32_t b = t >> SC_TAG_SHIFT, n = t & ((1u << SC_TAG_SHIFT) - 1u);
+        if (t == SC_NO_PAGE || n == 0 || b >= nb) continue;
+        my_pages++; my_lines += (n + 31u) / 32u;
+        atomicAdd(&cp[b], 1u); atomicAdd(&ce[b], n);
+    }
+#pragma unroll
+    for (int o = 32; o > 0; o >>= 1) { my_pages += (uint32_t)__shfl_xor((int)my_pages, o, 64); my_lines += (uint32_t)__shfl_xor((int)my_lines, o, 64); }
+    if ((j & 63u) == 0 && my_pages) { atomicAdd(s_pages, my_pages); atomicAdd(s_lines, my_lines); }
+    __syncthreads();
+    for (uint32_t b = j; b < nb; b += THREADS)
+        if (cp[b]) {
+            __hip_atomic_fetch_add(&bkt_pages[b], cp[b], __ATOMIC_RELAXED, __HIP_MEMORY_SCOPE_AGENT);
+            __hip_atomic_fetch_add(&bkt_elems[b], ce[b], __ATOMIC_RELAXED, __HIP_MEMORY_SCOPE_AGENT);
+        }
+    if (j == 0) {
+        __hip_atomic_store(&used[blockIdx.x], npg, __ATOMIC_RELAXED, __HIP_MEMORY_SCOPE_AGENT);
+        if (*s_pages) {
+            __hip_atomic_fetch_add(&ctr->pages_bases, (unsigned long long)*s_pages, __ATOMIC_RELAXED, __HIP_MEMORY_SCOPE_AGENT);
+            __hip_atomic_fetch_add(&ctr->lines_bases, (unsigned long long)*s_lines, __ATOMIC_RELAXED, __HIP_MEMORY_SCOPE_AGENT);
+        }
+    }
+    asm volatile("s_waitcnt vmcnt(0)" ::: "memory");
+    __syncthreads();
+    if (j == 0) {
+        __builtin_amdgcn_fence(__ATOMIC_RELEASE, "agent");
+        asm volatile("s_waitcnt vmcnt(0)" ::: "memory");
+        const uint32_t tk = __hip_atomic_fetch_add(ticket, 1u, __ATOMIC_RELAXED, __HIP_MEMORY_SCOPE_AGENT);
+        if (tk == out.grid - 1u) {
+            __builtin_amdgcn_fence(__ATOMIC_ACQUIRE, "agent");
+            asm volatile("s_waitcnt vmcnt(0)" ::: "memory");
+            *s_last = 1u;
+        }
+    }
+    __syncthreads();
+    if (*s_last == 0u) return;
+    const uint32_t per = (nb + (uint32_t)THREADS - 1u) / (uint32_t)THREADS;
+    const uint32_t lo = j * per < nb ? j * per : nb, hi = lo + per < nb ? lo + per : nb;
+    uint32_t sum = 0, ssum = 0;
+    unsigned long long el = 0;
+    for (uint32_t i = lo; i < hi; i++) {
+        const uint32_t v = __hip_atomic_load(&bkt_pages[i], __ATOMIC_RELAXED, __HIP_MEMORY_SCOPE_AGENT);
+        sum += v; ssum += (v + slice_pages - 1u) / slice_pages;
+        el += __hip_atomic_load(&bkt_elems[i], __ATOMIC_RELAXED, __HIP_MEMORY_SCOPE_AGENT);
+        __hip_atomic_store(&bkt_elems[i], 0u, __ATOMIC_RELAXED, __HIP_MEMORY_SCOPE_AGENT);
+        cp[i] = v;
+    }
+    uint32_t tot, stot;
+    uint32_t run = block_excl_scan<THREADS>(sum, wsum, &tot);
+    uint32_t srun = block_excl_scan<THREADS>(ssum, wsum, &stot);
+    for (uint32_t i = lo; i < hi; i++) {
+        const uint32_t v = cp[i];
+        page_base[i] = run; slice_base[i] = srun;
+        run += v; srun += (v + slice_pages - 1u) / slice_pages;
+    }
+    el = wave_sum(el);
+    if ((j & 63u) == 0 && el) atomicAdd(s_tot, el);
+    __syncthreads();
+    if (j == 0) {
+        page_base[nb] = tot; slice_base[nb] = stot;
+        if (*s_tot) __hip_atomic_fetch_add(&ctr->total_kmers, *s_tot, __ATOMIC_RELAXED, __HIP_MEMORY_SCOPE_AGENT);
+        __hip_atomic_store(ticket, 0u, __ATOMIC_RELAXED, __HIP_MEMORY_SCOPE_AGENT);
+    }
+}
+
 __global__ void hot_side_kernel(DevCounters *ctr, unsigned long long *side, unsigned long long cap)
 {
     if (side) { side[0] = 0ull; side[1] = cap; }
@@ -585,7 +684,8 @@
 {
     constexpr int NID = 16;
     if ((batch_uniform_len(ctr) == 0u) != RAGGED) return;
-    if (RAGGED && ctr->bad_layout) return;
+    const bool no_walk = RAGGED && ctr->bad_layout;
+    if (no_walk && !out_arg.fin) return;
     constexpr int TILE_CHUNKS = THREADS, TILE_STRIDE = THREADS - 1, TILE_POS = TILE_STRIDE * 16;
     using Tile = ScTile<EXPAND, TILE_CHUNKS>;
     if (K == 17 && !ElemFmt<ELEM>::HI) { k = 17; ring_shift = SC_LO_BITS_TWO_LEVEL + 9; ring_bits = 9; sub_log2 = __builtin_ctz((unsigned)RINGS) - 9; }
@@ -598,7 +698,12 @@
     __shared__ Tile T[2];
     static_assert(sizeof(Tile) >= THREADS * sizeof(LineDesc), "a dead tile image holds the waves' line lists");
     __shared__ RingLds<ELEM, RINGS, C> R;
+    static_assert(sizeof(R.ring) >= 16384, "the dead rings hold sc_finish_counts' counters");
     const int j = threadIdx.x;
+    if (no_walk) {
+        sc_finish_counts<THREADS>(out, reinterpret_cast<uint32_t *>(R.ring), nullptr, 1u << ring_bits, sc_slice_pages(ntiles, (uint32_t)TILE_POS), ctr);
+        return;
+    }
     for (int b = j; b < RINGS; b += THREADS) R.word[b] = 0;
     if (j == 0) { R.pg_count = 0; R.retry[0] = 0; R.retry[1] = 0; T[0].has_n[0] = 0; T[1].has_n[0] = 0; T[0].ncnt = 0; T[1].ncnt = 0; }
     if (j < SC_HOT) { R.hot_tag[j] = 0ull; R.hot_cnt[j] = 0; }
@@ -920,6 +1025,9 @@
         if (wb) __hip_atomic_fetch_add(&ctr->n_bad, wb, __ATOMIC_RELAXED, __HIP_MEMORY_SCOPE_AGENT);
         if (wm) __hip_atomic_fetch_add(&ctr->marks_seen, wm, __ATOMIC_RELAXED, __HIP_MEMORY_SCOPE_AGENT);
     }
+    if (out.fin) {
+        sc_finish_counts<THREADS>(out, reinterpret_cast<uint32_t *>(R.ring), &R.pg_count, 1u << ring_bits, sc_slice_pages(ntiles, (uint32_t)TILE_POS), ctr);
+    }
 }
 
 struct PageEntry { uint32_t page, nelems; };
@@ -1199,6 +1307,40 @@
     }
 }
 
+__global__ void __launch_bounds__(PAGES_THREADS)
+pages_place_used_kernel(const uint32_t *__restrict__ tag, const uint32_t *__restrict__ used, uint32_t wg_pages, uint32_t contig, uint32_t nb,
+                        uint32_t *__restrict__ bkt_pages, const uint32_t *__restrict__ page_base, PageEntry *__restrict__ list, SuspectsJob sus, DevCounters *ctr)
+{
+    __shared__ uint32_t cur[1024];
+    const uint32_t w = blockIdx.x, G = gridDim.x - (sus.bases ? 1u : 0u);
+    if (w == G) { resolve_suspects(sus.bases, sus.nbytes, sus.offs, sus.nreads, sus.k, ctr, threadIdx.x, PAGES_THREADS); return; }
+    uint32_t n_used = used[w];
+    if (n_used > wg_pages) n_used = wg_pages;
+    if (n_used == 0 || nb > 1024u) return;
+    const uint32_t base = contig ? w * wg_pages : w, step = contig ? 1u : G;
+    for (uint32_t b = threadIdx.x; b < nb; b += PAGES_THREADS) cur[b] = 0;
+    __syncthreads();
+    for (uint32_t p = threadIdx.x; p < n_used; p += PAGES_THREADS) {
+        const uint32_t t = tag[base + p * step];
+        if (t != SC_NO_PAGE && (t & ((1u << SC_TAG_SHIFT) - 1u)) && (t >> SC_TAG_SHIFT) < nb) atomicAdd(&cur[t >> SC_TAG_SHIFT], 1u);
+    }
+    __syncthreads();
+    for (uint32_t b = threadIdx.x; b < nb; b += PAGES_THREADS) {
+        const uint32_t c = cur[b];
+        if (c) cur[b] = page_base[b] + atomicSub(&bkt_pages[b], c) - c;
+    }
+    __syncthreads();
+    for (uint32_t p = threadIdx.x; p < n_used; p += PAGES_THREADS) {
+        const uint32_t pg = base + p * step, t = tag[pg];
+        if (t == SC_NO_PAGE) continue;
+        const uint32_t b = t >> SC_TAG_SHIFT, n = t & ((1u << SC_TAG_SHIFT) - 1u);
+        if (n == 0 || b >= nb) continue;
+        const uint32_t pos = atomicAdd(&cur[b], 1u);
+        list[pos].page = pg;
+        list[pos].nelems = n;
+    }
+}
+
 constexpr uint32_t WRAP_MAX = 4096;
 template <uint32_t CAP> struct WrapListT { uint32_t n; uint32_t e[CAP]; };
 using WrapList = WrapListT<WRAP_MAX>;
@@ -1454,10 +1596,16 @@
     }
     if (st.bkt_cap < nb) {
         if (st.d_bkt) { if (hipStreamSynchronize(stream) != hipSuccess) return 1; (void)hipFree(st.d_bkt); st.d_bkt = nullptr; st.bkt_cap = 0; }
-        if (hipMalloc((void **)&st.d_bkt, (4 * nb + 2) * sizeof(uint32_t)) != hipSuccess) { (void)hipGetLastError(); return 2; }
+        if (hipMalloc((void **)&st.d_bkt, sc_fin_words(nb) * sizeof(uint32_t)) != hipSuccess) { (void)hipGetLastError(); return 2; }
         st.bkt_cap = nb;
+        if (hipMemsetAsync(st.d_bkt, 0, sc_fin_words(nb) * sizeof(uint32_t), stream) != hipSuccess) return 1;
     }
     return 0;
+}
+
+inline int scatter_clear(ScatterState &st, hipStream_t stream)
+{
+    return st.d_bkt && hipMemsetAsync(st.d_bkt, 0, sc_fin_words(st.bkt_cap) * sizeof(uint32_t), stream) != hipSuccess ? 1 : 0;
 }
 
 constexpr int SC1_THREADS = 1024, SC1_RINGS = 1024, SC1_GRID = 256, SC1_K = 13;
@@ -1469,7 +1617,7 @@
     uint32_t tile_stride, tile_pos, Gmax;
     uint64_t ntiles_all, max_tiles;
 };
-struct ScLaunch { uint32_t nt, G, npages; };
+struct ScLaunch { uint32_t nt, G, npages, wg_pages; };
 
 inline ScGeom scatter_geometry(const ScatterState &st, size_t nbytes, int k, uint32_t grid_default = 0)
 {
@@ -1515,10 +1663,10 @@
     out.extra_elems = scatter_extra_elems((nt + G - 1) / G, g.tile_pos, n_expand);
     out.wg_pages = scatter_wg_pages((nt + G - 1) / G, g.rings, 512, g.tile_pos, out.extra_elems);
     out.wg_range = nullptr; out.contig = (uint32_t)st.contig_pages; out.wg_base = 0; out.grid = 0;
+    out.fin = st.d_bkt;
     const uint32_t npages = G * out.wg_pages;
-    L->nt = nt; L->G = G; L->npages = npages;
-    if (hipMemsetAsync(st.d_tag, 0xFF, (size_t)npages * sizeof(uint32_t), stream) != hipSuccess ||
-        hipMemsetAsync(st.d_bkt, 0, 2 * (size_t)nb * sizeof(uint32_t), stream) != hipSuccess) { partition_error_ref() = "memset failed"; return 1; }
+    L->nt = nt; L->G = G; L->npages = npages; L->wg_pages = out.wg_pages;
+    if (G > SC_FIN_MAX_GRID || nb > 1024 || (size_t)nb > st.bkt_cap) { partition_error_ref() = "one-level scatter: grid or bucket count out of range"; return 1; }
     prof.begin_on(KDB_KERNEL_SCATTER, stream);
 #define KDB_LAUNCH_SC1(EL, CC, E, CN, KK, RG, TH, RAG)                                                                                     \
     hipLaunchKernelGGL((scatter_bases_kernel<uint32_t, EL, RG, CC, 16, E, CN, KK, TH, RAG>), dim3(G), dim3(TH), 0, stream, d_bases,       \
@@ -1552,23 +1700,18 @@
     return 0;
 }
 
-inline int scatter_stage2(ScatterState &st, hipStream_t stream, const ScGeom &g, const ScLaunch &L, unsigned long long *d_table, DevCounters *d_ctr, ProfHook &prof)
-{
+inline int scatter_stage2(ScatterState &st, hipStream_t stream, const ScGeom &g, const ScLaunch &L, unsigned long long *d_table, DevCounters *d_ctr, ProfHook &prof,
+                          const SuspectsJob *sus = nullptr )
+{
+    const SuspectsJob sj = sus ? *sus : SuspectsJob{nullptr, 0, nullptr, 0, 0};
     const int nb = g.nb;
     const uint32_t npages = L.npages;
-    uint32_t *const bkt_pages = st.d_bkt, *const bkt_elems = st.d_bkt + nb, *const page_base = st.d_bkt + 2 * nb, *const slice_base = st.d_bkt + 3 * nb + 1;
+    uint32_t *const bkt_pages = st.d_bkt, *const page_base = st.d_bkt + 2 * nb, *const slice_base = st.d_bkt + 3 * nb + 1;
     prof.begin_on(KDB_KERNEL_PAGE_SORT, stream);
-    const uint32_t pgrid = (npages + 4095u) / 4096u < 256u ? (npages + 4095u) / 4096u : 256u;
-    const uint32_t target = 512u;
-    const uint32_t est_pages = (uint32_t)(((uint64_t)L.nt * g.tile_pos * 2) / SC_PAGE_BYTES) + 1u;
-    uint32_t slice_pages = (est_pages + target - 1) / target;
-    if (slice_pages < 128u) slice_pages = 128u;
-    hipLaunchKernelGGL(pages_count_kernel, dim3(pgrid), dim3(PAGES_THREADS), 0, stream, (const uint32_t *)st.d_tag, npages, (uint32_t)nb, bkt_pages, bkt_elems,
-                       &d_ctr->pages_bases, 32u);
-    hipLaunchKernelGGL(pages_scan_kernel, dim3(1), dim3(1024), 0, stream, (const uint32_t *)bkt_pages, (const uint32_t *)bkt_elems, (uint32_t)nb,
-                       page_base, slice_base, slice_pages, d_ctr);
-    hipLaunchKernelGGL(pages_place_kernel, dim3(pgrid), dim3(PAGES_THREADS), 0, stream, (const uint32_t *)st.d_tag, npages, (uint32_t)nb, bkt_pages,
-                       (const uint32_t *)page_base, st.d_list);
+    const uint32_t slice_pages = sc_slice_pages(L.nt, g.tile_pos);
+    hipLaunchKernelGGL(pages_place_used_kernel, dim3(L.G + (sj.bases ? 1u : 0u)), dim3(PAGES_THREADS), 0, stream, (const uint32_t *)st.d_tag,
+                       (const uint32_t *)(st.d_bkt + 4 * nb + 3), L.wg_pages, (uint32_t)st.contig_pages, (uint32_t)nb, bkt_pages, (const uint32_t *)page_base, st.d_list,
+                       sj, d_ctr);
     prof.end();
     prof.begin_on(KDB_KERNEL_PAGE_HIST, stream);
     const uint32_t p2_grid = npages / slice_pages + (uint32_t)nb + 1u;
@@ -1584,14 +1727,14 @@
 }
 
 inline int scatter_count(ScatterState &st, hipStream_t stream, const uint8_t *d_bases, size_t nbytes, const RecStarts &rs, int k, int canonical, int n_expand,
-                         unsigned long long *d_table, DevCounters *d_ctr, ProfHook &prof)
+                         unsigned long long *d_table, DevCounters *d_ctr, ProfHook &prof, const SuspectsJob *sus = nullptr)
 {
     const ScGeom g = scatter_geometry(st, nbytes, k);
     { const int rc = scatter_reserve_for(st, stream, g, n_expand); if (rc) return rc; }
     for (uint64_t t0 = 0; t0 < g.ntiles_all; t0 += g.max_tiles) {
         ScLaunch L;
         if (scatter_stage1(st, stream, g, t0, d_bases, nbytes, rs, k, canonical, n_expand, d_table, d_ctr, prof, &L)) return 1;
-        if (scatter_stage2(st, stream, g, L, d_table, d_ctr, prof)) return 1;
+        if (scatter_stage2(st, stream, g, L, d_table, d_ctr, prof, t0 + g.max_tiles >= g.ntiles_all ? sus : nullptr)) return 1;
     }
     return 0;
 }
@@ -1839,7 +1982,7 @@
         const uint32_t nt = (uint32_t)((ntiles_all - t0) < max_tiles ? (ntiles_all - t0) : max_tiles);
         const uint32_t G = nt < Gmax ? nt : Gmax;
         ScOut out1;
-        out1.pages = tp.l1.d_pages; out1.tag = tp.l1.d_tag; out1.wg_range = nullptr; out1.contig = (uint32_t)tp.l1.contig_pages; out1.wg_base = 0; out1.grid = 0;
+        out1.pages = tp.l1.d_pages; out1.tag = tp.l1.d_tag; out1.wg_range = nullptr; out1.contig = (uint32_t)tp.l1.contig_pages; out1.wg_base = 0; out1.grid = 0; out1.fin = nullptr;
         out1.extra_elems = scatter_extra_elems((nt + G - 1) / G, tile_pos1, n_expand);
         out1.wg_pages = scatter_wg_pages((nt + G - 1) / G, rings1, l1_page_elems, tile_pos1, out1.extra_elems);
         const uint32_t npages1 = G * out1.wg_pages;
@@ -1970,7 +2113,7 @@
             }
         }
         ScOut out2;
-        out2.pages = tp.d_pages2; out2.tag = tp.d_tag2; out2.wg_pages = 0; out2.wg_range = tp.d_wg_range; out2.contig = 0; out2.wg_base = 0; out2.grid = 0; out2.extra_elems = 0;
+        out2.pages = tp.d_pages2; out2.tag = tp.d_tag2; out2.wg_pages = 0; out2.wg_range = tp.d_wg_range; out2.contig = 0; out2.wg_base = 0; out2.grid = 0; out2.extra_elems = 0; out2.fin = nullptr;
         prof.begin(KDB_KERNEL_SCATTER_L2);
 #define KDB_LAUNCH_L2(IN, EL, CC, FX, TH)                                                                                                       \
     hipLaunchKernelGGL((scatter_ids_kernel<IN, EL, 512, CC, FX, TH>), dim3(G2), dim3(TH), 0, stream, (const uint8_t *)tp.l1.d_pages,            \
```
